# Xiugapurin/Etude

Measured on AMD Instinct MI355X. Metric: audio-sec/s transcribed + decoder tokens/s, 3-min clip batch, higher is better.
Workload: dtype f16

## Files before the change

etude_amd/_lib.py:

```python
from __future__ import annotations

import ctypes as C
import os
from pathlib import Path

import torch

LIB_PATH = Path(os.environ["ETD_LIB_PATH"]) if os.environ.get("ETD_LIB_PATH") else Path(__file__).resolve().parent / "libetude_hip.so"

c_int_p = C.POINTER(C.c_int)
c_i32_p = C.POINTER(C.c_int32)
c_i64_p = C.POINTER(C.c_int64)
c_f32_p = C.POINTER(C.c_float)


class _SizedCfg(C.Structure):

    def __init__(self, *a, **k):
        super().__init__(*a, **k)
        self.struct_bytes = C.sizeof(type(self))


class ExtCfg(_SizedCfg):
    _fields_ = [("struct_bytes", C.c_int)] + [(n, C.c_int) for n in ("n_margin", "n_frame", "n_bin", "cnn_channel", "cnn_kernel", "hid_dim", "pf_dim",
# ... 156 lines not shown
    "etd_prof_entry": (C.c_int, [C.c_int, C.c_char_p, C.c_int, C.POINTER(C.c_double), C.POINTER(C.c_longlong),
                                 C.POINTER(C.c_double), C.POINTER(C.c_double)]),
    "etd_debug_boundary_cost": (C.c_int, [C.c_int, C.c_int, C.c_int, C.c_void_p, C.POINTER(C.c_double), C.POINTER(C.c_double)]),
    "etd_debug_linear": (C.c_int, [C.c_int, C.c_int, C.c_int, C.c_int, C.c_void_p, C.POINTER(C.c_double)]),
    "etd_debug_kernel_loop": (C.c_int, [C.c_int, C.c_int, C.c_void_p]),
    "etd_debug_g3_bounds": (C.c_int, [C.c_void_p, C.c_void_p, C.c_int, C.c_int, C.c_void_p, C.c_void_p, C.c_float, C.c_void_p, C.c_void_p]),
    "etd_debug_gemm3": (C.c_int, [C.c_void_p, C.c_int, C.c_int, C.c_void_p, C.c_void_p, C.c_int, C.c_float, C.c_int, C.c_void_p, C.c_void_p, C.c_void_p, C.c_void_p]),
    "etd_debug_gemm3_case": (C.c_int, [C.POINTER(G3Case), C.c_void_p]),
    "etd_debug_ln_rows_f32": (C.c_int, [C.c_void_p, C.c_int, C.c_int, C.c_void_p, C.c_void_p, C.c_void_p, C.c_void_p, C.c_float, C.c_void_p, C.c_void_p, C.c_void_p]),
    "etd_debug_g3_pack": (C.c_int, [C.c_void_p, C.c_int, C.c_int, C.c_void_p, C.c_longlong, C.POINTER(C.c_longlong), C.POINTER(C.c_int32)]),
    "etd_debug_attn3": (C.c_int, [C.c_void_p, C.c_void_p, C.c_void_p, C.c_void_p, C.c_int, C.c_int, C.c_int, C.c_int, C.c_float, C.c_float, C.c_float, C.c_int, C.c_void_p, C.c_void_p]),
    "etd_debug_attn3_case": (C.c_int, [C.POINTER(Attn3Case), C.c_void_p]),
    "etd_debug_dattn_f32": (C.c_int, [C.c_void_p, C.c_void_p, C.c_void_p, C.c_void_p, C.c_longlong, C.c_longlong, C.c_int, C.c_int, C.c_int, C.c_int, C.c_void_p, C.c_void_p,
                                      C.c_int, C.c_void_p]),
    "etd_debug_empty_launch": (C.c_int, [C.c_int, C.c_int, C.c_int, C.c_void_p, C.c_void_p]),
    "etd_frontend_create": (C.c_int, [C.c_int, C.c_int, C.c_int, C.c_int, C.c_int, C.c_int, C.c_void_p, C.c_int, C.c_int,
                                      C.c_void_p, C.c_int, C.c_void_p, C.c_void_p, C.c_void_p, C.c_float, C.POINTER(C.c_void_p)]),
    "etd_frontend_destroy": (None, [C.c_void_p]),
    "etd_frontend_set_pad_mode": (C.c_int, [C.c_void_p, C.c_int]),
    "etd_rms_frames": (C.c_int, [C.c_void_p, C.c_longlong, C.c_int, C.c_int, C.c_void_p, C.c_longlong, C.c_void_p]),
    "etd_frontend_resampled_len": (C.c_longlong, [C.c_void_p, C.c_longlong]),
    "etd_frontend_num_frames": (C.c_longlong, [C.c_void_p, C.c_longlong]),
    "etd_frontend_run": (C.c_int, [C.c_void_p, C.c_void_p, C.c_int, C.c_longlong, C.c_void_p, C.c_void_p, C.c_longlong,
                                   C.POINTER(C.c_longlong), C.c_void_p]),
    "etd_extractor_create": (C.c_int, [C.POINTER(ExtCfg), C.POINTER(C.c_char_p), C.POINTER(C.c_void_p), c_i64_p, C.c_int,
                                       C.POINTER(C.c_void_p)]),
    "etd_extractor_destroy": (None, [C.c_void_p]),
    "etd_transcript": (C.c_int, [C.c_void_p, C.c_void_p, C.c_longlong] + [C.c_void_p] * 8 + [C.c_void_p]),
    "etd_transcript_windows": (C.c_int, [C.c_void_p, C.c_void_p, C.c_int] + [C.c_void_p] * 8 + [C.c_void_p]),
    "etd_extractor_debug_vel_logits": (C.c_int, [C.c_void_p, C.c_void_p]),
    "etd_extractor_debug_tap": (C.c_int, [C.c_void_p, C.c_int, C.c_void_p]),
    "etd_extractor_window_flops": (C.c_double, [C.c_void_p]),
    "etd_mpe2note": (C.c_int, [C.c_void_p, C.c_void_p, C.c_void_p, C.c_void_p, C.c_longlong, C.c_int, C.c_float, C.c_float,
                               C.c_float, C.c_int, C.c_int, C.c_int, C.POINTER(Note), C.c_longlong, C.POINTER(C.c_longlong)]),
    "etd_mpe2note_modes": (C.c_int, [C.c_void_p, C.c_void_p, C.c_void_p, C.c_void_p, C.c_longlong, C.c_int, C.c_float, C.c_float,
                                     C.c_float, C.c_int, C.c_int, C.c_int, C.c_int, C.c_int, C.POINTER(Note), C.c_longlong, C.POINTER(C.c_longlong)]),
    "etd_mpe2note_dev_create": (C.c_int, [C.c_int, C.POINTER(C.c_void_p)]),
    "etd_mpe2note_dev_destroy": (None, [C.c_void_p]),
    "etd_mpe2note_dev": (C.c_int, [C.c_void_p, C.c_void_p, C.c_void_p, C.c_void_p, C.c_void_p, C.c_longlong, C.c_float, C.c_float, C.c_float,
                                   C.c_int, C.c_int, C.c_int, C.POINTER(Note), C.c_longlong, C.POINTER(C.c_longlong), C.c_void_p]),
    "etd_mpe2note_dev_modes": (C.c_int, [C.c_void_p, C.c_void_p, C.c_void_p, C.c_void_p, C.c_void_p, C.c_longlong, C.c_float, C.c_float, C.c_float,
                                         C.c_int, C.c_int, C.c_int, C.c_int, C.c_int, C.POINTER(Note), C.c_longlong, C.POINTER(C.c_longlong), C.c_void_p]),
    "etd_tok_create": (C.c_int, [C.c_void_p, C.c_int, C.POINTER(C.c_void_p)]),
    "etd_tok_destroy": (None, [C.c_void_p]),
    "etd_tok_num_measures": (C.c_int, [C.c_void_p]),
    "etd_tok_measures": (C.c_int, [C.c_void_p, C.c_void_p, C.c_void_p, C.c_void_p, C.c_void_p]),
    "etd_tok_encode": (C.c_int, [C.c_void_p, C.c_void_p, C.c_longlong, C.c_int, C.c_void_p, C.c_longlong, C.POINTER(C.c_longlong)]),
    "etd_tok_split_bars": (C.c_int, [C.c_void_p, C.c_longlong, C.c_int, C.c_int, C.c_void_p, C.c_longlong, C.c_void_p, C.c_longlong,
                                     C.POINTER(C.c_longlong)]),
    "etd_tok_decode": (C.c_int, [C.c_void_p, C.c_void_p, C.c_longlong, C.c_void_p, C.c_longlong, C.c_void_p, C.c_longlong,
                                 C.POINTER(C.c_longlong)]),
    "etd_midi_write": (C.c_int, [C.c_void_p, C.c_longlong, C.c_char_p]),
    "etd_decoder_create": (C.c_int, [C.POINTER(DecCfg), C.POINTER(C.c_char_p), C.POINTER(C.c_void_p), c_i64_p, C.c_int,
                                     C.POINTER(C.c_void_p)]),
    "etd_decoder_destroy": (None, [C.c_void_p]),
    "etd_decoder_clone": (C.c_int, [C.c_void_p, C.POINTER(C.c_void_p)]),
    "etd_decoder_set_sampling": (C.c_int, [C.c_void_p, C.c_float, C.c_float, C.c_ulonglong, C.c_void_p]),
    "etd_decoder_set_keys": (C.c_int, [C.c_void_p, C.c_int, C.c_void_p, C.c_void_p]),
    "etd_decoder_begin_bar": (C.c_int, [C.c_void_p, C.c_int, C.c_void_p, C.c_void_p, C.c_void_p, C.c_int, C.c_void_p, C.c_int,
                                        C.c_int, C.c_void_p]),
    "etd_decoder_begin_bars": (C.c_int, [C.c_void_p, C.c_int] + [C.c_void_p] * 8 + [C.c_void_p]),
    "etd_decoder_step": (C.c_int, [C.c_void_p, C.c_void_p, C.c_int, C.c_int, C.c_void_p]),
    "etd_decoder_poll": (C.c_int, [C.c_void_p, C.c_void_p, C.c_int, C.c_void_p, C.c_void_p, C.c_void_p]),
    "etd_decoder_read_tokens": (C.c_int, [C.c_void_p, C.c_int, C.c_void_p, C.c_int, c_int_p, C.c_void_p]),
    "etd_decoder_read_many": (C.c_int, [C.c_void_p, C.c_int, C.c_void_p, C.c_void_p, C.c_int, C.c_void_p, C.c_void_p]),
    "etd_decoder_run_jobs": (C.c_int, [C.c_void_p, C.POINTER(SchedCfg), C.POINTER(Job), C.c_int, C.c_void_p, C.c_longlong, C.c_void_p,
                                       C.POINTER(C.c_longlong), C.c_void_p]),
    "etd_debug_assemble_prompt": (C.c_int, [C.POINTER(SchedCfg), C.c_int, C.c_void_p, C.c_void_p, C.c_void_p, C.c_void_p, C.c_void_p, C.c_void_p,
                                            C.c_int, C.c_void_p, C.c_void_p, C.c_void_p, C.c_void_p, C.c_int, c_int_p]),
    "etd_decoder_generate_bar": (C.c_int, [C.c_void_p, C.c_int, C.c_void_p, C.c_void_p, C.c_void_p, C.c_int, C.c_void_p,
                                           C.c_int, C.c_int, C.c_void_p, c_int_p, C.c_void_p]),
    "etd_decoder_prefill_logits": (C.c_int, [C.c_void_p, C.c_int, C.c_void_p, C.c_void_p, C.c_void_p, C.c_int, C.c_void_p,
                                             C.c_void_p]),
    "etd_decoder_score": (C.c_int, [C.c_void_p, C.c_int] + [C.c_void_p] * 11 + [C.c_void_p]),
    "etd_decoder_score_jobs": (C.c_int, [C.c_void_p, C.POINTER(SchedCfg), C.POINTER(ScoreJob), C.c_int, C.c_void_p, C.c_void_p, C.c_void_p, C.c_void_p]),
    "etd_debug_assemble_scored": (C.c_int, [C.POINTER(SchedCfg), C.c_int, C.c_void_p, C.c_void_p, C.c_void_p, C.c_void_p, C.c_void_p, C.c_void_p,
                                            C.c_int, C.c_void_p, C.c_int, C.c_void_p, C.c_void_p, C.c_void_p, C.c_void_p, C.c_void_p, C.c_int, c_int_p]),
    "etd_decoder_step_bytes": (C.c_double, [C.c_void_p, C.c_int, C.c_int]),
    "etd_decoder_stats": (C.c_int, [C.c_void_p, C.POINTER(C.c_double), C.c_int, C.c_void_p]),
    "etd_decoder_stats_reset": (C.c_int, [C.c_void_p, C.c_void_p]),
    "etd_decoder_stamp": (C.c_int, [C.c_void_p, C.c_int, C.c_int, C.c_void_p]),
    "etd_decoder_stamp_log": (C.c_int, [C.c_void_p, C.c_void_p, C.c_longlong, C.POINTER(C.c_longlong), C.c_void_p]),
    "etd_debug_decoder_force_pair": (C.c_int, [C.c_void_p, C.c_int]),
    "etd_debug_decoder_step_logits": (C.c_int, [C.c_void_p, C.c_int, C.c_void_p, C.c_int, C.c_void_p]),
    "etd_debug_decoder_bar_logits": (C.c_int, [C.c_void_p, C.c_void_p, C.c_int, C.c_void_p]),
    "etd_debug_sample_rows": (C.c_int, [C.c_void_p, C.c_int, C.c_int, C.c_int, C.c_float, C.c_float, C.c_ulonglong, C.c_void_p, C.c_void_p, C.c_void_p, C.c_void_p]),
    "etd_debug_decoder_checksum": (C.c_int, [C.c_void_p, C.POINTER(C.c_ulonglong), C.c_int, C.c_void_p]),
    "etd_debug_decoder_kv_rowsums": (C.c_int, [C.c_void_p, C.c_void_p, C.c_longlong, C.c_void_p]),
    "etd_debug_decoder_trace_begin": (C.c_int, [C.c_void_p, C.c_int, C.c_void_p]),
    "etd_debug_decoder_trace_slabs": (C.c_int, [C.c_void_p, C.c_void_p, C.c_longlong, C.c_int, C.c_void_p]),
    "etd_debug_decoder_trace_lanes": (C.c_int, [C.c_void_p, C.c_void_p, C.c_longlong, C.c_int, C.c_void_p]),
    "etd_debug_decoder_trace_q": (C.c_int, [C.c_void_p, C.c_void_p, C.c_longlong, C.c_int, C.c_void_p]),
    "etd_debug_decoder_stage_taps": (C.c_int, [C.c_void_p, C.c_void_p, C.c_void_p]),
    "etd_debug_decoder_peek_kv_many": (C.c_int, [C.c_void_p, C.c_int, C.c_int, C.c_void_p, C.c_int, C.c_void_p, C.c_void_p, C.c_void_p]),
    "etd_debug_decoder_peek_kv": (C.c_int, [C.c_void_p, C.c_int, C.c_int, C.c_int, C.c_int, C.c_void_p, C.c_void_p, C.c_void_p]),
    "etd_beat_create": (C.c_int, [C.POINTER(BeatCfg), C.POINTER(C.c_char_p), C.POINTER(C.c_void_p), c_i64_p, C.c_int, C.POINTER(C.c_void_p)]),
    "etd_beat_destroy": (None, [C.c_void_p]),
    "etd_beat_forward": (C.c_int, [C.c_void_p, C.c_void_p, C.c_int, c_i64_p, C.c_void_p, C.c_void_p, C.c_void_p]),
    "etd_beat_flops": (C.c_double, [C.c_void_p, C.c_longlong]),
    "etd_beat_debug_taps": (C.c_int, [C.c_void_p, C.c_void_p, C.c_void_p]),
    "etd_beat_debug_stage_taps": (C.c_int, [C.c_void_p, C.c_void_p]),
    "etd_dbn_describe": (C.c_int, [C.POINTER(DbnCfg), C.c_int, C.c_void_p, C.c_int, c_int_p, c_int_p, c_int_p, C.c_void_p, C.c_void_p]),
    "etd_dbn_workspace_bytes": (C.c_longlong, [C.POINTER(DbnCfg), C.c_longlong, C.c_int]),
    "etd_dbn_create": (C.c_int, [C.POINTER(DbnCfg), C.POINTER(C.c_void_p)]),
    "etd_dbn_destroy": (None, [C.c_void_p]),
    "etd_dbn_track": (C.c_int, [C.c_void_p, C.c_void_p, C.c_int, C.c_int, c_i64_p, C.c_void_p, C.c_longlong, C.c_void_p, C.c_void_p, C.c_void_p, C.c_longlong,
                                C.c_void_p, C.c_void_p, C.POINTER(C.c_longlong), C.c_void_p]),
    "etd_dbn_debug_viterbi": (C.c_int, [C.c_void_p, C.c_int, C.c_void_p, C.c_longlong, C.c_void_p, C.POINTER(C.c_double)]),
    "etd_stemfeat_create": (C.c_int, [C.POINTER(StemFeatCfg), C.c_void_p, C.c_void_p, C.c_void_p, C.c_void_p, C.POINTER(C.c_void_p)]),
    "etd_stemfeat_destroy": (None, [C.c_void_p]),
    "etd_stemfeat_num_frames": (C.c_longlong, [C.c_void_p, C.c_longlong]),
    "etd_stemfeat_workspace_bytes": (C.c_longlong, [C.c_void_p, C.c_int, C.c_int, c_i64_p]),
    "etd_stemfeat_run": (C.c_int, [C.c_void_p, C.POINTER(C.c_void_p), C.c_int, C.c_int, C.c_int, c_i64_p, C.c_void_p, C.c_void_p]),
    "etd_dtw_create": (C.c_int, [C.POINTER(DtwCfg), C.POINTER(C.c_void_p)]),
    "etd_dtw_destroy": (None, [C.c_void_p]),
    "etd_dtw_limits": (C.c_int, [c_int_p, c_int_p, C.POINTER(C.c_longlong), c_int_p]),
    "etd_dtw_workspace_bytes": (C.c_longlong, [C.c_void_p, C.c_int, c_i64_p, c_i64_p, C.POINTER(C.c_longlong), c_i64_p]),
    "etd_dtw_align": (C.c_int, [C.c_void_p, C.POINTER(C.c_void_p), C.c_int, c_i64_p, c_i64_p, C.c_void_p, C.c_longlong, C.c_void_p, C.c_longlong, C.c_void_p, C.c_void_p]),
    "etd_dtw_debug_cost": (C.c_int, [C.c_void_p, C.POINTER(C.c_void_p), C.c_longlong, C.c_longlong, C.c_int, C.c_void_p]),
    "etd_dtw_debug_path": (C.c_int, [C.c_void_p, C.POINTER(C.c_void_p), C.c_longlong, C.c_longlong, C.c_int, C.c_void_p, C.c_longlong, C.POINTER(C.c_longlong)]),
    "etd_dtw_debug_total": (C.c_int, [C.c_void_p, C.POINTER(C.c_void_p), C.c_longlong, C.c_longlong, C.c_int, C.POINTER(C.c_double)]),
    "etd_alignfeat_limits": (C.c_int, [c_int_p, c_int_p, C.POINTER(C.c_longlong), c_int_p, c_int_p]),
    "etd_alignfeat_create": (C.c_int, [C.POINTER(AlignFeatCfg), C.c_void_p, C.c_void_p, C.c_void_p, C.c_void_p, C.POINTER(C.c_void_p)]),
    "etd_alignfeat_destroy": (None, [C.c_void_p]),
    "etd_alignfeat_num_frames": (C.c_longlong, [C.c_void_p, C.c_longlong]),
    "etd_alignfeat_workspace_bytes": (C.c_longlong, [C.c_void_p, C.c_int, c_i64_p]),
    "etd_alignfeat_run": (C.c_int, [C.c_void_p, C.POINTER(C.c_void_p), C.c_int, c_i64_p, c_i32_p, C.c_void_p, C.c_void_p, C.c_void_p, C.c_longlong, C.c_void_p]),
    "etd_alignfeat_debug_layout": (C.c_int, [C.c_void_p, C.c_int, c_i64_p, C.c_int, c_i64_p, C.c_int]),
    "etd_tuning_limits": (C.c_int, [C.POINTER(C.c_longlong), C.POINTER(C.c_longlong), c_int_p]),
    "etd_tuning_create": (C.c_int, [C.POINTER(TuningCfg), C.POINTER(C.c_void_p)]),
    "etd_tuning_destroy": (None, [C.c_void_p]),
    "etd_tuning_workspace_bytes": (C.c_longlong, [C.c_void_p, C.c_int, c_i64_p]),
    "etd_tuning_run": (C.c_int, [C.c_void_p, C.POINTER(C.c_void_p), C.c_int, c_i64_p, C.c_void_p, C.c_void_p, C.c_void_p, C.c_longlong, C.c_void_p]),
    "etd_tuning_debug_layout": (C.c_int, [C.c_void_p, C.c_int, c_i64_p, C.c_int, c_i64_p, C.c_int]),
    "etd_tuning_debug_power": (C.c_int, [C.c_void_p, C.c_int, c_i32_p, C.c_int, C.c_void_p]),
    "etd_resample_create": (C.c_int, [C.POINTER(ResampleCfg), C.c_void_p, C.POINTER(C.c_void_p)]),
    "etd_resample_destroy": (None, [C.c_void_p]),
    "etd_resample_out_len": (C.c_longlong, [C.c_void_p, C.c_longlong]),
    "etd_resample_workspace_bytes": (C.c_longlong, [C.c_void_p, C.c_int, c_i64_p, c_i32_p, c_i32_p]),
    "etd_resample_run": (C.c_int, [C.c_void_p, C.POINTER(C.c_void_p), C.c_int, c_i64_p, c_i32_p, c_i32_p, c_i32_p, c_i64_p, C.POINTER(C.c_void_p), C.c_void_p, C.c_longlong, C.c_void_p]),
    "etd_resample_debug_layout": (C.c_int, [C.c_void_p, C.c_int, c_i64_p, c_i32_p, c_i32_p, c_i64_p, C.c_longlong, C.POINTER(C.c_longlong)]),
    "etd_rhythm_limits": (C.c_int, [c_int_p, c_int_p, c_int_p, c_int_p]),
    "etd_rhythm_create": (C.c_int, [C.POINTER(RhythmCfg), C.POINTER(C.c_void_p)]),
    "etd_rhythm_destroy": (None, [C.c_void_p]),
    "etd_rhythm_check": (C.c_int, [C.c_void_p, c_i64_p, C.c_int]),
    "etd_rhythm_run": (C.c_int, [C.c_void_p, C.c_void_p, C.c_void_p, c_i64_p, C.c_int, C.c_void_p, C.c_void_p, C.c_void_p]),
    "etd_rhythm_debug_logioi": (C.c_int, [C.c_void_p, C.c_void_p, C.c_void_p, C.c_void_p]),
    "etd_attr_limits": (C.c_int, [c_int_p, c_int_p, c_int_p, c_int_p]),
    "etd_attr_create": (C.c_int, [C.POINTER(AttrCfg), C.c_void_p, C.c_int, C.POINTER(C.c_void_p)]),
    "etd_attr_destroy": (None, [C.c_void_p]),
    "etd_attr_check": (C.c_int, [C.c_void_p, c_i64_p, C.c_int]),
    "etd_attr_run": (C.c_int, [C.c_void_p, C.c_void_p, C.c_void_p, c_i64_p, C.c_int, C.c_void_p, C.c_void_p, C.c_void_p, c_i64_p, C.c_int, C.c_void_p, C.c_int,
                               C.c_void_p, C.c_void_p, C.c_void_p, C.c_void_p, C.c_void_p, C.c_void_p, C.c_void_p]),
    "etd_render_limits": (C.c_int, [c_int_p, C.POINTER(C.c_longlong), c_int_p, c_int_p, c_int_p]),
    "etd_render_create": (C.c_int, [C.POINTER(RenderCfg), C.POINTER(C.c_void_p)]),
    "etd_render_destroy": (None, [C.c_void_p]),
    "etd_render_bytes": (C.c_longlong, [C.c_void_p, C.c_int, c_i64_p, c_i64_p]),
    "etd_render_run": (C.c_int, [C.c_void_p, C.c_void_p, c_i64_p, C.c_void_p, C.c_int, c_i64_p, c_i64_p, C.c_void_p, C.c_void_p, C.c_longlong, C.c_void_p]),
    "etd_render_peaks": (C.c_int, [C.c_void_p, C.c_void_p, C.c_void_p, C.c_void_p, C.c_int, C.c_void_p, C.c_void_p]),
    "etd_render_debug_plan": (C.c_int, [C.c_void_p, C.c_void_p, c_i64_p, C.c_int, c_i64_p, C.c_void_p, C.c_void_p]),
    "etd_sep_create": (C.c_int, [C.POINTER(SepCfg), C.POINTER(C.c_char_p), C.POINTER(C.c_char_p), C.POINTER(C.c_void_p), c_i64_p, C.c_int, C.POINTER(C.c_void_p)]),
    "etd_sep_destroy": (None, [C.c_void_p]),
    "etd_sep_num_frames": (C.c_longlong, [C.c_void_p, C.c_longlong]),
    "etd_sep_unit_bytes": (C.c_longlong, [C.c_void_p]),
    "etd_sep_workspace_bytes": (C.c_longlong, [C.c_void_p, C.c_int, c_i64_p]),
    "etd_sep_run": (C.c_int, [C.c_void_p, C.POINTER(C.c_void_p), C.c_int, c_i64_p, C.POINTER(C.c_void_p), C.c_void_p]),
# ... 175 lines not shown
```

etude_amd/csrc/api_dec.hip:

```cpp
#include <algorithm>
#include <atomic>
#include <chrono>
#include <cmath>
#include <cstdlib>
#include <cstring>
#include <map>
#include <string>
#include <mutex>
#include <vector>

#include "../../include/etude_hip_debug.h"
#include "dec_kernels.h"
#include "gemm3.h"
#include "ext_kernels.h"
#include "dec_score.h"
#include "prof.h"

namespace {

inline uint16_t f2bf_h(float f) { return ETD_DEC_IS_F16 ? f32_to_f16_bits(f) : f32_to_bf16_bits(f); }

struct Lin { void* W = nullptr; float* b = nullptr; int N = 0, Npad = 0, K = 0;
             void* Wf = nullptr;
             G3Lin g3; };
struct Layer { float *ln1g, *ln1b, *ln2g, *ln2b; Lin qkv, dense, up, down;
               void* dense_hw = nullptr;
               Lin cat;
               void* mlp_frag = nullptr;
               int q_log2 = 0, k_log2 = 0, v_log2 = 0; };

}

#define ETD_STAMP_WORDS (ETD_STAMP_HDR + 2 * ETD_STAMP_LOGCAP)
struct etd_dec {
  etd_dec_cfg cfg;
  DevPool pool;
  bool bf16w = false;
  int H, I, V, L, nh, S, ctx, Mmax, Mcap, out_cap;
  float *word = nullptr, *cls_emb = nullptr, *attr_tab = nullptr;
  std::vector<Layer> layers;
  float *lnfg = nullptr, *lnfb = nullptr;
  Lin head;
  float *X1f = nullptr, *X2f = nullptr;
  float *t_q = nullptr, *t_ao = nullptr, *t_do = nullptr, *t_m1 = nullptr;
  void* head_frag = nullptr;
  float *rope_cos = nullptr, *rope_sin = nullptr;
  void *Kc = nullptr, *Vc = nullptr;
  long long slot_stride = 0, layer_stride = 0;
  float *h = nullptr, *h2 = nullptr, *Q = nullptr, *AO = nullptr, *DO = nullptr, *M1 = nullptr, *logits = nullptr;
  int *row_slot = nullptr, *row_pos = nullptr, *row_active = nullptr, *row_sp = nullptr, *ids = nullptr, *slots_dev = nullptr;
  int *cur_tok = nullptr, *len = nullptr, *done = nullptr, *n_out = nullptr, *eos = nullptr, *limit = nullptr, *tgt_attrs = nullptr, *out_tok = nullptr;
  float* tgt_proj = nullptr;
  std::vector<int> last_slots;
  float* qkv_raw = nullptr;
  d16 *X1b = nullptr, *X2b = nullptr, *AOb = nullptr, *M1b = nullptr;
  d16* Qb = nullptr;
  float* hlast = nullptr;
  DSampleCfg* samp_dev = nullptr;
  unsigned long long* rng_key = nullptr;
  std::vector<unsigned long long> host_key; bool keys_dirty = true; bool sampling = false;
  float* Pk = nullptr;
  unsigned* trace = nullptr; int* trace_step = nullptr; int trace_cap = 0; float* trace_pk = nullptr; float* trace_q = nullptr; float* trace_dbg = nullptr;
  int* row_cnt = nullptr;
  d16* Xcat = nullptr;
  std::vector<int> stage;
  int* pin_stage = nullptr; size_t pin_stage_ints = 0; hipEvent_t pin_stage_evt = nullptr;
  int* pin_rb = nullptr;
  std::vector<int> host_n_out; bool host_n_out_valid = false;
  std::map<int, hipGraphExec_t> graphs;
  bool rows_identity = false;
  std::vector<int> host_len;
  double attn_bytes_hint = 0;
  bool step_pair = false;
  double stat_steps = 0, stat_row_steps = 0, stat_kv_bytes = 0, stat_attn_launches = 0, stat_stamp_bytes = 0;
  int force_pair = -1;
  unsigned long long* stamp_dev = nullptr;
  bool stamp_on = false, stamp_armed = false; long long stamp_skip = 0;
  int bar_logit_rows = 0;
  float* logits_dbg = nullptr; bool logits_dbg_on = false, last_step_fused = false;
  int* sc_i = nullptr; float* sc_f = nullptr; double* sc_d = nullptr; float* sc_x = nullptr; int score_hb = 0;
  etd_debug_dec_taps taps = {}; bool taps_on = false;
  etd_dec* weights_owner = nullptr;
  size_t n_weight_allocs = 0;
  int n_clones = 0; bool zombie = false;
};

namespace {

int load_lin(etd_dec* d, const WeightTable& L, const std::string& pfx, int N, int K, bool has_bias, Lin* w) {
  const float* W = L.get(pfx + ".weight", (int64_t)N * K);
  if (!W) return ETD_EINVAL;
  const float* b = nullptr;
  if (has_bias) { b = L.get(pfx + ".bias", N); if (!b) return ETD_EINVAL; }
  const int Npad = ((N + 127) / 128) * 128;
  w->N = N; w->Npad = Npad; w->K = K;
  DevPool& P = d->pool;
  if (d->bf16w) {
    std::vector<uint16_t> hb((size_t)Npad * K, 0);
    for (size_t i = 0; i < (size_t)N * K; ++i) hb[i] = f2bf_h(W[i]);
    uint16_t* p; ETD_TRY(P.upload(&p, hb.data(), hb.size()));
    w->W = p;
    if (K % 16 == 0) {
      std::vector<uint16_t> hp(hb.size());
      pack_wfrag_host(hb.data(), Npad, K, hp.data());
      uint16_t* pf; ETD_TRY(P.upload(&pf, hp.data(), hp.size()));
      w->Wf = pf;
    }
  } else {
    std::vector<float> hf((size_t)Npad * K, 0.f);
    memcpy(hf.data(), W, (size_t)N * K * 4);
    float* p; ETD_TRY(P.upload(&p, hf.data(), hf.size()));
    w->W = p;
    if (K % 32 == 0) {
      ETD_TRY(g3_lin_upload(P, W, b, N, K, 0.f, &w->g3));
      w->b = w->g3.b;
      return ETD_OK;
    }
  }
  std::vector<float> hb2(Npad, 0.f);
  if (b) memcpy(hb2.data(), b, (size_t)N * 4);
  return P.upload(&w->b, hb2.data(), hb2.size());
}

int load_vec(etd_dec* d, const WeightTable& L, const std::string& name, int n, float** dst) {
  const float* p = L.get(name, n);
  if (!p) return ETD_EINVAL;
  return d->pool.upload(dst, p, n);
}

struct PrefillInfo { int n; const int* seq_row0; const int* seq_len; int max_len; double attn_flops; };
__global__ __launch_bounds__(64) void k_trace_rows(const unsigned* buf, long long row_stride, int words, long long slab_stride, int M,
                                                   unsigned* trace, const int* step, int cap, long long wps, int off) {
  const int row = blockIdx.x, slab = blockIdx.y, lane = threadIdx.x;
  const unsigned* p = buf + (long long)slab * slab_stride + (long long)row * row_stride;
  unsigned acc = 0;
  for (int i = lane; i < words; i += 64) acc += p[i] * (2654435761u * (unsigned)(i + 1) | 1u);
  for (int o = 32; o; o >>= 1) acc += __shfl_xor(acc, o);
  if (lane == 0) trace[(long long)(*step % cap) * wps + off + slab * M + row] = acc;
}
__global__ __launch_bounds__(64) void k_trace_kv(const unsigned* Kc, const unsigned* Vc, long long slot_stride_w, int max_ctx, const int* row_slot, const int* row_pos, int M,
                                                 unsigned* trace, const int* step, int cap, long long wps, int off) {
  const int row = blockIdx.x, head = blockIdx.y, lane = threadIdx.x;
  const int slot = row_slot[row], pos = row_pos[row] < max_ctx ? row_pos[row] : max_ctx - 1;
  unsigned* out = trace + (long long)(*step % cap) * wps + off;
  for (int which = 0; which < 2; ++which) {
    const unsigned* base = (which ? Vc : Kc) + (long long)slot * slot_stride_w + (long long)head * max_ctx * 32;
    unsigned a_new = 0, a_all = 0;
    for (long long i = lane; i < (long long)(pos + 1) * 32; i += 64) {
      const unsigned w = base[i] * (2654435761u * (unsigned)(i + 1) | 1u);
      a_all += w;
      if (i >= (long long)pos * 32) a_new += w;
    }
    for (int o = 32; o; o >>= 1) { a_new += __shfl_xor(a_new, o); a_all += __shfl_xor(a_all, o); }
    if (lane == 0) { out[(which * 8 + head) * M + row] = a_new; out[(16 + which * 8 + head) * M + row] = a_all; }
  }
}
__global__ void k_trace_next(int* step) { *step += 1; }
#define ETD_TRACE_LAYER 49
static inline long long trace_wps(const etd_dec* d, int M) { return (long long)(ETD_TRACE_LAYER * d->L + 2) * M; }
static int trace_rows(etd_dec* d, const void* buf, long long row_stride, int words, int nslab, long long slab_stride, int M, int off, hipStream_t st) {
  hipLaunchKernelGGL(k_trace_rows, dim3(M, nslab), dim3(64), 0, st, (const unsigned*)buf, row_stride, words, slab_stride, M, d->trace, d->trace_step,
                     d->trace_cap, trace_wps(d, M), off);
  HIP_TRY(hipGetLastError());
  return ETD_OK;
// ... 177 lines not shown
                       d->row_slot, d->row_pos, M, d->trace, d->trace_step, d->trace_cap, trace_wps(d, M), l * ETD_TRACE_LAYER * M + 17 * M);
    HIP_TRY(hipGetLastError());
  }
  return ETD_OK;
}
static int skinny_attn_down(etd_dec* d, int l, const DecRows& rows, int M, const float* hin, float* hout, hipStream_t st, int ts) {
  const Layer& w = d->layers[l]; const NextLn nx = next_ln(d, l);
  const int ksd = d->I / 512;
  DAttnArgs at = attn_args(d, l, rows, M);
  attn_step_pairs(d, &at); attn_stamp(d, l, &at); at.pair = d->step_pair ? 1 : 0;
  at.dense_w = (const d16*)w.dense_hw; at.dense_out = d->Pk + (size_t)ksd * M * d->H; at.dbg = (d->trace && l == 0) ? d->trace_dbg : nullptr;
  DGemmArgs dn = lin_args(w.cat, nullptr, d->I + d->H, M); dn.Xb = d->Xcat; dn.k_splits = ksd; dn.Y = d->Pk; dn.ldy = d->H;
  if (rowfin_on() && ksd + d->nh == 12 && M <= DS_STEP_MAX_ROWS) {
    DRowFin fin = {};
    fin.cnt = d->row_cnt + (size_t)l * DS_STEP_MAX_ROWS; fin.target = d->nh + 16 * ksd; fin.P = d->Pk; fin.nslab = 12;
    fin.bias = w.cat.b; fin.hin = hin; fin.hout = hout; fin.eps = d->cfg.layer_norm_eps;
    fin.g1 = nx.g1; fin.b1 = nx.b1; fin.g2 = nx.g2; fin.b2 = nx.b2; fin.x1 = nx.x1; fin.x2 = nx.x2;
    return launch_dstep_attn_down(at, dn, &fin, st);
  }
  ETD_TRY(launch_dstep_attn_down(at, dn, nullptr, st));
  ETD_TRY(tap_xcat(d, ts, M, st));
  ETD_TRY(tap_slabs(d, ts, ksd + d->nh, M, st));
  if (d->trace && ksd + d->nh == 12) ETD_TRY(trace_rows(d, d->Pk, d->H, d->H, 12, (long long)M * d->H, M, l * ETD_TRACE_LAYER * M + 2 * M, st));
  if (d->trace && l == 0 && ksd + d->nh == 12) HIP_TRY(hipMemcpyAsync(d->trace_pk, d->Pk, (size_t)12 * M * d->H * 4, hipMemcpyDeviceToDevice, st));
  ETD_TRY(resid_ln(d, l, ksd + d->nh, hin, hout, M, nx, st));
  ETD_TRY(tap_rows(d, d->taps.hout, ts, hout, M, d->H, 4, st));
  if (d->trace) {
    ETD_TRY(trace_rows(d, hout, d->H, d->H, 1, 0, M, l * ETD_TRACE_LAYER * M + 14 * M, st));
    if (nx.x1) {
      ETD_TRY(trace_rows(d, d->X1b, d->H / 2, d->H / 2, 1, 0, M, l * ETD_TRACE_LAYER * M + 15 * M, st));
      ETD_TRY(trace_rows(d, d->X2b, d->H / 2, d->H / 2, 1, 0, M, l * ETD_TRACE_LAYER * M + 16 * M, st));
    }
  }
  return ETD_OK;
}
static int forward_skinny16(etd_dec* d, int M, const DecRows& rows, bool ln0_done, hipStream_t st, float** hfinal) {
  const bool attn_down = rows.slot == d->row_slot && d->H == 512 && d->nh == 8 && d->I % 512 == 0 && d->I / 512 + d->nh <= 12 && d->layers[0].dense_hw &&
                         d->ctx >= 256 && !getenv("ETD_NO_ATTN_DOWN");
  float* hin = d->h; float* hout = d->h2;
  if (!ln0_done) ETD_TRY(ln_rows16(d, 0, hin, M, st));
  for (int l = 0; l < d->L; ++l) {
    const int ts = tap_slice(d, l);
    ETD_TRY(tap_layer_in(d, ts, hin, M, st));
    ETD_TRY(step_qkv_up(d, l, hin, rows, M, st));
    ETD_TRY(tap_rows(d, d->taps.q, ts, d->Q, M, d->H, 4, st));
    ETD_TRY(trace_qkv_up(d, l, M, st));
    if (attn_down) ETD_TRY(skinny_attn_down(d, l, rows, M, hin, hout, st, ts));
    else {
      ETD_TRY(layer_dattn(d, l, rows, M, d->Xcat + d->I, d->I + d->H, st));
      ETD_TRY(tap_xcat(d, ts, M, st));
      ETD_TRY(down_splitk(d, l, hin, hout, M, next_ln(d, l), st, ts));
    }
    std::swap(hin, hout);
  }
  *hfinal = hin;
  return ETD_OK;
}

static int prefill16_qkv(etd_dec* d, int l, const float* hin, const DecRows& rows, int M, bool mfma_attn, hipStream_t st) {
  const Layer& w = d->layers[l];
  DGemmArgs q = qkv_args(d, l, hin, rows, M); q.Xb = d->X1b; q.Y = d->qkv_raw; q.ldy = 3 * d->H;
  if (mfma_attn) q.Qb = d->Qb;
  static const bool pqkv_on = !getenv("ETD_NO_PQKV");
  if (!(mfma_attn && pqkv_on && M >= 49152 && d->H == 512 && d->nh == 8 && w.qkv.N == 1536)) return linear16(w.qkv, d->X1b, M, q, DEPI_QKV, st);
  PQkvArgs pa = {};
  pa.X = d->X1b; pa.ldx = d->H; pa.Wf = (const d16*)w.qkv.Wf; pa.bias = w.qkv.b; pa.M = M; pa.N = w.qkv.N; pa.rows = rows;
  pa.rope_cos = d->rope_cos; pa.rope_sin = d->rope_sin; pa.Qb = d->Qb; pa.Kc = (d16*)q.Kc; pa.Vc = (d16*)q.Vc; pa.slot_stride = d->slot_stride; pa.max_ctx = d->ctx; pa.n_heads = d->nh;
  return launch_pqkv(pa, st);
}
static int prefill16_layer_rest(etd_dec* d, int l, const DecRows& rows, int M, const PrefillInfo* pf, bool fmlp, const float* hin, float* hout, hipStream_t st) {
  const Layer& w = d->layers[l]; const int ts = tap_slice(d, l);
  if (pf) {
    PAttnArgs t = {};
    t.Q = d->Qb; t.ldq = d->H; t.Kc = (const d16*)kv_layer(d, d->Kc, l); t.Vc = (const d16*)kv_layer(d, d->Vc, l); t.slot_stride = d->slot_stride; t.max_ctx = d->ctx; t.n_heads = d->nh;
    t.O = d->Xcat + d->I; t.ldo = d->I + d->H; t.seq_row0 = pf->seq_row0; t.seq_len = pf->seq_len; t.row_slot = rows.slot;
    t.n_seq = pf->n; t.max_len = pf->max_len; t.scale_log2e = 0.125f * 1.4426950408889634f; t.flops_hint = pf->attn_flops;
    ETD_TRY(launch_pattn(t, st));
  } else ETD_TRY(layer_dattn(d, l, rows, M, d->Xcat + d->I, d->I + d->H, st));
  if (fmlp) {
    const NextLn nx = next_ln(d, l); DMlpArgs ma = {};
    ma.X2 = d->X2b; ma.AO = d->Xcat + d->I; ma.ldao = d->I + d->H; ma.hin = hin; ma.hout = hout; ma.Wm = (const d16*)w.mlp_frag;
    ma.b_up = w.up.b; ma.b_cat = w.cat.b; ma.eps = d->cfg.layer_norm_eps; ma.M = M;
    ma.g1 = nx.g1; ma.b1 = nx.b1; ma.g2 = nx.g2; ma.b2 = nx.b2; ma.nx1 = nx.x1; ma.nx2 = nx.x2;
    ETD_TRY(tap_xcat(d, ts, M, st));
    ETD_TRY(launch_dmlp_fused(ma, st));
    return tap_rows(d, d->taps.hout, ts, hout, M, d->H, 4, st);
  }
  DGemmArgs up = {}; up.Yb = d->Xcat; up.ldy = d->I + d->H;
  ETD_TRY(linear16(w.up, d->X2b, M, up, DEPI_GELU, st));
  ETD_TRY(tap_xcat(d, ts, M, st));
  DGemmArgs dn = {}; dn.N = d->H; dn.hin = hin; dn.hout = hout;
  ETD_TRY(linear16(w.cat, d->Xcat, M, dn, DEPI_RESID, st));
  return tap_rows(d, d->taps.hout, ts, hout, M, d->H, 4, st);
}
static int prefill16_last_rows(etd_dec* d, const LastOnly& lo, const float* hin, float* hout, hipStream_t st) {
  const int n = lo.n, l = d->L - 1, ts = tap_slice(d, l, true);
  ETD_TRY(launch_gather_rows(hin, lo.idx, n, d->H, d->hlast, st));
  ETD_TRY(ln_rows16(d, l, d->hlast, n, st));
  ETD_TRY(tap_layer_in(d, ts, d->hlast, n, st));
  ETD_TRY(step_qkv_up(d, l, d->hlast, lo.rows, n, st));
  ETD_TRY(tap_rows(d, d->taps.q, ts, d->Q, n, d->H, 4, st));
  DAttnArgs at = attn_args(d, l, lo.rows, n); at.O = d->AO; at.Ob = d->Xcat + d->I; at.ldob = d->I + d->H; at.bytes_hint = 0;
  ETD_TRY(launch_dattn(at, d->bf16w, st));
  ETD_TRY(tap_xcat(d, ts, n, st));
  return down_splitk(d, l, d->hlast, hout, n, NextLn{}, st, ts);
}
static int forward_prefill16(etd_dec* d, int M, const DecRows& rows, const PrefillInfo* pf, const LastOnly* lo, hipStream_t st, float** hfinal, bool* compact) {
  const bool fmlp = d->layers[0].mlp_frag && d->H == 512 && d->I == 2048 && fused_pmlp_on();
  const bool tail = lo && pf && lo->n > 1 && lo->n <= DS_STEP_MAX_ROWS && step_shape(d) && !getenv("ETD_NO_LAST_ONLY");
  float* hin = d->h; float* hout = d->h2;
  for (int l = 0; l < d->L; ++l) {
    if (l == 0 || !fmlp) ETD_TRY(ln_rows16(d, l, hin, M, st));
    const int ts = tap_slice(d, l);
    ETD_TRY(tap_layer_in(d, ts, hin, M, st));
    ETD_TRY(prefill16_qkv(d, l, hin, rows, M, pf != nullptr, st));
    ETD_TRY(pf ? tap_rows(d, d->taps.qb, ts, d->Qb, M, d->H, 2, st) : tap_rows(d, d->taps.q, ts, d->Q, M, d->H, 4, st));
    ETD_TRY(tail && l == d->L - 1 ? prefill16_last_rows(d, *lo, hin, hout, st) : prefill16_layer_rest(d, l, rows, M, pf, fmlp, hin, hout, st));
    std::swap(hin, hout);
  }
  *hfinal = hin; if (tail) *compact = true;
  return ETD_OK;
}

static int forward_rows(etd_dec* d, int M, const DecRows& rows, const PrefillInfo* pf, const LastOnly* lo, hipStream_t st, float** hfinal, bool* compact) {
  if (compact) *compact = false; else lo = nullptr;
  const Layer& w0 = d->layers[0];
  if (!d->bf16w && M >= G3_MIN_ROWS && d->X1f && w0.qkv.g3.Wp && w0.down.g3.Wp) return forward_x3(d, M, rows, pf, lo, st, hfinal, compact);
  const bool act16 = d->bf16w && M > 1;
  if (act16 && M > DS_MAX_ROWS && w0.qkv.Wf && w0.up.Wf && w0.cat.Wf) return forward_prefill16(d, M, rows, pf, lo, st, hfinal, compact);
  if (act16 && ksplit_fits(d)) return forward_skinny16(d, M, rows, false, st, hfinal);
  return forward_plain(d, M, rows, act16, st, hfinal);
}

int head_logits(etd_dec* d, const float* X, int n, float* logits, hipStream_t st) {
  const bool g3 = !d->bf16w && n >= G3_MIN_ROWS && d->X1f && d->head.g3.Wp;
  if (g3) ETD_TRY(launch_ln_rows_f32(X, n, d->H, d->lnfg, d->lnfb, nullptr, nullptr, d->cfg.layer_norm_eps, d->X1f, nullptr, st));
  DGemmArgs lm = lin_args(d->head, g3 ? d->X1f : X, d->H, n);
  lm.bias = nullptr; lm.Y = logits; lm.ldy = d->V;
  if (g3) return launch_gemm3(lm, DEPI_LOGITS, st);
  lm.ln_g = d->lnfg; lm.ln_b = d->lnfb; lm.ln_eps = d->cfg.layer_norm_eps;
  return launch_dgemm(lm, DEPI_LOGITS, d->bf16w, st);
}

int check_slot(etd_dec* d, int slot) {
  if (!d || slot < 0 || slot >= d->S) ETD_FAIL(ETD_EINVAL, "decoder: bad slot %d", slot);
  return ETD_OK;
}

__global__ void k_init_slots(const int* __restrict__ init, int n, int* tgt_attrs, int* cur_tok, int* len, int* done, int* n_out, int* eos, int* limit) {
  const int i = blockIdx.x * blockDim.x + threadIdx.x;
  if (i >= n) return;
  const int* p = init + i * 7;
  const int s = p[0];
  tgt_attrs[4 * s] = p[1]; tgt_attrs[4 * s + 1] = p[2]; tgt_attrs[4 * s + 2] = p[3]; tgt_attrs[4 * s + 3] = p[4];
  cur_tok[s] = 0; len[s] = 0; done[s] = 0; n_out[s] = 0; eos[s] = p[5]; limit[s] = p[6];
}

__global__ __launch_bounds__(128) void k_slot_proj(const int* __restrict__ init, const float* __restrict__ attr_tab, int n_bins, int H, float* proj) {
  const int* p = init + blockIdx.x * 7;
  const int s = p[0];
  for (int k = threadIdx.x * 4; k < H; k += 128 * 4) {
    f32x4 t[4];
#pragma unroll
    for (int a = 0; a < 4; ++a) t[a] = *reinterpret_cast<const f32x4*>(attr_tab + (long long)(a * n_bins + p[1 + a]) * H + k);
    f32x4 o;
#pragma unroll
    for (int c = 0; c < 4; ++c) o[c] = ((t[0][c] + t[1][c]) + t[2][c]) + t[3][c];
    *reinterpret_cast<f32x4*>(proj + (long long)s * H + k) = o;
  }
}

struct Staged { int Mtot; const int *ids, *cls, *attrs, *row_slot, *row_pos, *row_active, *last_idx, *last_slot, *last_pos, *last_active, *init, *row_seq, *seq_row0, *seq_len; };

int stage_and_forward(etd_dec* d, int n, const int32_t* slots, const int32_t* T, const int32_t* ids, const int32_t* cls,
                      const int32_t* attrs4, const int32_t* init7 , Staged* sg, float** hfinal, hipStream_t st, bool* last_only = nullptr) {
  if (!d || n < 1 || n > d->S || !slots || !T || !ids || !cls || !attrs4) ETD_FAIL(ETD_EINVAL, "prefill: bad arguments");
  long long Mtot = 0;
  std::vector<char> seen((size_t)d->S, 0);
  for (int i = 0; i < n; ++i) {
    ETD_TRY(check_slot(d, slots[i]));
    if (T[i] <= 0 || T[i] > d->ctx) ETD_FAIL(ETD_EINVAL, "prefill: prompt %d has T=%d (max_ctx=%d)", i, T[i], d->ctx);
    if (seen[slots[i]]) ETD_FAIL(ETD_EINVAL, "prefill: slot %d listed twice", slots[i]);
    seen[slots[i]] = 1;
    Mtot += T[i];
  }
  if (Mtot > d->Mcap) ETD_FAIL(ETD_EINVAL, "prefill: %lld prompt rows exceed max_prefill_rows=%d", Mtot, d->Mcap);
  const int M = (int)Mtot;
  ETD_TRY(taps_fit(d, M, DS_K_SPLITS, n > 1 && M > DS_MAX_ROWS));
  for (int i = 0; i < M; ++i) {
    if (ids[i] < 0 || ids[i] >= d->V || cls[i] < 0 || cls[i] >= d->cfg.num_classes) ETD_FAIL(ETD_EINVAL, "prefill: token/class id out of range at row %d", i);
    for (int k = 0; k < 4; ++k) if (attrs4[(size_t)k * M + i] < 0 || attrs4[(size_t)k * M + i] >= d->cfg.num_attribute_bins) ETD_FAIL(ETD_EINVAL, "prefill: attribute bin out of range at row %d", i);
  }
  const size_t sv_ints = (size_t)10 * M + 13 * n;
  int* svp;
  const bool pinned = d->pin_stage && sv_ints <= d->pin_stage_ints;
  if (pinned) {
    HIP_TRY(hipEventSynchronize(d->pin_stage_evt));
    svp = d->pin_stage;
  } else {
    d->stage.resize(sv_ints);
    svp = d->stage.data();
  }
  memcpy(svp, ids, (size_t)M * 4);
  memcpy(svp + M, cls, (size_t)M * 4);
  memcpy(svp + 2 * (size_t)M, attrs4, (size_t)4 * M * 4);
  int* rs = svp + 6 * (size_t)M; int* rp = rs + M; int* ra = rp + M;
  int* li = ra + M; int* ls = li + n; int* lp = ls + n; int* la = lp + n; int* in7 = la + n;
  int* rq = in7 + 7 * n; int* sr0 = rq + M; int* sln = sr0 + n;
  int row = 0, max_len = 0; double kvb = 0, aflops = 0;
  for (int i = 0; i < n; ++i) {
    sr0[i] = row; sln[i] = T[i]; if (T[i] > max_len) max_len = T[i];
    aflops += 0.5 * 256.0 * d->nh * (double)T[i] * T[i];
    for (int t = 0; t < T[i]; ++t, ++row) { rs[row] = slots[i]; rp[row] = t; ra[row] = 1; rq[row] = i; }
    li[i] = row - 1; ls[i] = slots[i]; lp[i] = T[i] - 1; la[i] = 1;
    d->host_len[slots[i]] = T[i];
    kvb += (double)T[i] * d->nh * 64 * (2.0 * (d->bf16w ? 2 : 4) + 4 + 4);
  }
  if (init7) memcpy(in7, init7, (size_t)7 * n * 4); else memset(in7, 0, (size_t)7 * n * 4);
  d->attn_bytes_hint = kvb;
  HIP_TRY(hipMemcpyAsync(d->ids, svp, sv_ints * 4, hipMemcpyHostToDevice, st));
  if (pinned) HIP_TRY(hipEventRecord(d->pin_stage_evt, st));
  d->host_n_out_valid = false;
  const int* b = d->ids;
  *sg = Staged{M, b, b + M, b + 2 * (size_t)M, b + 6 * (size_t)M, b + 7 * (size_t)M, b + 8 * (size_t)M, b + 9 * (size_t)M, b + 9 * (size_t)M + n,
               b + 9 * (size_t)M + 2 * n, b + 9 * (size_t)M + 3 * n, b + 9 * (size_t)M + 4 * n,
               b + 9 * (size_t)M + 11 * n, b + 10 * (size_t)M + 11 * n, b + 10 * (size_t)M + 12 * n};
  if (init7) {
    hipLaunchKernelGGL(k_init_slots, dim3((n + 63) / 64), dim3(64), 0, st, sg->init, n, d->tgt_attrs, d->cur_tok, d->len, d->done, d->n_out, d->eos, d->limit);
    HIP_TRY(hipGetLastError());
    hipLaunchKernelGGL(k_slot_proj, dim3(n), dim3(128), 0, st, sg->init, d->attr_tab, d->cfg.num_attribute_bins, d->H, d->tgt_proj);
    HIP_TRY(hipGetLastError());
  }
  DEmbedArgs e = {};
  e.ids = sg->ids; e.cls = sg->cls; e.attrs = sg->attrs; e.M = M; e.H = d->H; e.n_bins = d->cfg.num_attribute_bins;
  e.word = d->word; e.cls_emb = d->cls_emb; e.attr_tab = d->attr_tab; e.h = d->h;
  e.rows = DecRows{sg->row_slot, sg->row_pos, sg->row_active, sg->row_seq};
  ETD_TRY(launch_dembed(e, st));
  PrefillInfo pf{n, sg->seq_row0, sg->seq_len, max_len, aflops};
  const bool can_mfma_attn = (d->bf16w ? d->Qb != nullptr : d->X1f != nullptr);
  LastOnly lo{n, sg->last_idx, DecRows{sg->last_slot, sg->last_pos, sg->last_active}};
  return forward_rows(d, M, e.rows, can_mfma_attn ? &pf : nullptr, &lo, st, hfinal, last_only);
}

int alloc_workspaces(etd_dec* d) {
  const int H = d->H;
  DevPool& P = d->pool;
  d->slot_stride = (long long)d->nh * d->ctx * 64;
  d->layer_stride = d->slot_stride * d->S;
  const size_t kv_elems = (size_t)d->layer_stride * d->L;
  if (d->bf16w) { uint16_t *k, *v; ETD_TRY(P.alloc(&k, kv_elems, true)); ETD_TRY(P.alloc(&v, kv_elems, true)); d->Kc = k; d->Vc = v; }
  else { float *k, *v; ETD_TRY(P.alloc(&k, kv_elems, true)); ETD_TRY(P.alloc(&v, kv_elems, true)); d->Kc = k; d->Vc = v; }
  const size_t M = d->Mcap;
  const size_t Mf = d->bf16w ? (size_t)(d->S > 1 ? d->S : 1) : M;
  ETD_TRY(P.alloc(&d->h, M * H)); ETD_TRY(P.alloc(&d->h2, M * H));
  ETD_TRY(P.alloc(&d->Q, M * H)); ETD_TRY(P.alloc(&d->AO, M * H)); ETD_TRY(P.alloc(&d->DO, M * H));
  ETD_TRY(P.alloc(&d->M1, Mf * d->I)); ETD_TRY(P.alloc(&d->logits, (size_t)d->Mmax * d->V));
  ETD_TRY(P.alloc(&d->qkv_raw, (size_t)3 * H)); ETD_TRY(P.alloc(&d->hlast, (size_t)d->S * H));
  if (d->bf16w) {
    ETD_TRY(P.alloc(&d->X1b, M * H)); ETD_TRY(P.alloc(&d->X2b, M * H)); ETD_TRY(P.alloc(&d->AOb, M * H));
    ETD_TRY(P.alloc(&d->M1b, M * d->I));
    ETD_TRY(P.alloc(&d->Pk, (size_t)12 * DS_STEP_MAX_ROWS * H));
    ETD_TRY(P.alloc(&d->row_cnt, (size_t)d->L * DS_STEP_MAX_ROWS, true));
    ETD_TRY(P.alloc(&d->Xcat, M * (d->I + H)));
    ETD_TRY(P.alloc(&d->Qb, M * H));
  }
  if (!d->bf16w) {
    ETD_TRY(P.alloc(&d->X1f, M * H)); ETD_TRY(P.alloc(&d->X2f, M * H));
    const size_t Sr = d->S > 1 ? d->S : 1;
    ETD_TRY(P.alloc(&d->t_q, Sr * H)); ETD_TRY(P.alloc(&d->t_ao, Sr * H)); ETD_TRY(P.alloc(&d->t_do, Sr * H)); ETD_TRY(P.alloc(&d->t_m1, Sr * d->I));
  }
  ETD_TRY(P.alloc(&d->samp_dev, (size_t)1, true)); ETD_TRY(P.alloc(&d->rng_key, (size_t)d->S, true));
  ETD_TRY(P.alloc(&d->row_sp, (size_t)2 * d->Mmax, true));
  ETD_TRY(P.alloc(&d->row_slot, (size_t)d->Mmax)); ETD_TRY(P.alloc(&d->row_pos, (size_t)d->Mmax)); ETD_TRY(P.alloc(&d->row_active, (size_t)d->Mmax));
  ETD_TRY(P.alloc(&d->ids, 10 * M + 13 * (size_t)d->S)); ETD_TRY(P.alloc(&d->slots_dev, (size_t)d->S));
  const size_t S = d->S;
  ETD_TRY(P.alloc(&d->cur_tok, S, true)); ETD_TRY(P.alloc(&d->len, S, true)); ETD_TRY(P.alloc(&d->done, S, true));
  ETD_TRY(P.alloc(&d->n_out, S, true)); ETD_TRY(P.alloc(&d->eos, S, true)); ETD_TRY(P.alloc(&d->limit, S, true));
  ETD_TRY(P.alloc(&d->tgt_proj, S * (size_t)d->H, true));
  ETD_TRY(P.alloc(&d->tgt_attrs, 4 * S, true)); ETD_TRY(P.alloc(&d->out_tok, S * d->out_cap, true));
  d->pin_stage_ints = 10 * M + 13 * S;
  if (hipHostMalloc((void**)&d->pin_stage, d->pin_stage_ints * 4, hipHostMallocDefault) != hipSuccess) { d->pin_stage = nullptr; (void)hipGetLastError(); }
  if (hipHostMalloc((void**)&d->pin_rb, (2 * S + S * (size_t)d->out_cap) * 4, hipHostMallocDefault) != hipSuccess) { d->pin_rb = nullptr; (void)hipGetLastError(); }
  if (d->pin_stage && hipEventCreateWithFlags(&d->pin_stage_evt, hipEventDisableTiming) != hipSuccess) { (void)hipHostFree(d->pin_stage); d->pin_stage = nullptr; d->pin_stage_evt = nullptr; }
  d->host_n_out.assign(S, 0);
  return ETD_OK;
}

void free_unborn(etd_dec* d) {
  d->pool.free_all();
  if (d->pin_stage) (void)hipHostFree(d->pin_stage);
  if (d->pin_rb) (void)hipHostFree(d->pin_rb);
  if (d->pin_stage_evt) (void)hipEventDestroy(d->pin_stage_evt);
  delete d;
}

struct LayerBounds { float ln1, ln2, q, k, v, up; };
int layer_bounds(const WeightTable& L, const std::string& p, int H, int I, LayerBounds* B) {
  const float* g1 = L.get(p + "input_layernorm.weight", H); const float* b1 = L.get(p + "input_layernorm.bias", H);
  const float* g2 = L.get(p + "post_attention_layernorm.weight", H); const float* b2 = L.get(p + "post_attention_layernorm.bias", H);
  const float* Wq = L.get(p + "attention.query_key_value.weight", (int64_t)3 * H * H); const float* bq = L.get(p + "attention.query_key_value.bias", 3 * H);
  const float* Wu = L.get(p + "mlp.dense_h_to_4h.weight", (int64_t)I * H); const float* bu = L.get(p + "mlp.dense_h_to_4h.bias", I);
  if (!g1 || !b1 || !g2 || !b2 || !Wq || !bq || !Wu || !bu) return ETD_EINVAL;
  std::vector<float> rb((size_t)3 * H);
  g3_row_bounds_of_ln(Wq, bq, 3 * H, H, g1, b1, rb.data());
  float bnd[3] = {0.f, 0.f, 0.f};
  for (int j = 0; j < 3 * H; ++j) { const int part = (j % 192) >> 6; bnd[part] = fmaxf(bnd[part], rb[j]); }
  *B = LayerBounds{g3_bound_ln(g1, b1, H), g3_bound_ln(g2, b2, H), 2.f * bnd[0], 2.f * bnd[1], bnd[2], g3_bound_linear_of_ln(Wu, bu, I, H, g2, b2)};
  return ETD_OK;
}

}

extern "C" int etd_has_experiments(void) {
#ifdef ETD_EXPERIMENTS
  return 1;
#else
  return 0;
#endif
}

extern "C" int etd_decoder_operand_type(void) { return ETD_DEC_IS_F16; }

extern "C" int etd_decoder_create(const etd_dec_cfg* cfg, const char* const* names, const float* const* host_ptrs,
                                  const int64_t* numels, int n, etd_dec** out) {
  if (!cfg || !names || !host_ptrs || !numels || !out) ETD_FAIL(ETD_EINVAL, "decoder_create: null argument");
  if (cfg->struct_bytes != (int)sizeof(etd_dec_cfg)) ETD_FAIL(ETD_EINVAL, "decoder_create: etd_dec_cfg of %d bytes, this library (ABI %d) expects %d -- caller built against another etude_hip.h", cfg->struct_bytes, ETD_ABI_VERSION, (int)sizeof(etd_dec_cfg));
  const etd_dec_cfg& c = *cfg;
  if (c.hidden_size % 256 || c.num_attention_heads <= 0 || c.hidden_size / c.num_attention_heads != 64 || c.intermediate_size % 128 ||
      (int)(64 * c.rotary_pct) != 16 || c.num_hidden_layers < 1 || c.vocab_size < 2 || c.max_streams < 1 || c.max_ctx < 16 ||
      c.attribute_emb_dim < 1 || c.num_attribute_bins < 1)
    ETD_FAIL(ETD_EINVAL, "decoder_create: unsupported config (need head_dim 64, rotary_ndims 16, hidden %% 256 == 0, intermediate %% 128 == 0)");
  etd_dec* d = new etd_dec();
  d->cfg = c; d->bf16w = c.precision == 1;
  d->H = c.hidden_size; d->I = c.intermediate_size; d->V = c.vocab_size; d->L = c.num_hidden_layers; d->nh = c.num_attention_heads;
  d->S = c.max_streams; d->ctx = c.max_ctx; d->out_cap = 1024;
  d->Mmax = d->ctx > d->S ? d->ctx : d->S;
  d->Mcap = c.max_prefill_rows > d->Mmax ? c.max_prefill_rows : d->Mmax;
  d->host_len.assign(d->S, 0);
  d->host_key.resize(d->S);
  for (int i = 0; i < d->S; ++i) d->host_key[i] = (unsigned long long)i;
  const WeightTable Ld(names, host_ptrs, numels, n);
  DevPool& P = d->pool;
  auto fail = [&](int rc) { free_unborn(d); return rc; };
  const int H = d->H, E = c.attribute_emb_dim, NB = c.num_attribute_bins;
  ETD_TRY_OR(fail, load_vec(d, Ld, "word_embeddings.weight", d->V * H, &d->word));
  ETD_TRY_OR(fail, load_vec(d, Ld, "class_embeddings.weight", c.num_classes * H, &d->cls_emb));
  {
    const char* an[4] = {"pitch_overlap_embeddings.weight", "polyphony_embeddings.weight", "note_sustain_embeddings.weight", "rhythm_intensity_embeddings.weight"};
    const float* pw = Ld.get("attribute_projection.weight", (int64_t)H * 4 * E);
    const float* pb = Ld.get("attribute_projection.bias", H);
    if (!pw || !pb) return fail(ETD_EINVAL);
    std::vector<float> tab((size_t)4 * NB * H);
    for (int a = 0; a < 4; ++a) {
      const float* em = Ld.get(an[a], (int64_t)NB * E);
      if (!em) return fail(ETD_EINVAL);
      for (int b = 0; b < NB; ++b)
        for (int o = 0; o < H; ++o) {
          double s = (a == 0) ? (double)pb[o] : 0.0;
          for (int e = 0; e < E; ++e) s += (double)pw[(size_t)o * 4 * E + a * E + e] * em[b * E + e];
          tab[((size_t)a * NB + b) * H + o] = (float)s;
        }
    }
    ETD_TRY_OR(fail, P.upload(&d->attr_tab, tab.data(), tab.size()));
// ... 70 lines not shown
  ETD_TRY_OR(fail, load_vec(d, Ld, "transformer.final_layer_norm.weight", H, &d->lnfg));
  ETD_TRY_OR(fail, load_vec(d, Ld, "transformer.final_layer_norm.bias", H, &d->lnfb));
  ETD_TRY_OR(fail, load_lin(d, Ld, "lm_head", d->V, H, false, &d->head));
  if (!d->bf16w) {
    const float* gf = Ld.get("transformer.final_layer_norm.weight", H); const float* bf_ = Ld.get("transformer.final_layer_norm.bias", H);
    if (!gf || !bf_) return fail(ETD_EINVAL);
    d->head.g3.x_log2 = g3_scale_log2(g3_bound_ln(gf, bf_, H));
  }
  if (d->bf16w && H % 16 == 0) {
    const float* W = Ld.get("lm_head.weight", (int64_t)d->V * H);
    if (!W) return fail(ETD_EINVAL);
    const int tiles = d->head.Npad / 32, ks = H / 16;
    std::vector<uint16_t> hp((size_t)tiles * ks * 64 * 8, 0);
    for (int t = 0; t < tiles; ++t)
      for (int sx = 0; sx < ks; ++sx)
        for (int l = 0; l < 64; ++l) {
          const int row = t * 32 + (l & 31);
          if (row >= d->V) continue;
          for (int e = 0; e < 8; ++e) hp[(((size_t)t * ks + sx) * 64 + l) * 8 + e] = f2bf_h(W[(size_t)row * H + sx * 16 + (l >> 5) * 8 + e]);
        }
    uint16_t* pp; ETD_TRY_OR(fail, P.upload(&pp, hp.data(), hp.size()));
    d->head_frag = pp;
  }
  {
    std::vector<float> cs((size_t)d->ctx * 8), sn((size_t)d->ctx * 8);
    for (int i = 0; i < 8; ++i) {
      const float inv = 1.0f / powf(c.rope_theta, (float)(2 * i) / 16.0f);
      for (int p = 0; p < d->ctx; ++p) { const float ang = (float)p * inv; cs[(size_t)p * 8 + i] = cosf(ang); sn[(size_t)p * 8 + i] = sinf(ang); }
    }
    ETD_TRY_OR(fail, P.upload(&d->rope_cos, cs.data(), cs.size()));
    ETD_TRY_OR(fail, P.upload(&d->rope_sin, sn.data(), sn.size()));
  }
  d->n_weight_allocs = P.mark();
  ETD_TRY_OR(fail, alloc_workspaces(d));
  if (hipDeviceSynchronize() != hipSuccess) { g_etd_err = "decoder_create: device synchronisation failed"; return fail(ETD_EHIP); }
  *out = d;
  return ETD_OK;
}

static std::mutex g_family_mu;

extern "C" int etd_decoder_clone(etd_dec* src, etd_dec** out) {
  if (!src || !out) ETD_FAIL(ETD_EINVAL, "decoder_clone: null argument");
  etd_dec* own = src->weights_owner ? src->weights_owner : src;
  {
    std::lock_guard<std::mutex> lk(g_family_mu);
    if (own->zombie) ETD_FAIL(ETD_EINVAL, "decoder_clone: the source handle was destroyed");
    ++own->n_clones;
  }
  auto unref = [own]() {
    bool last;
    { std::lock_guard<std::mutex> lk(g_family_mu); last = --own->n_clones == 0 && own->zombie; }
    if (last) { own->pool.free_all(); delete own; }
  };
  etd_dec* d = new etd_dec();
  d->cfg = own->cfg; d->bf16w = own->bf16w;
  d->H = own->H; d->I = own->I; d->V = own->V; d->L = own->L; d->nh = own->nh; d->S = own->S; d->ctx = own->ctx;
  d->Mmax = own->Mmax; d->Mcap = own->Mcap; d->out_cap = own->out_cap;
  d->word = own->word; d->cls_emb = own->cls_emb; d->attr_tab = own->attr_tab; d->layers = own->layers;
  d->lnfg = own->lnfg; d->lnfb = own->lnfb; d->head = own->head; d->head_frag = own->head_frag;
  d->rope_cos = own->rope_cos; d->rope_sin = own->rope_sin;
  d->host_len.assign(d->S, 0);
  d->host_key.resize(d->S);
  for (int i = 0; i < d->S; ++i) d->host_key[i] = (unsigned long long)i;
  d->weights_owner = own;
  int rc = alloc_workspaces(d);
  if (!rc && hipDeviceSynchronize() != hipSuccess) { g_etd_err = "decoder_clone: device synchronisation failed"; rc = ETD_EHIP; }
  if (rc) { free_unborn(d); unref(); return rc; }
  *out = d;
  return ETD_OK;
}

extern "C" void etd_decoder_destroy(etd_dec* d) {
  if (!d) return;
  (void)hipDeviceSynchronize();
  for (auto& kv : d->graphs) (void)hipGraphExecDestroy(kv.second);
  d->graphs.clear();
  if (d->trace) { (void)hipFree(d->trace); d->trace = nullptr; }
  if (d->trace_step) { (void)hipFree(d->trace_step); d->trace_step = nullptr; }
  if (d->trace_pk) { (void)hipFree(d->trace_pk); d->trace_pk = nullptr; }
  if (d->trace_q) { (void)hipFree(d->trace_q); d->trace_q = nullptr; }
  if (d->trace_dbg) { (void)hipFree(d->trace_dbg); d->trace_dbg = nullptr; }
  if (d->stamp_dev) { (void)hipFree(d->stamp_dev); d->stamp_dev = nullptr; }
  if (d->logits_dbg) { (void)hipFree(d->logits_dbg); d->logits_dbg = nullptr; }
  if (d->sc_i) { (void)hipFree(d->sc_i); d->sc_i = nullptr; }
  if (d->sc_f) { (void)hipFree(d->sc_f); d->sc_f = nullptr; }
  if (d->sc_d) { (void)hipFree(d->sc_d); d->sc_d = nullptr; }
  if (d->sc_x) { (void)hipFree(d->sc_x); d->sc_x = nullptr; }
  if (d->pin_stage) { (void)hipHostFree(d->pin_stage); d->pin_stage = nullptr; }
  if (d->pin_rb) { (void)hipHostFree(d->pin_rb); d->pin_rb = nullptr; }
  if (d->pin_stage_evt) { (void)hipEventDestroy(d->pin_stage_evt); d->pin_stage_evt = nullptr; }
  if (d->weights_owner) {
    etd_dec* own = d->weights_owner;
    d->pool.free_all();
    delete d;
    bool last;
    { std::lock_guard<std::mutex> lk(g_family_mu); last = --own->n_clones == 0 && own->zombie; }
    if (last) { own->pool.free_all(); delete own; }
    return;
  }
  bool keep;
  { std::lock_guard<std::mutex> lk(g_family_mu); keep = d->n_clones > 0; if (keep) d->zombie = true; }
  if (keep) {
    d->pool.free_from(d->n_weight_allocs);
    return;
  }
  d->pool.free_all();
  delete d;
}

static DArgmaxArgs argmax_args(const etd_dec* d, const DecRows& rows, int M) {
  DArgmaxArgs am = {};
  am.logits = d->logits; am.ldl = d->V; am.V = d->V; am.M = M; am.rows = rows; am.eos = d->eos; am.limit = d->limit;
  am.cur_tok = d->cur_tok; am.len = d->len; am.done = d->done; am.n_out = d->n_out; am.out_tok = d->out_tok; am.out_cap = d->out_cap;
  return am;
}
extern "C" int etd_decoder_begin_bars(etd_dec* d, int n, const int32_t* slots, const int32_t* T, const int32_t* ids, const int32_t* cls,
                                      const int32_t* attrs4, const int32_t* tgt_attrs4, const int32_t* eos_ids, const int32_t* limits, void* stream) {
  hipStream_t st = (hipStream_t)stream;
  if (!d || n < 1 || !T || !tgt_attrs4 || !eos_ids || !limits) ETD_FAIL(ETD_EINVAL, "begin_bars: bad arguments");
  std::vector<int> init((size_t)7 * n);
  for (int i = 0; i < n; ++i) {
    if (limits[i] < 1 || limits[i] > d->out_cap) ETD_FAIL(ETD_EINVAL, "begin_bars: limit %d outside [1, %d]", limits[i], d->out_cap);
    if ((long long)T[i] + limits[i] - 1 > d->ctx) ETD_FAIL(ETD_EINVAL, "begin_bars: prompt of %d tokens + limit %d needs %d KV positions, max_ctx is %d", T[i], limits[i], T[i] + limits[i] - 1, d->ctx);
    for (int k = 0; k < 4; ++k) if (tgt_attrs4[4 * i + k] < 0 || tgt_attrs4[4 * i + k] >= d->cfg.num_attribute_bins) ETD_FAIL(ETD_EINVAL, "begin_bars: target attribute out of range");
    init[7 * i] = slots ? slots[i] : 0;
    for (int k = 0; k < 4; ++k) init[7 * i + 1 + k] = tgt_attrs4[4 * i + k];
    init[7 * i + 5] = eos_ids[i]; init[7 * i + 6] = limits[i];
  }
  if (d->sampling && d->keys_dirty) {
    HIP_TRY(hipMemcpyAsync(d->rng_key, d->host_key.data(), (size_t)d->S * sizeof(unsigned long long), hipMemcpyHostToDevice, st));
    d->keys_dirty = false;
  }
  if (rowfin_on() && d->row_cnt) HIP_TRY(hipMemsetAsync(d->row_cnt, 0, (size_t)d->L * DS_STEP_MAX_ROWS * sizeof(int), st));
  Staged sg; float* hf = nullptr;
  bool compact = false;
  ETD_TRY(stage_and_forward(d, n, slots, T, ids, cls, attrs4, init.data(), &sg, &hf, st, &compact));
  if (compact) {
    ETD_TRY(head_logits(d, hf, n, d->logits, st));
  } else {
    ETD_TRY(launch_gather_rows(hf, sg.last_idx, n, d->H, d->hlast, st));
    ETD_TRY(head_logits(d, d->hlast, n, d->logits, st));
  }
  DArgmaxArgs am = argmax_args(d, DecRows{sg.last_slot, sg.last_pos, sg.last_active}, n);
  if (d->sampling) { am.samp = d->samp_dev; am.rng_key = d->rng_key; }
  ETD_TRY(launch_dargmax(am, st));
  d->bar_logit_rows = n;
  return ETD_OK;
}

extern "C" int etd_decoder_set_sampling(etd_dec* d, float temperature, float top_p, unsigned long long seed, void* stream) {
  if (!d || !(temperature >= 0.f) || !(top_p == top_p)) ETD_FAIL(ETD_EINVAL, "set_sampling: bad arguments");
  if (temperature > 0.f && d->V > 256) ETD_FAIL(ETD_EINVAL, "set_sampling: sampling supports vocabularies up to 256 entries");
  DSampleCfg c; c.inv_temp = temperature > 0.f ? 1.0f / temperature : 0.f; c.top_p = top_p; c.seed = seed;
  HIP_TRY(hipMemcpyAsync(d->samp_dev, &c, sizeof(c), hipMemcpyHostToDevice, (hipStream_t)stream));
  d->sampling = temperature > 0.f;
  return ETD_OK;
}

extern "C" int etd_decoder_set_keys(etd_dec* d, int n, const int32_t* slots, const unsigned long long* keys) {
  if (!d || n < 1 || !slots || !keys) ETD_FAIL(ETD_EINVAL, "set_keys: bad arguments");
  for (int i = 0; i < n; ++i) { ETD_TRY(check_slot(d, slots[i])); d->host_key[slots[i]] = keys[i]; }
  d->keys_dirty = true;
  return ETD_OK;
}

// ... 68 lines not shown
    const DecRows rows{d->row_slot, d->row_pos, d->row_active};
    if (!fused) ETD_TRY(embed(s_));
    if (fused && d->taps_on) {
      if (d->taps.step_slot) HIP_TRY(hipMemcpyAsync(d->taps.step_slot, d->row_slot, (size_t)n_active * 4, hipMemcpyDeviceToDevice, s_));
      if (d->taps.step_pos) HIP_TRY(hipMemcpyAsync(d->taps.step_pos, d->row_pos, (size_t)n_active * 4, hipMemcpyDeviceToDevice, s_));
    }
    float* hf = nullptr;
    ETD_TRY(fused ? forward_skinny16(d, n_active, rows, true, s_, &hf) : forward_rows(d, n_active, rows, nullptr, nullptr, s_, &hf, nullptr));
    if (fused) {
      ETD_TRY(launch_dstep_head(head_args(d, hf, n_active, vpad), s_));
      if (d->taps_on) {
        ETD_TRY(tap_rows(d, d->taps.next_h, 0, d->h, n_active, d->H, 4, s_));
        ETD_TRY(tap_rows(d, d->taps.next_ln1, 0, d->X1b, n_active, d->H, 2, s_));
        ETD_TRY(tap_rows(d, d->taps.next_ln2, 0, d->X2b, n_active, d->H, 2, s_));
        ETD_TRY(tap_rows(d, d->taps.next_pos, 0, d->row_pos, n_active, 1, 4, s_));
      }
      if (d->trace) {
        ETD_TRY(trace_rows(d, d->h, d->H, d->H, 1, 0, n_active, ETD_TRACE_LAYER * d->L * n_active, s_));
        ETD_TRY(trace_rows(d, d->cur_tok, 1, 1, 1, 0, n_active, ETD_TRACE_LAYER * d->L * n_active + n_active, s_));
        hipLaunchKernelGGL(k_trace_next, dim3(1), dim3(1), 0, s_, d->trace_step);
      }
      return ETD_OK;
    }
    ETD_TRY(head_logits(d, hf, n_active, d->logits, s_));
    DArgmaxArgs am = argmax_args(d, rows, n_active);
    am.samp = d->samp_dev; am.rng_key = d->rng_key;
    ETD_TRY(launch_dargmax(am, s_));
    return ETD_OK;
  };
  if (fused) {
    ETD_TRY(embed(st));
    ETD_TRY(ln_rows16(d, 0, d->h, n_active, st));
  }
  const bool use_graph = st != nullptr && !prof_enabled() && !ETD_XENV("ETD_NO_GRAPH");
  if (use_graph) {
    const int gkey = 16 * n_active + (d->logits_dbg_on ? 8 : 0) + (d->stamp_on ? 4 : 0) + (d->step_pair ? 2 : 0) + (d->rows_identity ? 1 : 0);
    auto it = d->graphs.find(gkey);
    if (it == d->graphs.end()) {
      hipGraph_t g = nullptr;
      HIP_TRY(hipStreamBeginCapture(st, hipStreamCaptureModeThreadLocal));
      const int rc = one_step(st);
      const hipError_t ce = hipStreamEndCapture(st, &g);
      eager_step = 0;
      if (rc != ETD_OK) { if (g) (void)hipGraphDestroy(g); return rc; }
      if (ce != hipSuccess || !g) ETD_FAIL(ETD_EHIP, "decoder_step: stream capture failed: %s", hipGetErrorString(ce));
      hipGraphExec_t ge = nullptr;
      const hipError_t ie = hipGraphInstantiate(&ge, g, nullptr, nullptr, 0);
      (void)hipGraphDestroy(g);
      if (ie != hipSuccess) ETD_FAIL(ETD_EHIP, "decoder_step: graph instantiate failed: %s", hipGetErrorString(ie));
      it = d->graphs.emplace(gkey, ge).first;
    }
    for (int s = 0; s < n_steps; ++s) HIP_TRY(hipGraphLaunch(it->second, st));
  } else {
    for (int s = 0; s < n_steps; ++s) ETD_TRY(one_step(st));
  }
  {
    double kv = 0;
    for (int s2 = 0; s2 < n_steps; ++s2) kv += step_kv_bytes(s2);
    kv *= d->L;
    d->stat_steps += n_steps; d->stat_row_steps += (double)n_steps * n_active; d->stat_kv_bytes += kv; d->stat_attn_launches += (double)n_steps * d->L;
    if (d->stamp_on) d->stat_stamp_bytes += kv + (fused ? (double)n_steps * d->L * ((double)d->I + d->H) * d->H * 2.0 : 0.0);
    for (int i = 0; i < n_active; ++i) { int& hl = d->host_len[slots[i]]; hl = hl + n_steps < d->ctx - 1 ? hl + n_steps : d->ctx - 1; }
  }
  return ETD_OK;
}

extern "C" int etd_decoder_stats(etd_dec* d, double* out, int n, void* stream) {
  if (!d || !out || n < 1) ETD_FAIL(ETD_EINVAL, "decoder_stats: bad arguments");
  unsigned long long sum_ticks = 0, n_stamped = 0;
  if (d->stamp_dev) {
    std::vector<unsigned long long> sp(ETD_STAMP_HDR);
    HIP_TRY(hipStreamSynchronize((hipStream_t)stream));
    HIP_TRY(hipMemcpy(sp.data(), d->stamp_dev, ETD_STAMP_HDR * 8, hipMemcpyDeviceToHost));
    sum_ticks = sp[0]; n_stamped = sp[1];
    for (int bank = 0; bank < 2; ++bank) {
      unsigned long long e = 0;
      for (int i = 0; i < 64; ++i) e = std::max(e, sp[8 + 64 * bank + i]);
      if (sp[2 + bank] != 0 && e > sp[2 + bank]) { sum_ticks += e - sp[2 + bank]; ++n_stamped; }
    }
  }
  double w = 0;
  for (const Layer& l : d->layers) w += ((double)l.qkv.N * l.qkv.K + (double)l.dense.N * l.dense.K + (double)l.up.N * l.up.K + (double)l.down.N * l.down.K) * (d->bf16w ? 2.0 : 4.0);
  w += (double)d->V * d->H * (d->bf16w ? 2.0 : 4.0);
  const double v[8] = {d->stat_steps, d->stat_row_steps, d->stat_kv_bytes, d->stat_attn_launches, (double)n_stamped, (double)sum_ticks * 1e-8 , d->stat_stamp_bytes, w};
  for (int i = 0; i < n; ++i) out[i] = i < 8 ? v[i] : 0.0;
  return ETD_OK;
}

extern "C" int etd_decoder_stamp_log(etd_dec* d, unsigned long long* out_pairs, long long cap, long long* n, void* stream) {
  if (!d || !out_pairs || cap < 1 || !n) ETD_FAIL(ETD_EINVAL, "decoder_stamp_log: bad arguments");
  *n = 0;
  if (!d->stamp_dev) return ETD_OK;
  std::vector<unsigned long long> sp(ETD_STAMP_WORDS);
  HIP_TRY(hipStreamSynchronize((hipStream_t)stream));
  HIP_TRY(hipMemcpy(sp.data(), d->stamp_dev, ETD_STAMP_WORDS * 8, hipMemcpyDeviceToHost));
  long long k = (long long)std::min<unsigned long long>(sp[1], ETD_STAMP_LOGCAP), w = 0;
  for (long long i = 0; i < k && w < cap; ++i, ++w) { out_pairs[2 * w] = sp[ETD_STAMP_HDR + 2 * i]; out_pairs[2 * w + 1] = sp[ETD_STAMP_HDR + 2 * i + 1]; }
  for (int bank = 0; bank < 2 && w < cap; ++bank) {
    unsigned long long e = 0;
    for (int i = 0; i < 64; ++i) e = std::max(e, sp[8 + 64 * bank + i]);
    if (sp[2 + bank] != 0 && e > sp[2 + bank]) { out_pairs[2 * w] = sp[2 + bank]; out_pairs[2 * w + 1] = e; ++w; }
  }
  *n = w;
  return ETD_OK;
}

extern "C" int etd_decoder_stats_reset(etd_dec* d, void* stream) {
  if (!d) ETD_FAIL(ETD_EINVAL, "decoder_stats_reset: null handle");
  d->stat_steps = d->stat_row_steps = d->stat_kv_bytes = d->stat_attn_launches = d->stat_stamp_bytes = 0;
  if (d->stamp_dev) {
    HIP_TRY(hipStreamSynchronize((hipStream_t)stream));
    HIP_TRY(hipMemset(d->stamp_dev, 0, ETD_STAMP_HDR * 8));
  }
  return ETD_OK;
}

extern "C" int etd_decoder_stamp(etd_dec* d, int on, int skip_steps, void* stream) {
  if (!d || skip_steps < 0) ETD_FAIL(ETD_EINVAL, "decoder_stamp: bad arguments");
  if (on && !d->stamp_dev) {
    HIP_TRY(hipMalloc((void**)&d->stamp_dev, ETD_STAMP_WORDS * 8));
    HIP_TRY(hipMemset(d->stamp_dev, 0, ETD_STAMP_WORDS * 8));
  }
  HIP_TRY(hipStreamSynchronize((hipStream_t)stream));
  d->stamp_armed = on != 0; d->stamp_on = false; d->stamp_skip = on ? skip_steps : 0;
  return ETD_OK;
}

extern "C" int etd_debug_decoder_force_pair(etd_dec* d, int mode) {
  if (!d || mode < -1 || mode > 1) ETD_FAIL(ETD_EINVAL, "force_pair: bad arguments");
  d->force_pair = mode;
  return ETD_OK;
}

extern "C" int etd_debug_decoder_step_logits(etd_dec* d, int on, float* out_host, int n_active, void* stream) {
  hipStream_t st = (hipStream_t)stream;
  if (!d || n_active < 0 || n_active > d->S) ETD_FAIL(ETD_EINVAL, "step_logits: bad arguments");
  HIP_TRY(hipStreamSynchronize(st));
  if (out_host && n_active > 0) {
    if (d->last_step_fused && !(d->logits_dbg_on && d->logits_dbg)) ETD_FAIL(ETD_EINVAL, "step_logits: the fused step stores its logits only while the hook is on");
    const float* src = d->last_step_fused ? d->logits_dbg : d->logits;
    HIP_TRY(hipMemcpy(out_host, src, (size_t)n_active * d->V * 4, hipMemcpyDeviceToHost));
  }
  if (on && !d->logits_dbg) HIP_TRY(hipMalloc((void**)&d->logits_dbg, (size_t)d->S * d->V * 4));
  d->logits_dbg_on = on != 0;
  return ETD_OK;
}

extern "C" int etd_debug_decoder_bar_logits(etd_dec* d, float* out_host, int n, void* stream) {
  if (!d || !out_host || n < 1 || n > d->bar_logit_rows) ETD_FAIL(ETD_EINVAL, "bar_logits: bad arguments (the latest begin_bars had %d streams)", d ? d->bar_logit_rows : 0);
  HIP_TRY(hipStreamSynchronize((hipStream_t)stream));
  HIP_TRY(hipMemcpy(out_host, d->logits, (size_t)n * d->V * 4, hipMemcpyDeviceToHost));
  return ETD_OK;
}

extern "C" int etd_decoder_poll(etd_dec* d, const int32_t* slots, int n, int32_t* done_out, int32_t* n_out_out, void* stream) {
  hipStream_t st = (hipStream_t)stream;
  if (!d || !slots || n < 1 || !done_out || !n_out_out) ETD_FAIL(ETD_EINVAL, "decoder_poll: bad args");
  std::vector<int> dnv, nov;
  int *dn, *no;
  if (d->pin_rb) { dn = d->pin_rb; no = d->pin_rb + d->S; }
  else { dnv.resize(d->S); nov.resize(d->S); dn = dnv.data(); no = nov.data(); }
  HIP_TRY(hipMemcpyAsync(dn, d->done, (size_t)d->S * 4, hipMemcpyDeviceToHost, st));
  HIP_TRY(hipMemcpyAsync(no, d->n_out, (size_t)d->S * 4, hipMemcpyDeviceToHost, st));
  HIP_TRY(hipStreamSynchronize(st));
  for (int i = 0; i < n; ++i) { ETD_TRY(check_slot(d, slots[i])); done_out[i] = dn[slots[i]]; n_out_out[i] = no[slots[i]]; }
  memcpy(d->host_n_out.data(), no, (size_t)d->S * 4);
  d->host_n_out_valid = true;
  return ETD_OK;
}

extern "C" int etd_decoder_read_tokens(etd_dec* d, int slot, int32_t* out, int cap, int* n, void* stream) {
  hipStream_t st = (hipStream_t)stream;
  ETD_TRY(check_slot(d, slot));
  if (!out || !n) ETD_FAIL(ETD_EINVAL, "read_tokens: null");
  int cnt = 0;
  HIP_TRY(hipMemcpyAsync(&cnt, d->n_out + slot, 4, hipMemcpyDeviceToHost, st));
  HIP_TRY(hipStreamSynchronize(st));
  if (cnt > d->out_cap) cnt = d->out_cap;
  *n = cnt;
  if (cnt > cap) ETD_FAIL(ETD_ENOMEM, "read_tokens: need room for %d tokens", cnt);
  if (cnt > 0) {
    HIP_TRY(hipMemcpyAsync(out, d->out_tok + (size_t)slot * d->out_cap, (size_t)cnt * 4, hipMemcpyDeviceToHost, st));
    HIP_TRY(hipStreamSynchronize(st));
  }
  return ETD_OK;
}

extern "C" int etd_decoder_read_many(etd_dec* d, int n, const int32_t* slots, int32_t* out, int cap, int32_t* counts, void* stream) {
  hipStream_t st = (hipStream_t)stream;
  if (!d || n < 1 || !slots || !out || !counts || cap < 1) ETD_FAIL(ETD_EINVAL, "read_many: bad args");
  for (int i = 0; i < n; ++i) ETD_TRY(check_slot(d, slots[i]));
  if (!d->host_n_out_valid) {
    HIP_TRY(hipMemcpyAsync(d->host_n_out.data(), d->n_out, (size_t)d->S * 4, hipMemcpyDeviceToHost, st));
    HIP_TRY(hipStreamSynchronize(st));
  }
  int wmax = 0;
  for (int i = 0; i < n; ++i) { int c = d->host_n_out[slots[i]]; if (c > d->out_cap) c = d->out_cap; if (c > wmax) wmax = c; }
  std::vector<int> allv;
  int* all;
  if (d->pin_rb) all = d->pin_rb + 2 * (size_t)d->S; else { allv.resize((size_t)d->S * (wmax > 0 ? wmax : 1)); all = allv.data(); }
  if (wmax > 0) {
    HIP_TRY(hipMemcpy2DAsync(all, (size_t)wmax * 4, d->out_tok, (size_t)d->out_cap * 4, (size_t)wmax * 4, (size_t)d->S, hipMemcpyDeviceToHost, st));
    HIP_TRY(hipStreamSynchronize(st));
  }
  for (int i = 0; i < n; ++i) {
    int c = d->host_n_out[slots[i]]; if (c > d->out_cap) c = d->out_cap;
    if (c > cap) ETD_FAIL(ETD_ENOMEM, "read_many: slot %d holds %d tokens (cap %d)", slots[i], c, cap);
// ... 271 lines not shown
```

etude_amd/csrc/dec_epilogue.h:

```cpp
#pragma once
#include "dec_kernels.h"

__device__ __forceinline__ float gelu_erf(float x) { return 0.5f * x * (1.f + erff(x * 0.70710678118654752440f)); }
__device__ __forceinline__ float gelu_fast(float x) {
  const float u = __builtin_amdgcn_fmed3f(x, -3.875f, 3.875f);
  const float s = u * u;
  float q = fmaf(3.1433767589e-08f, s, -2.0315644633e-06f);
  q = fmaf(q, s, 5.6378066802e-05f); q = fmaf(q, s, -8.9401804144e-04f); q = fmaf(q, s, 9.1527355835e-03f);
  q = fmaf(q, s, -6.5392248333e-02f); q = fmaf(q, s, 3.9845609665e-01f);
  return x * fmaf(q, u, 0.5f);
}

template <bool WBF16, int EPI>
__device__ __forceinline__ void dgemm_epilogue(const DGemmArgs& a, const f32x16& acc, int m, int nb, int h) {
  if constexpr (EPI == DEPI_QKV) {
    const int head = nb / 192, j0 = nb - head * 192, part = j0 >> 6, dbase = j0 & 63;
    float v[16];
#pragma unroll
    for (int i = 0; i < 16; ++i) v[i] = acc[i] + a.bias[nb + acc_row(i, h)];
    const int pos = a.rows.pos[m];
    if (part < 2 && dbase == 0) {
      const int pt = pos < a.max_ctx ? pos : a.max_ctx - 1;
      const float* cs = a.rope_cos + (long long)pt * a.rot_half;
      const float* sn = a.rope_sin + (long long)pt * a.rot_half;
#pragma unroll
      for (int i = 0; i < 4; ++i) {
        const int d = i + 4 * h;
        const float c = cs[d], s = sn[d];
        const float x1 = v[i], x2 = v[i + 4];
        v[i] = x1 * c - x2 * s;
        v[i + 4] = x2 * c + x1 * s;
      }
    }
    if (a.Qb && part == 0) {
      d16* dp = a.Qb + (long long)m * (a.n_heads * 64) + head * 64 + dbase;
#pragma unroll
      for (int q = 0; q < 4; ++q) *reinterpret_cast<d16x4*>(dp + 8 * q + 4 * h) = pack4d(v[4 * q], v[4 * q + 1], v[4 * q + 2], v[4 * q + 3]);
    }
    if (part == 0) {
      if (!a.Qb) {
        float* qp = a.Q + (long long)m * (a.n_heads * 64) + head * 64 + dbase;
#pragma unroll
        for (int q = 0; q < 4; ++q) { const f32x4 o = {v[4 * q], v[4 * q + 1], v[4 * q + 2], v[4 * q + 3]}; *reinterpret_cast<f32x4*>(qp + 8 * q + 4 * h) = o; }
      }
    } else if (a.rows.active[m] && pos < a.max_ctx) {
      const long long off = (long long)a.rows.slot[m] * a.slot_stride + ((long long)head * a.max_ctx + pos) * 64 + dbase;
      void* base = part == 1 ? a.Kc : a.Vc;
      if constexpr (WBF16) {
        d16* kp = reinterpret_cast<d16*>(base) + off;
#pragma unroll
        for (int q = 0; q < 4; ++q) *reinterpret_cast<d16x4*>(kp + 8 * q + 4 * h) = pack4d(v[4 * q], v[4 * q + 1], v[4 * q + 2], v[4 * q + 3]);
      } else {
        float* kp = reinterpret_cast<float*>(base) + off;
#pragma unroll
        for (int q = 0; q < 4; ++q) { const f32x4 o = {v[4 * q], v[4 * q + 1], v[4 * q + 2], v[4 * q + 3]}; *reinterpret_cast<f32x4*>(kp + 8 * q + 4 * h) = o; }
      }
    }
  } else {
#pragma unroll
    for (int q = 0; q < 4; ++q) {
      const int n = nb + 8 * q + 4 * h;
      if (n >= a.N) continue;
      float v[4];
#pragma unroll
      for (int j = 0; j < 4; ++j) {
        v[j] = acc[4 * q + j];
        if (EPI != DEPI_LOGITS && EPI != DEPI_PARTIAL) v[j] += a.bias[n + j];
        if (EPI == DEPI_GELU) v[j] = WBF16 ? gelu_fast(v[j]) : gelu_erf(v[j]);
        if (EPI == DEPI_RELU) v[j] = fmaxf(v[j], 0.f);
      }
      if constexpr (EPI == DEPI_RESID) {
        const f32x4 ad = *reinterpret_cast<const f32x4*>(a.add + (long long)m * a.N + n);
        const f32x4 hi = *reinterpret_cast<const f32x4*>(a.hin + (long long)m * a.N + n);
        const f32x4 o = {(v[0] + ad[0]) + hi[0], (v[1] + ad[1]) + hi[1], (v[2] + ad[2]) + hi[2], (v[3] + ad[3]) + hi[3]};
        *reinterpret_cast<f32x4*>(a.hout + (long long)m * a.N + n) = o;
      } else if (a.Yb) {
        *reinterpret_cast<d16x4*>(a.Yb + (long long)m * a.ldy + n) = pack4d(v[0], v[1], v[2], v[3]);
      } else if (n + 3 < a.N) {
        const f32x4 o = {v[0], v[1], v[2], v[3]};
        float* yp = a.Y + (long long)m * a.ldy + n;
        if ((a.ldy & 3) == 0) *reinterpret_cast<f32x4*>(yp) = o;
        else { yp[0] = v[0]; yp[1] = v[1]; yp[2] = v[2]; yp[3] = v[3]; }
      } else {
        for (int j = 0; j < 4 && n + j < a.N; ++j) a.Y[(long long)m * a.ldy + n + j] = v[j];
      }
    }
  }
}
```

etude_amd/csrc/dec_fused.hip:

```cpp
#include "dec_epilogue.h"
#include "dec_kernels.h"
#include "prof.h"

#include <cstdlib>
#include <utility>
#define PM_SLOT_ELEMS (32 * 1024)

typedef const __attribute__((address_space(1))) void* pm_gptr_t;
typedef __attribute__((address_space(3))) void* pm_lptr_t;

template <int F> __device__ __forceinline__ void pm_rd(d16x8& b, unsigned addr) {
  asm volatile("ds_read_b128 %0, %1 offset:%2" : "=v"(b) : "v"(addr), "n"(F * 1024));
}
template <int F0> __device__ __forceinline__ void pm_rd4(d16x8 (&b)[4], unsigned addr) {
  pm_rd<F0>(b[0], addr); pm_rd<F0 + 1>(b[1], addr); pm_rd<F0 + 2>(b[2], addr); pm_rd<F0 + 3>(b[3], addr);
}
template <int N> __device__ __forceinline__ void pm_wait_lds() { asm volatile("s_waitcnt lgkmcnt(%0)" ::"n"(N) : "memory"); }
__device__ __forceinline__ void pm_mfma_v_a(f32x16& acc, const d16x8& af, const d16x8& bf) {
  asm volatile(ETD_MFMA16_DEC " %0, %1, %2, %0" : "+v"(acc) : "v"(af), "a"(bf));
}
template <int T, bool B_AGPR> __device__ __forceinline__ void pm_mfma_out(f32x16& acc, const d16x8& af, const d16x8& bf) {
  if constexpr (T < 8) {
    if constexpr (B_AGPR) asm volatile(ETD_MFMA16_DEC " %0, %1, %2, %0" : "+a"(acc) : "v"(af), "a"(bf));
    else                  asm volatile(ETD_MFMA16_DEC " %0, %1, %2, %0" : "+a"(acc) : "v"(af), "v"(bf));
// ... 93 lines not shown
    else pm_mfma_out<t0 + (q), false>(acc2[t0 + (q)], buf[J & 1][q], hfk);                                                      \
  } while (0)
  PM_MFMA(0);
  float x0 = 0.f, uu = 0.f, ss = 0.f, qq = 0.f;
  if constexpr (GELU) {
    if constexpr (!LAST) asm volatile("s_waitcnt lgkmcnt(4)" : "+v"(bb) : : "memory"); else asm volatile("s_waitcnt lgkmcnt(0)" : "+v"(bb) : : "memory");
    x0 = g[GR < 0 ? 0 : GR] + bb;
    uu = __builtin_amdgcn_fmed3f(x0, -3.875f, 3.875f);
    ss = uu * uu;
    qq = fmaf(3.1433767589e-08f, ss, -2.0315644633e-06f);
    qq = fmaf(qq, ss, 5.6378066802e-05f);
    PM_PIN(x0); PM_PIN(uu); PM_PIN(ss); PM_PIN(qq);
  }
  PM_MFMA(1);
  if constexpr (GELU) {
    PM_PIN(x0); PM_PIN(uu); PM_PIN(ss); PM_PIN(qq);
    qq = fmaf(qq, ss, -8.9401804144e-04f); qq = fmaf(qq, ss, 9.1527355835e-03f);
    qq = fmaf(qq, ss, -6.5392248333e-02f); qq = fmaf(qq, ss, 3.9845609665e-01f);
    float r0 = x0 * fmaf(qq, uu, 0.5f);
    PM_PIN(r0);
    g[GR < 0 ? 0 : GR] = r0;
  }
  PM_MFMA(2);
  if constexpr (ND >= 1) pm_dma<D0>(nx);
  PM_MFMA(3);
  if constexpr (ND >= 2) pm_dma<D0 + 1>(nx);
#undef PM_MFMA
#undef PM_PIN
  __builtin_amdgcn_sched_barrier(0);
}
template <int KS> __device__ __forceinline__ void pm_hidden_frag1(const f32x16& acc1, d16x8& hfk) {
  const d16x4 p0 = pack4d(acc1[8 * KS], acc1[8 * KS + 1], acc1[8 * KS + 2], acc1[8 * KS + 3]);
  const d16x4 p1 = pack4d(acc1[8 * KS + 4], acc1[8 * KS + 5], acc1[8 * KS + 6], acc1[8 * KS + 7]);
  const u32x2 v0 = __builtin_bit_cast(u32x2, p0), v1 = __builtin_bit_cast(u32x2, p1);
  const auto s0 = __builtin_amdgcn_permlane32_swap(v0[0], v1[0], false, false);
  const auto s1 = __builtin_amdgcn_permlane32_swap(v0[1], v1[1], false, false);
  const u32x4 o = {s0[0], s1[0], s0[1], s1[1]};
  hfk = __builtin_bit_cast(d16x8, o);
  asm volatile("s_nop 4" : "+v"(hfk) : : "memory");
}
#define PM_LOADX(dst, ptr, S) asm volatile("global_load_dwordx4 %0, %1, off offset:%2" : "=a"(dst) : "v"(ptr), "n"(32 * (S)) : "memory")
template <bool AOL>
__device__ __forceinline__ void pm_chunk(d16x8 (&buf)[2][4], unsigned sa, f32x16& prev, f32x16& cur, f32x16 (&acc2)[16], d16x8 (&xf)[32], d16x8 (&hf)[2],
                                         unsigned bias_prev, unsigned bias_cur, const PmNext& nx, const d16* ao, long long ao_off) {
  const d16* ap = nullptr;
  if constexpr (AOL) { ap = ao + ao_off; asm volatile("" : "+v"(ap)); }
#define PM_AOL(G) do { if constexpr (AOL) { PM_LOADX(xf[4 * (G)], ap, 4 * (G)); PM_LOADX(xf[4 * (G) + 1], ap, 4 * (G) + 1); PM_LOADX(xf[4 * (G) + 2], ap, 4 * (G) + 2); PM_LOADX(xf[4 * (G) + 3], ap, 4 * (G) + 3); } } while (0)
  pm_rd4<PmMlpGroup<0>::f0>(buf[0], sa);
  pm_group<0, 4, 0, 2>(buf, sa, cur, acc2, xf, hf[0], prev, bias_prev, nx);
  pm_group<1, 5, 2, 2>(buf, sa, cur, acc2, xf, hf[0], prev, bias_prev, nx);
  pm_group<2, 6, 4, 1>(buf, sa, cur, acc2, xf, hf[0], prev, bias_prev, nx);
  pm_group<3, 7, 5, 1>(buf, sa, cur, acc2, xf, hf[0], prev, bias_prev, nx);
  pm_group<4, 8, 6, 2>(buf, sa, cur, acc2, xf, hf[0], prev, bias_prev, nx);
  pm_group<5, 9, 8, 2>(buf, sa, cur, acc2, xf, hf[0], prev, bias_prev, nx);
  pm_group<6, 10, 10, 1>(buf, sa, cur, acc2, xf, hf[0], prev, bias_prev, nx);
  pm_group<7, 11, 11, 1>(buf, sa, cur, acc2, xf, hf[0], prev, bias_prev, nx);
  pm_hidden_frag1<0>(prev, hf[0]);
  pm_group<8, 12, 12, 1>(buf, sa, cur, acc2, xf, hf[0], prev, bias_prev, nx);
  PM_AOL(0);
  pm_group<9, 13, 13, 1>(buf, sa, cur, acc2, xf, hf[0], prev, bias_prev, nx);
  PM_AOL(1);
  pm_group<10, 14, 14, 1>(buf, sa, cur, acc2, xf, hf[0], prev, bias_prev, nx);
  PM_AOL(2);
  pm_group<11, 15, 15, 1>(buf, sa, cur, acc2, xf, hf[0], prev, bias_prev, nx);
  PM_AOL(3);
  pm_hidden_frag1<1>(prev, hf[1]);
  pm_group<12, 0, 0, 0>(buf, sa, cur, acc2, xf, hf[1], cur, bias_cur, nx);
  PM_AOL(4);
  pm_group<13, 1, 0, 0>(buf, sa, cur, acc2, xf, hf[1], cur, bias_cur, nx);
  PM_AOL(5);
  pm_group<14, 2, 0, 0>(buf, sa, cur, acc2, xf, hf[1], cur, bias_cur, nx);
  PM_AOL(6);
  pm_group<15, 3, 0, 0>(buf, sa, cur, acc2, xf, hf[1], cur, bias_cur, nx);
  PM_AOL(7);
#undef PM_AOL
}

#ifdef ETD_PMLP_STAMP
__device__ unsigned long long g_pmlp_stamp[64 * 4 * 8];
#define PMS(i) do { const unsigned long long t_ = __builtin_amdgcn_s_memtime(); ps_acc[i] += t_ - ps_t; ps_t = t_; } while (0)
#else
#define PMS(i) do { } while (0)
#endif
__global__ __launch_bounds__(256) __attribute__((amdgpu_waves_per_eu(1, 1))) void k_dmlp_fused(DMlpArgs a) {
  __shared__ __attribute__((aligned(16))) unsigned char smem[2 * PM_SLOT_ELEMS * 2 + 2048 * 4];
  d16* ring = reinterpret_cast<d16*>(smem);
  float* sbu = reinterpret_cast<float*>(smem + 2 * PM_SLOT_ELEMS * 2);
  const int tid = threadIdx.x, lane = tid & 63, wave = __builtin_amdgcn_readfirstlane(tid >> 6), r = lane & 31, h = lane >> 5;
  const int m = blockIdx.x * 128 + wave * 32 + r;
  const int mc = m < a.M ? m : a.M - 1;
  const unsigned ring_lds = (unsigned)reinterpret_cast<uintptr_t>(ring) + lane * 16;
#ifdef ETD_PMLP_STAMP
  const unsigned long long ps_t0 = __builtin_amdgcn_s_memtime();
#endif
  const unsigned sbu_lds = (unsigned)reinterpret_cast<uintptr_t>(sbu) + h * 16;

  auto issue = [&](int k) {
    const d16* src = a.Wm + (long long)k * PM_SLOT_ELEMS + wave * (16 * 512) + lane * 8;
    d16* dst = ring + (k & 1) * PM_SLOT_ELEMS + wave * (16 * 512);
#pragma unroll
    for (int i = 0; i < 16; ++i)
      __builtin_amdgcn_global_load_lds((pm_gptr_t)(src + i * 512), (pm_lptr_t)(dst + i * 512), 16, 0, 0);
  };
#define PM_TOP(k)                                                                                                     \
  do {                                                                                                                \
    asm volatile("s_waitcnt vmcnt(0) lgkmcnt(0)" ::: "memory");      \
    __syncthreads();                                     \
  } while (0)
  auto next_of = [&](int k) {
    return PmNext{a.Wm + (long long)(k + 1) * PM_SLOT_ELEMS + wave * (16 * 512) + lane * 8, ring + ((k + 1) & 1) * PM_SLOT_ELEMS + wave * (16 * 512), k + 1 < DMLP_NCHUNK};
  };

  issue(0);
  d16x8 xf[32];
  {
    const d16* xp = a.X2 + (long long)mc * 512 + 8 * h;
#define PM_X4(S) PM_LOADX(xf[S], xp, S); PM_LOADX(xf[(S) + 1], xp, (S) + 1); PM_LOADX(xf[(S) + 2], xp, (S) + 2); PM_LOADX(xf[(S) + 3], xp, (S) + 3)
    PM_X4(0); PM_X4(4); PM_X4(8); PM_X4(12); PM_X4(16); PM_X4(20); PM_X4(24); PM_X4(28);
#undef PM_X4
    asm volatile("s_waitcnt vmcnt(0)" ::: "memory");
  }
#ifdef ETD_PMLP_STAMP
  const unsigned long long ps_tx = __builtin_amdgcn_s_memtime();
#endif
  for (int i = tid; i < 2048; i += 256) sbu[i] = a.b_up[i];

  f32x16 acc2[16];
#pragma unroll
  for (int t = 0; t < 16; ++t)
#pragma unroll
    for (int i = 0; i < 16; ++i) acc2[t][i] = 0.f;
  f32x16 accA, accB;
  d16x8 buf[2][4], hf[2];
  using seq8 = std::make_integer_sequence<int, 8>;
  using seq16 = std::make_integer_sequence<int, 16>;
#define PM_ZERO(x) _Pragma("unroll") for (int i_ = 0; i_ < 16; ++i_) x[i_] = 0.f

  {
    PM_TOP(0);
    PM_ZERO(accA);
    pm_up_only(buf, ring_lds, accA, xf, next_of(0), seq8{});
    asm volatile("s_nop 15\n\ts_nop 15" : "+v"(accA) : : "memory");
    pm_gelu2<0>(accA, sbu, 0, h); pm_gelu2<1>(accA, sbu, 0, h);
  }
#ifdef ETD_PMLP_STAMP
  unsigned long long ps_acc[5] = {0, 0, 0, 0, 0}, ps_t = __builtin_amdgcn_s_memtime();
  const unsigned long long ps_t1 = ps_t;
#define PM_TOP_S(k)                                                                         \
  do {                                                                                      \
    if ((k) > 1) PMS(0); else ps_t = __builtin_amdgcn_s_memtime();                          \
    asm volatile("s_waitcnt vmcnt(0) lgkmcnt(0)" ::: "memory");                             \
    PMS(1);                                                                                 \
    __syncthreads();                                                                        \
    PMS(2);                                                                                 \
  } while (0)
#else
#define PM_TOP_S(k) PM_TOP(k)
#endif
#define PM_CHUNK(k, prev, cur, AOLV)                                                                                                                \
  do {                                                                                                                                          \
    PM_TOP_S(k);                                                                                                                                \
    pm_chunk<(AOLV)>(buf, ring_lds + ((k) & 1) * (PM_SLOT_ELEMS * 2), prev, cur, acc2, xf, hf, sbu_lds + ((k) - 1) * 128, sbu_lds + (k) * 128, next_of(k), a.AO, (long long)mc * a.ldao + 8 * h); \
  } while (0)
  for (int k = 1; k < 63; k += 2) {
    PM_CHUNK(k, accA, accB, false);
    PM_CHUNK(k + 1, accB, accA, false);
  }
  PM_CHUNK(63, accA, accB, true);
#ifdef ETD_PMLP_STAMP
  PMS(0);
  const unsigned long long ps_t2 = ps_t;
#endif
  {
    PM_TOP(64);
    const unsigned sa = ring_lds;
    pm_gelu2<2>(accB, sbu, 63, h); pm_gelu2<3>(accB, sbu, 63, h);
    pm_gelu2<4>(accB, sbu, 63, h); pm_gelu2<5>(accB, sbu, 63, h); pm_gelu2<6>(accB, sbu, 63, h); pm_gelu2<7>(accB, sbu, 63, h);
    pm_hidden_frags(accB, hf);
    pm_down_only(buf, sa, acc2, hf, next_of(64), seq8{});
  }
#ifdef ETD_PMLP_STAMP
  const unsigned long long ps_t2b = __builtin_amdgcn_s_memtime();
#endif
  { PM_TOP(65); pm_dense_chunk<0>(buf, ring_lds + (65 & 1) * (PM_SLOT_ELEMS * 2), acc2, xf, next_of(65), seq16{}); }
  { PM_TOP(66); pm_dense_chunk<1>(buf, ring_lds + (66 & 1) * (PM_SLOT_ELEMS * 2), acc2, xf, next_of(66), seq16{}); }
  { PM_TOP(67); pm_dense_chunk<2>(buf, ring_lds + (67 & 1) * (PM_SLOT_ELEMS * 2), acc2, xf, next_of(67), seq16{}); }
  { PM_TOP(68); pm_dense_chunk<3>(buf, ring_lds + (68 & 1) * (PM_SLOT_ELEMS * 2), acc2, xf, next_of(68), seq16{}); }
  { PM_TOP(69); pm_dense_chunk<4>(buf, ring_lds + (69 & 1) * (PM_SLOT_ELEMS * 2), acc2, xf, next_of(69), seq16{}); }
  { PM_TOP(70); pm_dense_chunk<5>(buf, ring_lds + (70 & 1) * (PM_SLOT_ELEMS * 2), acc2, xf, next_of(70), seq16{}); }
  { PM_TOP(71); pm_dense_chunk<6>(buf, ring_lds + (71 & 1) * (PM_SLOT_ELEMS * 2), acc2, xf, next_of(71), seq16{}); }
  { PM_TOP(72); pm_dense_chunk<7>(buf, ring_lds + (72 & 1) * (PM_SLOT_ELEMS * 2), acc2, xf, next_of(72), seq16{}); }

#ifdef ETD_PMLP_STAMP
  const unsigned long long ps_t3 = __builtin_amdgcn_s_memtime();
#endif
  asm volatile("s_nop 15\n\ts_nop 15" : "+a"(acc2[0]), "+a"(acc2[1]), "+a"(acc2[2]), "+a"(acc2[3]), "+a"(acc2[4]), "+a"(acc2[5]), "+a"(acc2[6]), "+a"(acc2[7]) : : "memory");
  asm volatile("" : "+v"(acc2[8]), "+v"(acc2[9]), "+v"(acc2[10]), "+v"(acc2[11]), "+v"(acc2[12]), "+v"(acc2[13]), "+v"(acc2[14]), "+v"(acc2[15]));
  __syncthreads();
  constexpr int SROW = 132;
  float* stg = reinterpret_cast<float*>(smem) + wave * (32 * SROW + 128);
  float* spar = reinterpret_cast<float*>(smem) + 4 * (32 * SROW + 128);
  for (int i = tid; i < 512; i += 256) {
    spar[i] = a.b_cat[i];
    if (a.nx1) { spar[512 + i] = a.g1[i]; spar[1024 + i] = a.b1[i]; spar[1536 + i] = a.g2[i]; spar[2048 + i] = a.b2[i]; }
  }
  __syncthreads();
  const int m0w = blockIdx.x * 128 + wave * 32;
  const int rrow = lane >> 5, rcol = lane & 31;
  f32x4 hv[16];
  auto load_rows = [&](int g) {
#pragma unroll
    for (int it = 0; it < 16; ++it) {
      int mm = m0w + 2 * it + rrow; mm = mm < a.M ? mm : a.M - 1;
      hv[it] = *reinterpret_cast<const f32x4*>(a.hin + (long long)mm * 512 + g * 128 + rcol * 4);
    }
  };
  load_rows(0);
  float gs[16][2];
#pragma unroll
  for (int g = 0; g < 4; ++g) {
#pragma unroll
    for (int it = 0; it < 16; ++it) *reinterpret_cast<f32x4*>(stg + (2 * it + rrow) * SROW + rcol * 4) = hv[it];
    if (g < 3) load_rows(g + 1);
#pragma unroll
    for (int tt = 0; tt < 4; ++tt)
#pragma unroll
      for (int u = 0; u < 2; ++u) {
        const int t = 4 * g + tt, f0 = 32 * t + 16 * u + 8 * h;
        float* sp = stg + r * SROW + 32 * tt + 16 * u + 8 * h;
        const f32x4 ba = *reinterpret_cast<const f32x4*>(spar + f0), bb = *reinterpret_cast<const f32x4*>(spar + f0 + 4);
        const f32x4 ha = *reinterpret_cast<const f32x4*>(sp), hb = *reinterpret_cast<const f32x4*>(sp + 4);
        float sm = 0.f;
#pragma unroll
        for (int j = 0; j < 4; ++j) {
          const float va = (acc2[t][8 * u + j] + ba[j]) + ha[j], vb = (acc2[t][8 * u + 4 + j] + bb[j]) + hb[j];
          acc2[t][8 * u + j] = va; acc2[t][8 * u + 4 + j] = vb;
        }
#pragma unroll
        for (int j = 0; j < 8; ++j) sm += acc2[t][8 * u + j];
        gs[t][u] = sm;
        const f32x4 oa = {acc2[t][8 * u], acc2[t][8 * u + 1], acc2[t][8 * u + 2], acc2[t][8 * u + 3]};
        const f32x4 ob = {acc2[t][8 * u + 4], acc2[t][8 * u + 5], acc2[t][8 * u + 6], acc2[t][8 * u + 7]};
        *reinterpret_cast<f32x4*>(sp) = oa;
        *reinterpret_cast<f32x4*>(sp + 4) = ob;
      }
#pragma unroll
    for (int it = 0; it < 16; ++it) {
      const int mm = m0w + 2 * it + rrow;
      const f32x4 v = *reinterpret_cast<const f32x4*>(stg + (2 * it + rrow) * SROW + rcol * 4);
      if (mm < a.M) *reinterpret_cast<f32x4*>(a.hout + (long long)mm * 512 + g * 128 + rcol * 4) = v;
    }
  }
#ifdef ETD_PMLP_STAMP
  {
    asm volatile("s_waitcnt vmcnt(0)" ::: "memory");
    const unsigned long long ps_t4 = __builtin_amdgcn_s_memtime();
    if (lane == 0 && blockIdx.x < 64) {
      unsigned long long* o = g_pmlp_stamp + (blockIdx.x * 4 + wave) * 8;
      o[0] = ps_t2b - ps_t2; o[1] = ps_tx - ps_t0; o[2] = ps_acc[1] + ps_acc[2];
      o[3] = ps_t1 - ps_t0; o[4] = ps_t2 - ps_t1; o[5] = ps_t3 - ps_t2; o[6] = ps_t4 - ps_t3;
    }
  }
#endif
  if (!a.nx1) return;
#define PM_FOLD(gsv, tot)                                                                                             \
  {                                                                                                                   \
    _Pragma("unroll") for (int w = 8; w >= 1; w >>= 1)                                                                \
      _Pragma("unroll") for (int t = 0; t < w; ++t) { gsv[t][0] += gsv[t + w][0]; gsv[t][1] += gsv[t + w][1]; }        \
    tot = gsv[0][0] + gsv[0][1];                                                                                      \
    tot += xhalf(tot);                                                                                                \
  }
  float tot;
  PM_FOLD(gs, tot);
  const float mean = tot / 512.f;
#pragma unroll
  for (int t = 0; t < 16; ++t)
#pragma unroll
    for (int u = 0; u < 2; ++u) {
      float q = 0.f;
#pragma unroll
      for (int j = 0; j < 8; ++j) { const float d0 = acc2[t][8 * u + j] - mean; q += d0 * d0; }
      gs[t][u] = q;
    }
  float qt;
  PM_FOLD(gs, qt);
  const float rstd = rsqrtf(qt / 512.f + a.eps);
  d16* stb = reinterpret_cast<d16*>(stg);
#pragma unroll
  for (int which = 0; which < 2; ++which) {
    const float* gam = spar + (which ? 1536 : 512); const float* bet = spar + (which ? 2048 : 1024);
    d16* dstp = which ? a.nx2 : a.nx1;
#pragma unroll
    for (int hh = 0; hh < 2; ++hh) {
#pragma unroll
      for (int tt = 0; tt < 8; ++tt)
#pragma unroll
        for (int u = 0; u < 2; ++u) {
          const int t = 8 * hh + tt, f0 = 32 * t + 16 * u + 8 * h;
          const f32x4 ga = *reinterpret_cast<const f32x4*>(gam + f0), gb = *reinterpret_cast<const f32x4*>(gam + f0 + 4);
          const f32x4 ba = *reinterpret_cast<const f32x4*>(bet + f0), bb = *reinterpret_cast<const f32x4*>(bet + f0 + 4);
          d16x8 o;
#pragma unroll
          for (int j = 0; j < 4; ++j) {
            o[j] = (d16)((acc2[t][8 * u + j] - mean) * rstd * ga[j] + ba[j]); o[4 + j] = (d16)((acc2[t][8 * u + 4 + j] - mean) * rstd * gb[j] + bb[j]);
          }
          *reinterpret_cast<d16x8*>(stb + r * (2 * SROW) + 32 * tt + 16 * u + 8 * h) = o;
        }
#pragma unroll
      for (int it = 0; it < 16; ++it) {
        const int mm = m0w + 2 * it + rrow;
        const u32x4 v = *reinterpret_cast<const u32x4*>(stb + (2 * it + rrow) * (2 * SROW) + rcol * 8);
        if (mm < a.M) *reinterpret_cast<u32x4*>(dstp + (long long)mm * 512 + hh * 256 + rcol * 8) = v;
      }
    }
  }
#ifdef ETD_PMLP_STAMP
  asm volatile("s_waitcnt vmcnt(0)" ::: "memory");
  if (lane == 0 && blockIdx.x < 64) g_pmlp_stamp[(blockIdx.x * 4 + wave) * 8 + 7] = __builtin_amdgcn_s_memtime() - ps_t0;
#endif
}

#ifdef ETD_PMLP_STAMP
extern "C" int etd_debug_pmlp_stamps(unsigned long long* out) {
  HIP_TRY(hipDeviceSynchronize());
  HIP_TRY(hipMemcpyFromSymbol(out, HIP_SYMBOL(g_pmlp_stamp), sizeof(unsigned long long) * 64 * 4 * 8));
  return ETD_OK;
}
#endif
int launch_dmlp_fused(const DMlpArgs& a, hipStream_t st) {
  if (a.M <= 0 || !a.X2 || !a.AO || a.ldao < 512 || (a.ldao % 8) || !a.hin || !a.hout || a.hin == a.hout || !a.Wm || !a.b_up || !a.b_cat ||
      (((uintptr_t)a.X2 | (uintptr_t)a.AO | (uintptr_t)a.Wm | (uintptr_t)a.hin | (uintptr_t)a.hout | (uintptr_t)a.nx1 | (uintptr_t)a.nx2) & 15) ||
      (a.nx1 && (!a.nx2 || !a.g1 || !a.b1 || !a.g2 || !a.b2)))
    ETD_FAIL(ETD_EINVAL, "dmlp_fused: bad arguments");
  ProfScope ps("k_dmlp_fused", st, 2.0 * a.M * 512.0 * (2048.0 * 2 + 512.0), (double)a.M * 512 * (2 + 2 + 4 + 4 + (a.nx1 ? 4 : 0)) + (double)DMLP_STREAM_ELEMS * 2);
  hipLaunchKernelGGL(k_dmlp_fused, dim3((a.M + 127) / 128), dim3(256), 0, st, a);
  HIP_TRY(hipGetLastError());
  return ETD_OK;
}

void pack_dmlp_weights(const uint16_t* Wup, const uint16_t* Wcat, uint16_t* dst) {
  auto perm = [](int r) { const int i = (r & 3) + 4 * (r >> 3), hh = (r >> 2) & 1; return 16 * (i >> 3) + 8 * hh + (i & 7); };
  const int KC = 2560;
  for (int k = 0; k < DMLP_NCHUNK; ++k)
    for (int fr = 0; fr < 64; ++fr)
      for (int l = 0; l < 64; ++l) {
        const int r = l & 31, h = l >> 5;
        uint16_t* d = dst + (((size_t)k * 64 + fr) * 64 + l) * 8;
        for (int j = 0; j < 8; ++j) d[j] = 0;
        if (k <= 64) {
          if (fr < 32) {
            if (k == 0) continue;
            const int ks = fr >> 4, t = fr & 15, feat = 32 * t + perm(r);
            for (int j = 0; j < 8; ++j) d[j] = Wcat[(size_t)feat * KC + 32 * (k - 1) + 16 * ks + 8 * h + j];
          } else {
            if (k == 64) continue;
            const int s = fr - 32;
            for (int j = 0; j < 8; ++j) d[j] = Wup[(size_t)(32 * k + r) * 512 + 16 * s + 8 * h + j];
          }
        } else {
          const int dc = k - 65, sl = fr >> 4, t = fr & 15, feat = 32 * t + perm(r), s = 4 * dc + sl;
          for (int j = 0; j < 8; ++j) d[j] = Wcat[(size_t)feat * KC + 2048 + 16 * s + 8 * h + j];
        }
      }
}
```

etude_amd/csrc/dec_kernels.h:

```cpp
#pragma once
#include "common.h"

#ifdef ETD_DEC_BF16
typedef bf16 d16; typedef bf16x8 d16x8; typedef bf16x4 d16x4; typedef bf16x2 d16x2;
#define ETD_MFMA16_DEC "v_mfma_f32_32x32x16_bf16"
#define ETD_DEC_IS_F16 0
#ifdef __HIPCC__
__device__ __forceinline__ d16x4 pack4d(float a, float b, float c, float d) { return pack4(a, b, c, d); }
#endif
#else
typedef f16 d16; typedef f16x8 d16x8; typedef f16x4 d16x4; typedef f16x2 d16x2;
#define ETD_MFMA16_DEC "v_mfma_f32_32x32x16_f16"
#define ETD_DEC_IS_F16 1
#ifdef __HIPCC__
__device__ __forceinline__ d16x4 pack4d(float a, float b, float c, float d) { return pack4h(a, b, c, d); }
#endif
#endif

#define DS_MAX_ROWS 512
#define DS_STEP_MAX_ROWS 2048

struct DecRows {
  const int* slot;
  const int* pos;
// ... 20 lines not shown
  d16* Yb;
  int k_splits;
  const d16* Xb;
  const float* add; const float* hin; float* hout;
  DecRows rows;
  const float* rope_cos; const float* rope_sin;
  int rot_half;
  float* Q;
  void* Kc; void* Vc;
  long long slot_stride;
  int max_ctx, n_heads;
  d16* Qb;
  const void* Wp; int w_log2;
  int x_log2;
};
int launch_dgemm(const DGemmArgs& a, int epi, bool w_bf16, hipStream_t st);
int launch_dstep_qkv_up(const DGemmArgs& q, const DGemmArgs& up, hipStream_t st);

struct DHeadArgs {
  const float* hfin; int M, H, V, Vpad;
  const float* lnf_g; const float* lnf_b; float eps;
  const d16* Whead;
  int* row_slot; int* row_pos; int* row_active; int* row_sp;
  int* cur_tok; int* len; int* done; int* n_out; int* out_tok; int out_cap; const int* eos; const int* limit;
  const int* tgt_attrs; const float* tgt_proj ; int tgt_cls; int n_bins;
  const float* word; const float* cls_emb; const float* attr_tab;
  const float* g1; const float* b1; const float* g2; const float* b2;
  float* h; d16* x1; d16* x2;
  const DSampleCfg* samp; const unsigned long long* rng_key;
  float* logits_dbg;
};
int launch_dstep_head(const DHeadArgs& a, hipStream_t st);

struct DAttnArgs {
  const float* Q;
  const void* Kc; const void* Vc; long long slot_stride; int max_ctx, n_heads;
  DecRows rows; int M;
  const int* row_sp;
  int identity;
  int pair;
  float* O;
  d16* Ob; int ldob;
  float scale;
  double bytes_hint;
  const d16* dense_w;
  float* dense_out;
  float* dbg;
  unsigned long long* stamp;
  int stamp_par;
};
int launch_dattn(const DAttnArgs& a, bool kv_bf16, hipStream_t st);
struct DRowFin {
  int* cnt; int target;
  const float* P; int nslab;
  const float* bias; const float* hin; float* hout;
  const float* g1; const float* b1; const float* g2; const float* b2; float eps;
  d16* x1; d16* x2;
};
int launch_dstep_attn_down(const DAttnArgs& a, const DGemmArgs& down, const DRowFin* fin, hipStream_t st);

struct PAttnArgs {
  const d16* Q; int ldq;
  const d16* Kc; const d16* Vc;
  long long slot_stride; int max_ctx, n_heads;
  d16* O; int ldo;
  const int* seq_row0; const int* seq_len; const int* row_slot;
  int n_seq, max_len;
  float scale_log2e;
  double flops_hint;
};
int launch_pattn(const PAttnArgs& a, hipStream_t st);

struct PQkvArgs {
  const d16* X; int ldx;
  const d16* Wf;
  const float* bias;
  int M, N;
  DecRows rows;
  const float* rope_cos; const float* rope_sin;
  d16* Qb;
  d16* Kc; d16* Vc; long long slot_stride; int max_ctx, n_heads;
};
int launch_pqkv(const PQkvArgs& a, hipStream_t st);

int launch_ln_rows(const float* h, int M, int H, const float* g1, const float* b1, const float* g2, const float* b2, float eps,
                   d16* x1, d16* x2, hipStream_t st);
int launch_resid_ln_rows(const float* P, int k_splits, const float* bias, const float* add, const float* hin, float* hout, int M, int H,
                         const float* g1, const float* b1, const float* g2, const float* b2, float eps, d16* x1, d16* x2, hipStream_t st);
int launch_gather_rows(const float* src, const int* idx, int n, int H, float* out, hipStream_t st);

#define DMLP_NCHUNK 73
#define DMLP_STREAM_ELEMS (DMLP_NCHUNK * 32 * 1024)
struct DMlpArgs {
  const d16* X2;
  const d16* AO; int ldao;
  const float* hin; float* hout;
  const d16* Wm;
  const float* b_up;
  const float* b_cat;
  const float* g1; const float* b1; const float* g2; const float* b2; float eps;
  d16* nx1; d16* nx2;
  int M;
};
int launch_dmlp_fused(const DMlpArgs& a, hipStream_t st);
void pack_dmlp_weights(const uint16_t* Wup_bf16 , const uint16_t* Wcat_bf16 , uint16_t* dst );

struct DEmbedArgs {
  const int* ids; const int* cls; const int* attrs;
  const int* cur_tok; const int* tgt_attrs;
  int tgt_cls;
  DecRows rows; int M, H, n_bins;
  const int* slots; const int* len; const int* done;
  int* row_slot_out; int* row_pos_out; int* row_active_out; int* row_sp_out;
  const float* word; const float* cls_emb; const float* attr_tab;
  float* h;
};
int launch_dembed(const DEmbedArgs& a, hipStream_t st);

struct DArgmaxArgs {
  const float* logits; int ldl; int V; int M;
  DecRows rows;
  int* cur_tok; int* len; int* done; int* n_out; int* out_tok; int out_cap; const int* eos; const int* limit;
  int set_len_from_pos;
  const DSampleCfg* samp; const unsigned long long* rng_key;
};
int launch_dargmax(const DArgmaxArgs& a, hipStream_t st);
extern "C" int etd_debug_sample_rows(const float* logits_dev, int M, int V, int ld, float temperature, float top_p, unsigned long long seed,
                                     const unsigned long long* keys_dev, const unsigned* ctrs_dev, int* out_tok_dev, void* stream);
```

etude_amd/csrc/dec_prefill.hip:

```cpp
#include "dec_kernels.h"
#include "prof.h"

#include <cstdlib>

#define PA_LDK 72
#define PA_LDV 96

typedef __attribute__((ext_vector_type(4))) short pa_s16x4;
typedef __attribute__((address_space(3))) pa_s16x4* pa_lds_s16x4;

__global__ __launch_bounds__(256) void k_pattn(PAttnArgs a) {
  __shared__ __attribute__((aligned(16))) unsigned char smem[64 * PA_LDK * 2 + 64 * PA_LDV * 2];
  d16* Ks = reinterpret_cast<d16*>(smem);
  d16* Vs = Ks + 64 * PA_LDK;
  const int tid = threadIdx.x, lane = tid & 63, wave = __builtin_amdgcn_readfirstlane(tid >> 6), r = lane & 31, h = lane >> 5;
  const int nh = a.n_heads;
  const int seq = blockIdx.y / nh, head = blockIdx.y - seq * nh;
  const int S = a.seq_len[seq];
  const long long r0 = a.seq_row0[seq];
  const int off = (128 - (S & 127)) & 127;
  if ((int)blockIdx.x * 128 - off >= S) return;
  const int slot = a.row_slot[r0];
  const int q0 = (int)blockIdx.x * 128 + wave * 32 - off;
  int qi = q0 + r; const bool qvalid = qi >= 0 && qi < S; qi = qi < 0 ? 0 : (qi < S ? qi : S - 1);
// ... 157 lines not shown
      __builtin_amdgcn_global_load_lds((pq_gptr_t)(src + 2048), (pq_lptr_t)(dst + 2048), 16, 0, 0);
      __builtin_amdgcn_global_load_lds((pq_gptr_t)(src + 2048), (pq_lptr_t)(dst + 2048), 16, 1024, 0);
      __builtin_amdgcn_global_load_lds((pq_gptr_t)(src + 2048), (pq_lptr_t)(dst + 2048), 16, 2048, 0);
      __builtin_amdgcn_global_load_lds((pq_gptr_t)(src + 2048), (pq_lptr_t)(dst + 2048), 16, 3072, 0);
    }
  };
  issue(0);
  for (int i = tid; i < a.N; i += 64 * NW) sb[i] = a.bias[i];
  d16x8 xf[32];
  {
    const d16* xp = a.X + (long long)mc * a.ldx + 8 * h;
#pragma unroll
    for (int s = 0; s < 32; ++s) xf[s] = *reinterpret_cast<const d16x8*>(xp + 16 * s);
  }
  const int pos_l = a.rows.pos[mc];
  const f32x4 c4 = *reinterpret_cast<const f32x4*>(a.rope_cos + (long long)pos_l * 8 + 4 * h);
  const f32x4 s4 = *reinterpret_cast<const f32x4*>(a.rope_sin + (long long)pos_l * 8 + 4 * h);
  const int er8 = lane >> 3, ec8 = lane & 7;
  long long qoff[4], coff[4];
#pragma unroll
  for (int it = 0; it < 4; ++it) {
    const int mr = mw + it * 8 + er8, mrc = mr < a.M ? mr : a.M - 1;
    const int rpos = a.rows.pos[mrc], rslot = a.rows.slot[mrc], ract = a.rows.active[mrc];
    qoff[it] = mr < a.M ? (long long)mr * (a.n_heads * 64) + ec8 * 8 : -1;
    coff[it] = (mr < a.M && ract && rpos < a.max_ctx) ? (long long)rslot * a.slot_stride + (long long)rpos * 64 + ec8 * 8 : -1;
  }
  const unsigned ring_l = (unsigned)reinterpret_cast<uintptr_t>(ring) + lane * 16;

  auto store_block = [&](int u) {
    const int head = u / 3, part = u - head * 3;
    d16* cbase = (part == 1 ? a.Kc : a.Vc) + (long long)head * a.max_ctx * 64;
#pragma unroll
    for (int it = 0; it < 4; ++it) {
      const u32x4 val = *reinterpret_cast<const u32x4*>(stg + (it * 8 + er8) * PQ_EPP + ec8 * 8);
      if (part == 0) { if (qoff[it] >= 0) *reinterpret_cast<u32x4*>(a.Qb + qoff[it] + head * 64) = val; }
      else if (coff[it] >= 0) *reinterpret_cast<u32x4*>(cbase + coff[it]) = val;
    }
  };
#define PQ_RD4(buf, F0)                                                                                                  \
  do {                                                                                                                   \
    asm volatile("ds_read_b128 %0, %1 offset:%2" : "=v"(buf[0]) : "v"(sl), "n"((F0) * 1024));                            \
    asm volatile("ds_read_b128 %0, %1 offset:%2" : "=v"(buf[1]) : "v"(sl), "n"((F0) * 1024 + 1024));                     \
    asm volatile("ds_read_b128 %0, %1 offset:%2" : "=v"(buf[2]) : "v"(sl), "n"((F0) * 1024 + 2048));                     \
    asm volatile("ds_read_b128 %0, %1 offset:%2" : "=v"(buf[3]) : "v"(sl), "n"((F0) * 1024 + 3072));                     \
  } while (0)
#define PQ_MFMA(c, af, bfr) asm volatile(ETD_MFMA16_DEC " %0, %1, %2, %0" : "+v"(c) : "v"(af), "v"(bfr))
#define PQ_MFMA0(c, af, bfr) asm volatile(ETD_MFMA16_DEC " %0, %1, %2, 0" : "=&v"(c) : "v"(af), "v"(bfr))
#define PQ_GROUP(c, G)                                                                                                   \
  do {                                                                                                                   \
    if constexpr ((G) < 7) { PQ_RD4(wf[((G) + 1) & 1], ((G) + 1) * 4); asm volatile("s_waitcnt lgkmcnt(4)" ::: "memory"); } \
    else asm volatile("s_waitcnt lgkmcnt(0)" ::: "memory");                                                              \
    if constexpr ((G) == 0) PQ_MFMA0(c, wf[0][0], xf[0]); else PQ_MFMA(c, wf[(G) & 1][0], xf[4 * (G)]);                  \
    PQ_MFMA(c, wf[(G) & 1][1], xf[4 * (G) + 1]);                                                                         \
    PQ_MFMA(c, wf[(G) & 1][2], xf[4 * (G) + 2]);                                                                         \
    PQ_MFMA(c, wf[(G) & 1][3], xf[4 * (G) + 3]);                                                                         \
    __builtin_amdgcn_sched_barrier(0);                                                                                   \
  } while (0)
#define PQ_TILE(c, t)                                                                                                    \
  do {                                                                                                                   \
    asm volatile("s_waitcnt vmcnt(0) lgkmcnt(0)" ::: "memory");    \
    __syncthreads();                                               \
    if ((t) + 1 < NT) issue((t) + 1);                                                                                    \
    if ((t) >= 2 && !((t) & 1)) store_block(((t) - 2) >> 1);                                                              \
    const unsigned sl = ring_l + ((t) & 1) * (PQ_TILE_ELEMS * 2);                                                        \
    d16x8 wf[2][4];                                                                                                     \
    asm volatile("s_waitcnt lgkmcnt(0)" ::: "memory");             \
    __builtin_amdgcn_sched_barrier(0);                                                                                   \
    PQ_RD4(wf[0], 0);                                                                                                    \
    PQ_GROUP(c, 0); PQ_GROUP(c, 1); PQ_GROUP(c, 2); PQ_GROUP(c, 3); PQ_GROUP(c, 4); PQ_GROUP(c, 5); PQ_GROUP(c, 6); PQ_GROUP(c, 7); \
  } while (0)
  for (int u = 0; u < (NT >> 1); ++u) {
    f32x16 c0, c1;
    PQ_TILE(c0, 2 * u);
    PQ_TILE(c1, 2 * u + 1);
    asm volatile("s_nop 15\n\ts_nop 15" : "+v"(c1) : : "memory");
    {
      const int part = u % 3;
      float v[2][16];
#pragma unroll
      for (int i = 0; i < 16; ++i) { v[0][i] = c0[i] + sb[64 * u + acc_row(i, h)]; v[1][i] = c1[i] + sb[64 * u + 32 + acc_row(i, h)]; }
      if (part < 2) {
#pragma unroll
        for (int i = 0; i < 4; ++i) {
          const float x1 = v[0][i], x2 = v[0][i + 4];
          v[0][i] = x1 * c4[i] - x2 * s4[i];
          v[0][i + 4] = x2 * c4[i] + x1 * s4[i];
        }
      }
#pragma unroll
      for (int nn = 0; nn < 2; ++nn)
#pragma unroll
        for (int q = 0; q < 4; ++q)
          *reinterpret_cast<d16x4*>(stg + r * PQ_EPP + nn * 32 + 8 * q + 4 * h) = pack4d(v[nn][4 * q], v[nn][4 * q + 1], v[nn][4 * q + 2], v[nn][4 * q + 3]);
    }
  }
#undef PQ_TILE
#undef PQ_GROUP
#undef PQ_MFMA
#undef PQ_MFMA0
#undef PQ_RD4
  store_block((NT >> 1) - 1);
}

int launch_pqkv(const PQkvArgs& a, hipStream_t st) {
  if (a.M <= 0 || a.N != 1536 || a.ldx < 512 || (a.ldx % 8) || !a.X || !a.Wf || !a.bias || !a.Qb || !a.Kc || !a.Vc || !a.rows.pos || !a.rows.slot || !a.rows.active ||
      !a.rope_cos || !a.rope_sin || a.n_heads != 8 || (((uintptr_t)a.X | (uintptr_t)a.Wf | (uintptr_t)a.Qb | (uintptr_t)a.Kc | (uintptr_t)a.Vc) & 15) || (a.slot_stride % 8))
    ETD_FAIL(ETD_EINVAL, "pqkv: bad arguments");
  ETD_LAUNCH_FILTER("k_pqkv");
  ProfScope ps("k_pqkv", st, 2.0 * a.M * a.N * 512.0, ((double)a.M * 512 + (double)a.N * 512 + 3.0 * a.M * 512) * 2);
  static const int nw = getenv("ETD_PQKV_WAVES") ? atoi(getenv("ETD_PQKV_WAVES")) : 8;
  if (nw == 4) hipLaunchKernelGGL(k_pqkv<4>, dim3((a.M + 127) / 128), dim3(256), 0, st, a);
  else hipLaunchKernelGGL(k_pqkv<8>, dim3((a.M + 255) / 256), dim3(512), 0, st, a);
  HIP_TRY(hipGetLastError());
  return ETD_OK;
}
```

etude_amd/csrc/ext_kernels.hip:

```cpp
#include "ext_kernels.h"
#include "prof.h"
#include "dec_epilogue.h"
#include <cstdint>
#include <cstdlib>
#include <cstdio>
#include <vector>

#define LDK 72
#define EPP 136

typedef __amdgpu_buffer_rsrc_t rsrc_t;
__device__ __forceinline__ rsrc_t lin_rsrc(const void* p, long long bytes) {
  return __builtin_amdgcn_make_buffer_rsrc(const_cast<void*>(p), 0, (int)(bytes > 0x7fffffffLL ? 0x7fffffffLL : bytes), 0x00020000);
}
__device__ __forceinline__ void lin_gload_x4(rsrc_t xs, const int (&xo)[4], int kc, u32x4 (&xr)[4]) {
#pragma unroll
  for (int i = 0; i < 4; ++i) xr[i] = __builtin_bit_cast(u32x4, __builtin_amdgcn_raw_buffer_load_b128(xs, xo[i], kc * 128, 0));
}
__device__ __forceinline__ void lin_gload_w8(rsrc_t ws, const int (&wo)[8], int kc, u32x4 (&wr)[8]) {
#pragma unroll
  for (int i = 0; i < 8; ++i) wr[i] = __builtin_bit_cast(u32x4, __builtin_amdgcn_raw_buffer_load_b128(ws, wo[i], kc * 128, 0));
}
__device__ __forceinline__ void lin_lstore_xw(e16* Xs, e16* Ws, int tid, const u32x4 (&xr)[4], const u32x4 (&wr)[8]) {
#pragma unroll
// ... 187 lines not shown
    if constexpr (EPI == DEPI_GELU) {
#pragma unroll
      for (int mt = 0; mt < 2; ++mt) {
#pragma unroll
        for (int nt = 0; nt < 4; ++nt)
#pragma unroll
          for (int q = 0; q < 4; ++q) {
            const int fl = nt * 32 + 8 * q + 4 * h, f = wn * 128 + fl;
            *reinterpret_cast<d16x4*>(stg + r * EPP + fl) =
                pack4d(gelu_fast(acc[mt][nt][4 * q] + sb[f]), gelu_fast(acc[mt][nt][4 * q + 1] + sb[f + 1]),
                      gelu_fast(acc[mt][nt][4 * q + 2] + sb[f + 2]), gelu_fast(acc[mt][nt][4 * q + 3] + sb[f + 3]));
          }
        __syncthreads();
#pragma unroll
        for (int it = 0; it < 8; ++it) {
          const int row = it * 4 + er, m = mw + mt * 32 + row;
          if (m < a.M) *reinterpret_cast<u32x4*>(g.Yb + (long long)m * g.ldy + nw + ec * 8) = *reinterpret_cast<const u32x4*>(stg + row * EPP + ec * 8);
        }
        __syncthreads();
      }
    } else if constexpr (EPI == DEPI_RESID) {
#pragma unroll
      for (int mt = 0; mt < 2; ++mt)
#pragma unroll
        for (int ntp = 0; ntp < 2; ++ntp) {
#pragma unroll
          for (int nn = 0; nn < 2; ++nn)
#pragma unroll
            for (int q = 0; q < 4; ++q) {
              const int nt = ntp * 2 + nn, fl = nn * 32 + 8 * q + 4 * h, f = wn * 128 + ntp * 64 + fl;
              const f32x4 o = {acc[mt][nt][4 * q] + sb[f], acc[mt][nt][4 * q + 1] + sb[f + 1], acc[mt][nt][4 * q + 2] + sb[f + 2], acc[mt][nt][4 * q + 3] + sb[f + 3]};
              *reinterpret_cast<f32x4*>(stf + r * (EPP / 2) + fl) = o;
            }
          __syncthreads();
#pragma unroll
          for (int it = 0; it < 8; ++it) {
            const int row = it * 4 + er, m = mw + mt * 32 + row;
            if (m < a.M) {
              const long long off = (long long)m * g.N + nw + ntp * 64 + ec * 4;
              f32x4 v = *reinterpret_cast<const f32x4*>(stf + row * (EPP / 2) + ec * 4);
              if (g.add) { const f32x4 ad = *reinterpret_cast<const f32x4*>(g.add + off); v[0] += ad[0]; v[1] += ad[1]; v[2] += ad[2]; v[3] += ad[3]; }
              const f32x4 hi = *reinterpret_cast<const f32x4*>(g.hin + off);
              const f32x4 o = {v[0] + hi[0], v[1] + hi[1], v[2] + hi[2], v[3] + hi[3]};
              *reinterpret_cast<f32x4*>(g.hout + off) = o;
            }
          }
          __syncthreads();
        }
    } else if constexpr (EPI == DEPI_QKV) {
      if (!g.Qb) {
#pragma unroll
        for (int mt = 0; mt < 2; ++mt) {
          const int m = mw + mt * 32 + r;
          if (m < a.M) {
#pragma unroll
            for (int nt = 0; nt < 4; ++nt) dgemm_epilogue<true, EPI>(g, acc[mt][nt], m, nw + nt * 32, h);
          }
        }
      } else {
        const int er8 = lane >> 3, ec8 = lane & 7;
#pragma unroll
        for (int mt = 0; mt < 2; ++mt) {
          const int ml = mw + mt * 32 + r, mlc = ml < a.M ? ml : a.M - 1;
          const int pos_l = g.rows.pos[mlc];
          int rpos[4], rslot[4], ract[4];
#pragma unroll
          for (int it = 0; it < 4; ++it) {
            int m = mw + mt * 32 + it * 8 + er8; m = m < a.M ? m : a.M - 1;
            rpos[it] = g.rows.pos[m]; rslot[it] = g.rows.slot[m]; ract[it] = g.rows.active[m];
          }
#pragma unroll
          for (int ntp = 0; ntp < 2; ++ntp) {
            const int fb = nw + ntp * 64, head = fb / 192, part = (fb - head * 192) >> 6;
            float v[2][16];
#pragma unroll
            for (int nn = 0; nn < 2; ++nn)
#pragma unroll
              for (int i = 0; i < 16; ++i) v[nn][i] = acc[mt][ntp * 2 + nn][i] + sb[wn * 128 + ntp * 64 + nn * 32 + acc_row(i, h)];
            if (part < 2) {
              const f32x4 c4 = *reinterpret_cast<const f32x4*>(g.rope_cos + (long long)pos_l * 8 + 4 * h);
              const f32x4 s4 = *reinterpret_cast<const f32x4*>(g.rope_sin + (long long)pos_l * 8 + 4 * h);
#pragma unroll
              for (int i = 0; i < 4; ++i) {
                const float x1 = v[0][i], x2 = v[0][i + 4];
                v[0][i] = x1 * c4[i] - x2 * s4[i];
                v[0][i + 4] = x2 * c4[i] + x1 * s4[i];
              }
            }
#pragma unroll
            for (int nn = 0; nn < 2; ++nn)
#pragma unroll
              for (int q = 0; q < 4; ++q)
                *reinterpret_cast<d16x4*>(stg + r * EPP + nn * 32 + 8 * q + 4 * h) = pack4d(v[nn][4 * q], v[nn][4 * q + 1], v[nn][4 * q + 2], v[nn][4 * q + 3]);
            __syncthreads();
#pragma unroll
            for (int it = 0; it < 4; ++it) {
              const int row = it * 8 + er8, m = mw + mt * 32 + row;
              if (m < a.M) {
                const u32x4 val = *reinterpret_cast<const u32x4*>(stg + row * EPP + ec8 * 8);
                if (part == 0) *reinterpret_cast<u32x4*>(g.Qb + (long long)m * (g.n_heads * 64) + head * 64 + ec8 * 8) = val;
                else {
                  if (ract[it] && rpos[it] < g.max_ctx) {
                    d16* cp = reinterpret_cast<d16*>(part == 1 ? g.Kc : g.Vc) + (long long)rslot[it] * g.slot_stride + ((long long)head * g.max_ctx + rpos[it]) * 64 + ec8 * 8;
                    *reinterpret_cast<u32x4*>(cp) = val;
                  }
                }
              }
            }
            __syncthreads();
          }
        }
      }
    } else {
#pragma unroll
      for (int mt = 0; mt < 2; ++mt) {
        const int m = mw + mt * 32 + r;
        if (m < a.M) {
#pragma unroll
          for (int nt = 0; nt < 4; ++nt) dgemm_epilogue<true, EPI>(g, acc[mt][nt], m, nw + nt * 32, h);
        }
      }
    }
  } else if constexpr (!LN) {
    if constexpr (vt) {
      const bool rowseg = (a.S % 64 == 0) && (a.M % 64 == 0) && (a.Spad % 8 == 0) && (a.vtz % 8 == 0) && ((reinterpret_cast<uintptr_t>(a.VT) & 15) == 0) && !(a.dbg & 4);
      if (rowseg) {
        const int mb = m0 + wm * 64, seq = mb / a.S, pos0 = mb - seq * a.S;
#pragma unroll
        for (int nt = 0; nt < 4; ++nt) {
          const float b = sb[wn * 128 + nt * 32 + r];
#pragma unroll
          for (int mt = 0; mt < 2; ++mt)
#pragma unroll
            for (int q = 0; q < 4; ++q)
              *reinterpret_cast<e16x4*>(stg + r * 72 + mt * 32 + 8 * q + 4 * h) =
                  pack4e(acc[mt][nt][4 * q] + b, acc[mt][nt][4 * q + 1] + b, acc[mt][nt][4 * q + 2] + b, acc[mt][nt][4 * q + 3] + b);
          __syncthreads();
          if (mb < a.M) {
#pragma unroll
            for (int it = 0; it < 4; ++it) {
              const int row = it * 8 + (lane >> 3), ch = lane & 7, fr = wn * 128 + nt * 32 + row;
              e16* dst = a.VT + (long long)z * a.vtz + ((long long)(seq * 4 + (fr >> 6)) * 64 + (fr & 63)) * a.Spad + pos0 + ch * 8;
              *reinterpret_cast<u32x4*>(dst) = *reinterpret_cast<const u32x4*>(stg + row * 72 + ch * 8);
            }
          }
          __syncthreads();
        }
      } else
#pragma unroll
      for (int nt = 0; nt < 4; ++nt) {
        const int f = wn * 128 + nt * 32 + r;
        const float b = sb[f];
        const int head = f >> 6, d = f & 63;
#pragma unroll
        for (int mt = 0; mt < 2; ++mt)
#pragma unroll
          for (int q = 0; q < 4; ++q) {
            const int m = m0 + wm * 64 + mt * 32 + 8 * q + 4 * h;
            if (m < a.M) {
              const int seq = m / a.S, pos = m - seq * a.S;
              e16* dst = a.VT + (long long)z * a.vtz + ((long long)(seq * 4 + head) * 64 + d) * a.Spad + pos;
              *reinterpret_cast<e16x4*>(dst) = pack4e(acc[mt][nt][4 * q] + b, acc[mt][nt][4 * q + 1] + b, acc[mt][nt][4 * q + 2] + b, acc[mt][nt][4 * q + 3] + b);
            }
          }
      }
    } else {
      e16* ybase = a.Y + (long long)z * a.yz + nw + ec * 8;
#pragma unroll
      for (int mt = 0; mt < 2; ++mt) {
// ... 539 lines not shown
```

include/etude_hip_debug.h:

```cpp
#ifndef ETUDE_HIP_DEBUG_H
#define ETUDE_HIP_DEBUG_H
#include "etude_hip.h"

#ifdef __cplusplus
extern "C" {
#endif

int etd_debug_boundary_cost(int n_nodes, int iters, int big_args, void* stream, double* eager_us, double* graph_us);
int etd_debug_linear(int M, int N, int K, int iters, void* stream, double* us);
int etd_debug_kernel_loop(int which, int iters, void* stream);
int etd_debug_empty_launch(int gx, int gy, int gz, int* sink_dev, void* stream);

int etd_extractor_debug_vel_logits(etd_ext*, float* vel_logits_dev);
int etd_extractor_debug_tap(etd_ext*, int stage, void* dst_dev);

int etd_debug_assemble_prompt(const etd_sched_cfg* cfg, int n_hist, const int32_t* const* hx, const int32_t* hxn, const int32_t* const* hy,
                              const int32_t* hyn, const int32_t* hattrs4, const int32_t* x, int xn, const int32_t* y_attrs4,
                              int32_t* ids_out, int32_t* cls_out, int32_t* attrs4_out, int cap, int* T_out);
int etd_debug_assemble_scored(const etd_sched_cfg* cfg, int n_hist, const int32_t* const* hx, const int32_t* hxn, const int32_t* const* hy,
                              const int32_t* hyn, const int32_t* hattrs4, const int32_t* x, int xn, const int32_t* y, int yn, const int32_t* y_attrs4,
                              int32_t* ids_out, int32_t* cls_out, int32_t* attrs4_out, int32_t* labels_out, int cap, int* T_out);

int etd_debug_decoder_checksum(etd_dec*, unsigned long long* out, int cap, void* stream);
int etd_debug_decoder_kv_rowsums(etd_dec*, unsigned* out_host, long long cap, void* stream);
int etd_debug_decoder_trace_begin(etd_dec*, int cap_steps, void* stream);
int etd_debug_decoder_trace_slabs(etd_dec*, float* out_host, long long cap_floats, int n_active, void* stream);
int etd_debug_decoder_trace_lanes(etd_dec*, float* out_host, long long cap_floats, int n_active, void* stream);
int etd_debug_decoder_trace_q(etd_dec*, float* out_host, long long cap_floats, int n_active, void* stream);
int etd_debug_decoder_peek_kv(etd_dec*, int layer, int slot, int head, int n_pos, unsigned short* k_out, unsigned short* v_out, void* stream);
int etd_debug_decoder_trace_read(etd_dec*, unsigned* out_host, long long cap_words, int n_active, int* steps_done, void* stream);

int etd_debug_decoder_force_pair(etd_dec*, int mode);
int etd_debug_decoder_step_logits(etd_dec*, int on, float* out_host, int n_active, void* stream);
int etd_debug_decoder_bar_logits(etd_dec*, float* out_host, int n, void* stream);
typedef struct etd_debug_dec_taps {
  int struct_bytes;
  unsigned layer_mask;
  int rows, hidden, intermediate, slab_cap;
  int slices;
  float* hin;
  void *ln1, *ln2;
  float* q;
  void* qb;
  void* xcat;
  float* slabs;
  float* hout;
  int32_t *step_slot, *step_pos;
  float* next_h; void *next_ln1, *next_ln2; int32_t* next_pos;
} etd_debug_dec_taps;
int etd_debug_decoder_stage_taps(etd_dec*, const etd_debug_dec_taps* taps, void* stream);
int etd_debug_decoder_peek_kv_many(etd_dec*, int layer, int n, const int32_t* slots, int n_pos, unsigned short* k_out, unsigned short* v_out, void* stream);

int etd_debug_sample_rows(const float* logits_dev, int M, int V, int ld, float temperature, float top_p, unsigned long long seed,
                          const unsigned long long* keys_dev, const unsigned* ctrs_dev, int* out_tok_dev, void* stream);

int etd_debug_gemm3(const float* x_dev, int M, int K, const float* w_host, const float* bias_host, int N, float x_bound, int gelu, float* y_dev,
                    const float* ln_g_host, const float* ln_b_host, void* stream);
enum { ETD_G3_KERNEL_AUTO = 0 , ETD_G3_KERNEL_TILE = 1 , ETD_G3_KERNEL_SMALL = 2  };
enum { ETD_G3_EPI_BIAS = 0, ETD_G3_EPI_GELU = 1, ETD_G3_EPI_RESID = 2, ETD_G3_EPI_LOGITS = 3, ETD_G3_EPI_QKV = 4, ETD_G3_EPI_RELU = 6 };
typedef struct etd_debug_g3_case {
  int struct_bytes;
  int kernel, epi;
  int M, N, K, ldx, ldy;
  const float* X; long long x_elems;
  const float* W; const float* bias;
  float x_bound;
  const float* ln_g; const float* ln_b; float ln_eps;
  float* Y; long long y_elems;
  const float* add; const float* hin; float* hout; long long h_elems;
  const int32_t* pos; const int32_t* slot; const int32_t* active;
  int n_heads, max_ctx, n_slots, rope_rows;
  const float* rope_cos; const float* rope_sin;
  float* Q; long long q_elems;
  float* Kc; float* Vc; long long kv_elems;
} etd_debug_g3_case;
int etd_debug_gemm3_case(const etd_debug_g3_case* c, void* stream);
int etd_debug_ln_rows_f32(const float* h_dev, int M, int H, const float* g1_host, const float* b1_host, const float* g2_host, const float* b2_host, float eps,
                          float* x1_dev, float* x2_dev, void* stream);
int etd_debug_g3_pack(const float* W, int N, int K, uint16_t* planes_out, long long cap, long long* n_out, int32_t* log2_out);

int etd_debug_attn3(const float* q_dev, const float* k_dev, const float* v_dev, float* o_dev, int n_seq, int n_heads, int Sq, int Sk, float q_bound, float k_bound, float v_bound,
                    int causal, const int32_t* lens_host, void* stream);
struct etd_debug_attn3_case {
  int struct_bytes;
  int n_seq, n_heads, Sq, Sk;
  const float* Q; long long q_elems; int ldq; long long q_seq;
  const float* K; long long k_elems; int ldk; long long k_seq;
  const float* V; long long v_elems; int ldv; long long v_seq;
  float* O; long long o_elems; int ldo; long long o_seq;
  float q_bound, k_bound, v_bound;
  const int32_t* seq_len; const int32_t* slot_of_seq;
  long long slot_stride; int max_ctx, n_slots, row0;
  int32_t* log2_out3;
};
int etd_debug_attn3_case(const struct etd_debug_attn3_case* c, void* stream);
int etd_debug_dattn_f32(const float* q_dev, const float* kc_dev, const float* vc_dev, float* o_dev, long long qo_elems, long long kv_elems, int M, int n_heads, int n_slots,
                        int max_ctx, const int32_t* slot_host, const int32_t* pos_host, int form, void* stream);

int etd_debug_g3_bounds(const float* W, const float* c, int N, int K, const float* g, const float* b, float elem_bound, float* out4, int32_t* log2_out4);

int etd_beat_debug_taps(etd_beat*, float* front_dev, float* layer0_dev);
typedef struct etd_debug_beat_taps {
  int struct_bytes;
  unsigned layer_mask;
  int rows, frames, segs;
  int d_hid;
  int slices, islices;
  float *c1, *c2, *x3, *c3, *front;
  float *ln1, *qkv, *skip, *x_attn, *tacc, *ln2, *hid, *x_ffn;
  float *iln1, *iqkv, *iao, *ix_attn, *iln2, *ihid, *ix_ffn;
  float* part;
} etd_debug_beat_taps;
int etd_beat_debug_stage_taps(etd_beat*, const etd_debug_beat_taps* taps);

int etd_dbn_debug_viterbi(etd_dbn*, int hmm_index, const double* densities_dev, long long T, int32_t* path_out, double* logprob_out);

int etd_dtw_debug_cost(etd_dtw*, const float* const* feat_ptrs, long long N1, long long N2, int shift, float* cost_dev);
int etd_dtw_debug_total(etd_dtw*, const float* const* feat_ptrs, long long N1, long long N2, int shift, double* total_host);
int etd_dtw_debug_path(etd_dtw*, const float* const* feat_ptrs, long long N1, long long N2, int shift, int32_t* path_host, long long cap, long long* n_out);

int etd_alignfeat_debug_layout(const etd_alignfeat*, int n_songs, const int64_t* N_host, int song, int64_t* out, int n_out);

int etd_tuning_debug_layout(const etd_tuning*, int n_songs, const int64_t* N_host, int song, int64_t* out, int n_out);
int etd_tuning_debug_power(etd_tuning*, int song, const int32_t* frames_host, int n_frames, float* power_dev);

int etd_resample_debug_layout(const etd_resample*, int n_songs, const int64_t* frames_host, const int32_t* channels_host, const int32_t* mono_host, int64_t* out,
                              long long capacity, long long* n_tiles);

int etd_rhythm_debug_logioi(etd_rhythm*, double* logioi_dev, signed char* labels_dev, double* centres_dev);

int etd_debug_dtrain_gemm(int form, int M, int N, int K, const float* A_dev, int lda, const float* B_dev, int ldb, const float* bias_dev, float* C_dev, int ldc,
                          int accumulate, void* stream);
int etd_debug_dtrain_attn(int n_seq, const int32_t* T_host, int n_heads, const float* qkv_dev, const float* dO_dev, float* O_dev, float* lse_dev, float* dqkv_dev,
// ... 70 lines not shown
```

Before: 597.3.

## Memoize decoder layer-0 QKV and MLP partials per token key in prefill

```diff
diff --git a/etude_amd/_lib.py b/etude_amd/_lib.py
--- a/etude_amd/_lib.py
+++ b/etude_amd/_lib.py
@@ -262,6 +262,9 @@
     "etd_decoder_stamp": (C.c_int, [C.c_void_p, C.c_int, C.c_int, C.c_void_p]),
     "etd_decoder_stamp_log": (C.c_int, [C.c_void_p, C.c_void_p, C.c_longlong, C.POINTER(C.c_longlong), C.c_void_p]),
     "etd_debug_decoder_force_pair": (C.c_int, [C.c_void_p, C.c_int]),
+    "etd_debug_decoder_l0_key": (C.c_int, [C.c_void_p, C.c_int, C.c_int, C.c_void_p, C.POINTER(C.c_longlong)]),
+    "etd_debug_decoder_l0_key_space": (C.c_longlong, [C.c_void_p]),
+    "etd_debug_decoder_l0_capacity": (C.c_int, [C.c_void_p, C.c_int, C.c_void_p]),
     "etd_debug_decoder_step_logits": (C.c_int, [C.c_void_p, C.c_int, C.c_void_p, C.c_int, C.c_void_p]),
     "etd_debug_decoder_bar_logits": (C.c_int, [C.c_void_p, C.c_void_p, C.c_int, C.c_void_p]),
     "etd_debug_sample_rows": (C.c_int, [C.c_void_p, C.c_int, C.c_int, C.c_int, C.c_float, C.c_float, C.c_ulonglong, C.c_void_p, C.c_void_p, C.c_void_p, C.c_void_p]),
diff --git a/etude_amd/csrc/api_dec.hip b/etude_amd/csrc/api_dec.hip
--- a/etude_amd/csrc/api_dec.hip
+++ b/etude_amd/csrc/api_dec.hip
@@ -80,6 +80,14 @@
   float* logits_dbg = nullptr; bool logits_dbg_on = false, last_step_fused = false;
   int* sc_i = nullptr; float* sc_f = nullptr; double* sc_d = nullptr; float* sc_x = nullptr; int score_hb = 0;
   etd_debug_dec_taps taps = {}; bool taps_on = false;
+  float* l0_D0 = nullptr;
+  unsigned char* l0_QKV = nullptr;
+  int l0_cap = 0, l0_n = 0, l0_cap_req = 0;
+  std::vector<int> l0_map;
+  std::vector<int> l0_idx, l0_new;
+  const int* l0_rows_dev = nullptr;
+  bool l0_failed = false;
+  double stat_l0_fills = 0, stat_l0_passes = 0, stat_l0_overflows = 0, stat_l0_keys = 0, stat_l0_nomem = 0;
   etd_dec* weights_owner = nullptr;
   size_t n_weight_allocs = 0;
   int n_clones = 0; bool zombie = false;
@@ -423,6 +431,7 @@
     ma.X2 = d->X2b; ma.AO = d->Xcat + d->I; ma.ldao = d->I + d->H; ma.hin = hin; ma.hout = hout; ma.Wm = (const d16*)w.mlp_frag;
     ma.b_up = w.up.b; ma.b_cat = w.cat.b; ma.eps = d->cfg.layer_norm_eps; ma.M = M;
     ma.g1 = nx.g1; ma.b1 = nx.b1; ma.g2 = nx.g2; ma.b2 = nx.b2; ma.nx1 = nx.x1; ma.nx2 = nx.x2;
+    if (l == 0 && pf && d->l0_rows_dev) { ma.mode = DMLP_L0;       ma.D0 = d->l0_D0; ma.l0_row = d->l0_rows_dev; d->stat_l0_passes += 1; }
     ETD_TRY(tap_xcat(d, ts, M, st));
     ETD_TRY(launch_dmlp_fused(ma, st));
     return tap_rows(d, d->taps.hout, ts, hout, M, d->H, 4, st);
@@ -451,10 +460,15 @@
   const bool tail = lo && pf && lo->n > 1 && lo->n <= DS_STEP_MAX_ROWS && step_shape(d) && !getenv("ETD_NO_LAST_ONLY");
   float* hin = d->h; float* hout = d->h2;
   for (int l = 0; l < d->L; ++l) {
-    if (l == 0 || !fmlp) ETD_TRY(ln_rows16(d, l, hin, M, st));
+    const bool l0 = l == 0 && fmlp && pf && d->l0_rows_dev;
+    if ((l == 0 || !fmlp) && !l0) ETD_TRY(ln_rows16(d, l, hin, M, st));
     const int ts = tap_slice(d, l);
     ETD_TRY(tap_layer_in(d, ts, hin, M, st));
-    ETD_TRY(prefill16_qkv(d, l, hin, rows, M, pf != nullptr, st));
+    if (l0) {
+      L0QkvArgs qa = {}; qa.tab = d->l0_QKV; qa.l0_row = d->l0_rows_dev; qa.M = M; qa.rows = rows; qa.rope_cos = d->rope_cos; qa.rope_sin = d->rope_sin; qa.Qb = d->Qb;
+      qa.Kc = (d16*)kv_layer(d, d->Kc, 0); qa.Vc = (d16*)kv_layer(d, d->Vc, 0); qa.slot_stride = d->slot_stride; qa.max_ctx = d->ctx;
+      ETD_TRY(launch_l0_qkv(qa, st));
+    } else ETD_TRY(prefill16_qkv(d, l, hin, rows, M, pf != nullptr, st));
     ETD_TRY(pf ? tap_rows(d, d->taps.qb, ts, d->Qb, M, d->H, 2, st) : tap_rows(d, d->taps.q, ts, d->Q, M, d->H, 4, st));
     ETD_TRY(tail && l == d->L - 1 ? prefill16_last_rows(d, *lo, hin, hout, st) : prefill16_layer_rest(d, l, rows, M, pf, fmlp, hin, hout, st));
     std::swap(hin, hout);
@@ -511,6 +525,50 @@
   }
 }
 
+constexpr long long L0_MAX_KEYS = 1ll << 22;
+constexpr int L0_MAX_ROWS = 65536;
+static long long l0_key_space(const etd_dec_cfg& c) {
+  if (c.vocab_size < 1 || c.num_classes < 1 || c.num_attribute_bins < 1) return 0;
+  const double nb = c.num_attribute_bins, ks = (double)c.vocab_size * c.num_classes * nb * nb * nb * nb;
+  return ks < 9e18 ? (long long)ks : 0;
+}
+static inline long long l0_key(const etd_dec_cfg& c, int id, int cls, int a0, int a1, int a2, int a3) {
+  const long long nb = c.num_attribute_bins;
+  return (((((long long)id * c.num_classes + cls) * nb + a0) * nb + a1) * nb + a2) * nb + a3;
+}
+static inline bool l0_switched_off() { const char* e = getenv("ETD_NO_L0_TABLE"); return e && atoi(e) > 0; }
+static bool l0_eligible(const etd_dec* d, int M) {
+  const Layer& w0 = d->layers[0];
+  if (!d->bf16w || M <= DS_MAX_ROWS || d->L < 2 || !d->Qb || d->nh != 8 || !w0.qkv.Wf || !w0.up.Wf || !w0.cat.Wf || !w0.mlp_frag || d->H != 512 || d->I != 2048) return false;
+  if (!fused_pmlp_on() || l0_switched_off() || (d->taps_on && (d->taps.layer_mask & 1u) && (d->taps.ln1 || d->taps.ln2 || d->taps.xcat))) return false;
+  const long long ks = l0_key_space(d->cfg);
+  return ks > 0 && ks <= L0_MAX_KEYS;
+}
+static void l0_release(etd_dec* d) {
+  if (d->l0_D0) { (void)hipFree(d->l0_D0); d->l0_D0 = nullptr; }
+  if (d->l0_QKV) { (void)hipFree(d->l0_QKV); d->l0_QKV = nullptr; }
+  d->l0_cap = d->l0_n = 0; d->l0_map.clear();
+}
+static bool l0_prepare(etd_dec* d) {
+  if (d->l0_failed) { d->stat_l0_nomem += 1; return false; }
+  if (d->l0_D0) return true;
+  const long long ks = l0_key_space(d->cfg);
+  const int cap = d->l0_cap_req > 0 ? d->l0_cap_req : (int)std::min<long long>(ks, L0_MAX_ROWS);
+  if (hipMalloc((void**)&d->l0_D0, (size_t)cap * 512 * 4) != hipSuccess || hipMalloc((void**)&d->l0_QKV, (size_t)cap * L0Q_ROW_BYTES) != hipSuccess) {
+    (void)hipGetLastError();
+    if (d->l0_D0) { (void)hipFree(d->l0_D0); d->l0_D0 = nullptr; }
+    d->l0_QKV = nullptr; d->l0_failed = true; d->stat_l0_nomem += 1;
+    return false;
+  }
+  d->l0_cap = cap; d->l0_n = 0; d->l0_map.assign((size_t)ks, -1);
+  return true;
+}
+struct L0Pending {
+  etd_dec* d; bool committed = false;
+  void rollback() { for (int k : d->l0_new) d->l0_map[k] = -1; d->l0_new.clear(); }
+  ~L0Pending() { if (!committed) rollback(); }
+};
+
 struct Staged { int Mtot; const int *ids, *cls, *attrs, *row_slot, *row_pos, *row_active, *last_idx, *last_slot, *last_pos, *last_active, *init, *row_seq, *seq_row0, *seq_len; };
 
 int stage_and_forward(etd_dec* d, int n, const int32_t* slots, const int32_t* T, const int32_t* ids, const int32_t* cls,
@@ -532,7 +590,25 @@
     if (ids[i] < 0 || ids[i] >= d->V || cls[i] < 0 || cls[i] >= d->cfg.num_classes) ETD_FAIL(ETD_EINVAL, "prefill: token/class id out of range at row %d", i);
     for (int k = 0; k < 4; ++k) if (attrs4[(size_t)k * M + i] < 0 || attrs4[(size_t)k * M + i] >= d->cfg.num_attribute_bins) ETD_FAIL(ETD_EINVAL, "prefill: attribute bin out of range at row %d", i);
   }
-  const size_t sv_ints = (size_t)10 * M + 13 * n;
+  d->l0_new.clear();
+  L0Pending l0p{d};
+  bool l0 = l0_eligible(d, M) && l0_prepare(d);
+  if (l0) {
+    d->l0_idx.resize((size_t)M);
+    int* map = d->l0_map.data(); const int room = d->l0_cap - d->l0_n;
+    for (int i = 0; i < M && l0; ++i) {
+      const int key = (int)l0_key(d->cfg, ids[i], cls[i], attrs4[i], attrs4[(size_t)M + i], attrs4[(size_t)2 * M + i], attrs4[(size_t)3 * M + i]);
+      int r = map[key];
+      if (r < 0) {
+        if ((int)d->l0_new.size() >= room) { l0 = false; break; }
+        r = d->l0_n + (int)d->l0_new.size(); map[key] = r; d->l0_new.push_back(key);
+      }
+      d->l0_idx[i] = r;
+    }
+    if (!l0) { l0p.rollback(); d->stat_l0_overflows += 1; }
+  }
+  const int K = l0 ? (int)d->l0_new.size() : 0;
+  const size_t sv_ints = (size_t)10 * M + 13 * n + (l0 ? (size_t)M + 6 * (size_t)K : 0);
   int* svp;
   const bool pinned = d->pin_stage && sv_ints <= d->pin_stage_ints;
   if (pinned) {
@@ -558,6 +634,16 @@
     kvb += (double)T[i] * d->nh * 64 * (2.0 * (d->bf16w ? 2 : 4) + 4 + 4);
   }
   if (init7) memcpy(in7, init7, (size_t)7 * n * 4); else memset(in7, 0, (size_t)7 * n * 4);
+  if (l0) {
+    int* l0r = sln + n; int* nid = l0r + M; int* ncl = nid + K; int* nat = ncl + K;
+    memcpy(l0r, d->l0_idx.data(), (size_t)M * 4);
+    const int nb = d->cfg.num_attribute_bins, nc = d->cfg.num_classes;
+    for (int j = 0; j < K; ++j) {
+      int k = d->l0_new[j];
+      for (int a = 3; a >= 0; --a) { nat[(size_t)a * K + j] = k % nb; k /= nb; }
+      ncl[j] = k % nc; nid[j] = k / nc;
+    }
+  }
   d->attn_bytes_hint = kvb;
   HIP_TRY(hipMemcpyAsync(d->ids, svp, sv_ints * 4, hipMemcpyHostToDevice, st));
   if (pinned) HIP_TRY(hipEventRecord(d->pin_stage_evt, st));
@@ -573,14 +659,38 @@
     HIP_TRY(hipGetLastError());
   }
   DEmbedArgs e = {};
-  e.ids = sg->ids; e.cls = sg->cls; e.attrs = sg->attrs; e.M = M; e.H = d->H; e.n_bins = d->cfg.num_attribute_bins;
-  e.word = d->word; e.cls_emb = d->cls_emb; e.attr_tab = d->attr_tab; e.h = d->h;
+  e.H = d->H; e.n_bins = d->cfg.num_attribute_bins; e.word = d->word; e.cls_emb = d->cls_emb; e.attr_tab = d->attr_tab; e.h = d->h;
+  const int* l0_rows = l0 ? b + 10 * (size_t)M + 13 * n : nullptr;
+  if (K > 0) {
+    const int* nk = l0_rows + M;
+    e.ids = nk; e.cls = nk + K; e.attrs = nk + 2 * (size_t)K; e.M = K;
+    ETD_TRY(launch_dembed(e, st));
+    ETD_TRY(ln_rows16(d, 0, d->h, K, st));
+    const Layer& w0 = d->layers[0]; DMlpArgs fa = {};
+    fa.mode = DMLP_FILL; fa.D0 = d->l0_D0 + (size_t)d->l0_n * 512; fa.X2 = d->X2b; fa.AO = d->Xcat + d->I; fa.ldao = d->I + d->H; fa.hin = d->h; fa.hout = d->h2;
+    fa.Wm = (const d16*)w0.mlp_frag; fa.b_up = w0.up.b; fa.b_cat = w0.cat.b; fa.eps = d->cfg.layer_norm_eps; fa.M = K;
+    ETD_TRY(launch_dmlp_fused(fa, st));
+    const int chunk = (int)std::min<size_t>((size_t)K, (size_t)d->Mcap * (d->I + d->H) / 2 / 1536);
+    for (int k0 = 0; k0 < K; k0 += chunk) {
+      const int kn = std::min(chunk, K - k0);
+      DGemmArgs g = lin_args(w0.qkv, nullptr, d->H, kn); g.Y = reinterpret_cast<float*>(d->Xcat); g.ldy = 1536;
+      ETD_TRY(linear16(w0.qkv, d->X1b + (size_t)k0 * d->H, kn, g, DEPI_BIAS, st));
+      L0QkvArgs qa = {}; qa.tab = d->l0_QKV + (size_t)(d->l0_n + k0) * L0Q_ROW_BYTES; qa.raw = g.Y; qa.n = kn;
+      ETD_TRY(launch_l0_qkv_fill(qa, st));
+    }
+    d->l0_n += K; d->stat_l0_fills += 1; d->stat_l0_keys += K;
+  }
+  l0p.committed = true; d->l0_new.clear();
+  e.ids = sg->ids; e.cls = sg->cls; e.attrs = sg->attrs; e.M = M;
   e.rows = DecRows{sg->row_slot, sg->row_pos, sg->row_active, sg->row_seq};
   ETD_TRY(launch_dembed(e, st));
   PrefillInfo pf{n, sg->seq_row0, sg->seq_len, max_len, aflops};
   const bool can_mfma_attn = (d->bf16w ? d->Qb != nullptr : d->X1f != nullptr);
   LastOnly lo{n, sg->last_idx, DecRows{sg->last_slot, sg->last_pos, sg->last_active}};
-  return forward_rows(d, M, e.rows, can_mfma_attn ? &pf : nullptr, &lo, st, hfinal, last_only);
+  d->l0_rows_dev = l0_rows;
+  const int rc = forward_rows(d, M, e.rows, can_mfma_attn ? &pf : nullptr, &lo, st, hfinal, last_only);
+  d->l0_rows_dev = nullptr;
+  return rc;
 }
 
 int alloc_workspaces(etd_dec* d) {
@@ -613,13 +723,14 @@
   ETD_TRY(P.alloc(&d->samp_dev, (size_t)1, true)); ETD_TRY(P.alloc(&d->rng_key, (size_t)d->S, true));
   ETD_TRY(P.alloc(&d->row_sp, (size_t)2 * d->Mmax, true));
   ETD_TRY(P.alloc(&d->row_slot, (size_t)d->Mmax)); ETD_TRY(P.alloc(&d->row_pos, (size_t)d->Mmax)); ETD_TRY(P.alloc(&d->row_active, (size_t)d->Mmax));
-  ETD_TRY(P.alloc(&d->ids, 10 * M + 13 * (size_t)d->S)); ETD_TRY(P.alloc(&d->slots_dev, (size_t)d->S));
+  const size_t stage_ints = (d->bf16w ? 17 : 10) * M + 13 * (size_t)d->S;
+  ETD_TRY(P.alloc(&d->ids, stage_ints)); ETD_TRY(P.alloc(&d->slots_dev, (size_t)d->S));
   const size_t S = d->S;
   ETD_TRY(P.alloc(&d->cur_tok, S, true)); ETD_TRY(P.alloc(&d->len, S, true)); ETD_TRY(P.alloc(&d->done, S, true));
   ETD_TRY(P.alloc(&d->n_out, S, true)); ETD_TRY(P.alloc(&d->eos, S, true)); ETD_TRY(P.alloc(&d->limit, S, true));
   ETD_TRY(P.alloc(&d->tgt_proj, S * (size_t)d->H, true));
   ETD_TRY(P.alloc(&d->tgt_attrs, 4 * S, true)); ETD_TRY(P.alloc(&d->out_tok, S * d->out_cap, true));
-  d->pin_stage_ints = 10 * M + 13 * S;
+  d->pin_stage_ints = stage_ints;
   if (hipHostMalloc((void**)&d->pin_stage, d->pin_stage_ints * 4, hipHostMallocDefault) != hipSuccess) { d->pin_stage = nullptr; (void)hipGetLastError(); }
   if (hipHostMalloc((void**)&d->pin_rb, (2 * S + S * (size_t)d->out_cap) * 4, hipHostMallocDefault) != hipSuccess) { d->pin_rb = nullptr; (void)hipGetLastError(); }
   if (d->pin_stage && hipEventCreateWithFlags(&d->pin_stage_evt, hipEventDisableTiming) != hipSuccess) { (void)hipHostFree(d->pin_stage); d->pin_stage = nullptr; d->pin_stage_evt = nullptr; }
@@ -856,6 +967,7 @@
   if (d->trace_q) { (void)hipFree(d->trace_q); d->trace_q = nullptr; }
   if (d->trace_dbg) { (void)hipFree(d->trace_dbg); d->trace_dbg = nullptr; }
   if (d->stamp_dev) { (void)hipFree(d->stamp_dev); d->stamp_dev = nullptr; }
+  l0_release(d);
   if (d->logits_dbg) { (void)hipFree(d->logits_dbg); d->logits_dbg = nullptr; }
   if (d->sc_i) { (void)hipFree(d->sc_i); d->sc_i = nullptr; }
   if (d->sc_f) { (void)hipFree(d->sc_f); d->sc_f = nullptr; }
@@ -1090,8 +1202,9 @@
   double w = 0;
   for (const Layer& l : d->layers) w += ((double)l.qkv.N * l.qkv.K + (double)l.dense.N * l.dense.K + (double)l.up.N * l.up.K + (double)l.down.N * l.down.K) * (d->bf16w ? 2.0 : 4.0);
   w += (double)d->V * d->H * (d->bf16w ? 2.0 : 4.0);
-  const double v[8] = {d->stat_steps, d->stat_row_steps, d->stat_kv_bytes, d->stat_attn_launches, (double)n_stamped, (double)sum_ticks * 1e-8 , d->stat_stamp_bytes, w};
-  for (int i = 0; i < n; ++i) out[i] = i < 8 ? v[i] : 0.0;
+  const double v[13] = {d->stat_steps, d->stat_row_steps, d->stat_kv_bytes, d->stat_attn_launches, (double)n_stamped, (double)sum_ticks * 1e-8 , d->stat_stamp_bytes, w,
+                        d->stat_l0_fills, d->stat_l0_passes, d->stat_l0_overflows, d->stat_l0_keys, d->stat_l0_nomem};
+  for (int i = 0; i < n; ++i) out[i] = i < 13 ? v[i] : 0.0;
   return ETD_OK;
 }
 
@@ -1116,6 +1229,7 @@
 extern "C" int etd_decoder_stats_reset(etd_dec* d, void* stream) {
   if (!d) ETD_FAIL(ETD_EINVAL, "decoder_stats_reset: null handle");
   d->stat_steps = d->stat_row_steps = d->stat_kv_bytes = d->stat_attn_launches = d->stat_stamp_bytes = 0;
+  d->stat_l0_fills = d->stat_l0_passes = d->stat_l0_overflows = d->stat_l0_keys = d->stat_l0_nomem = 0;
   if (d->stamp_dev) {
     HIP_TRY(hipStreamSynchronize((hipStream_t)stream));
     HIP_TRY(hipMemset(d->stamp_dev, 0, ETD_STAMP_HDR * 8));
@@ -1131,6 +1245,22 @@
   }
   HIP_TRY(hipStreamSynchronize((hipStream_t)stream));
   d->stamp_armed = on != 0; d->stamp_on = false; d->stamp_skip = on ? skip_steps : 0;
+  return ETD_OK;
+}
+
+extern "C" long long etd_debug_decoder_l0_key_space(const etd_dec_cfg* cfg) { return cfg ? l0_key_space(*cfg) : 0; }
+extern "C" int etd_debug_decoder_l0_key(const etd_dec_cfg* cfg, int id, int cls, const int32_t* attrs4, long long* key) {
+  if (!cfg || !attrs4 || !key || l0_key_space(*cfg) <= 0) ETD_FAIL(ETD_EINVAL, "l0_key: bad arguments");
+  if (id < 0 || id >= cfg->vocab_size || cls < 0 || cls >= cfg->num_classes) ETD_FAIL(ETD_EINVAL, "l0_key: token/class id out of range");
+  for (int a = 0; a < 4; ++a) if (attrs4[a] < 0 || attrs4[a] >= cfg->num_attribute_bins) ETD_FAIL(ETD_EINVAL, "l0_key: attribute bin out of range");
+  *key = l0_key(*cfg, id, cls, attrs4[0], attrs4[1], attrs4[2], attrs4[3]);
+  return ETD_OK;
+}
+extern "C" int etd_debug_decoder_l0_capacity(etd_dec* d, int rows, void* stream) {
+  if (!d || rows < 0) ETD_FAIL(ETD_EINVAL, "l0_capacity: bad arguments");
+  HIP_TRY(hipStreamSynchronize((hipStream_t)stream));
+  l0_release(d);
+  d->l0_cap_req = rows; d->l0_failed = false;
   return ETD_OK;
 }
 
diff --git a/etude_amd/csrc/dec_epilogue.h b/etude_amd/csrc/dec_epilogue.h
--- a/etude_amd/csrc/dec_epilogue.h
+++ b/etude_amd/csrc/dec_epilogue.h
@@ -26,10 +26,7 @@
 #pragma unroll
       for (int i = 0; i < 4; ++i) {
         const int d = i + 4 * h;
-        const float c = cs[d], s = sn[d];
-        const float x1 = v[i], x2 = v[i + 4];
-        v[i] = x1 * c - x2 * s;
-        v[i + 4] = x2 * c + x1 * s;
+        rope_pair(v[i], v[i + 4], cs[d], sn[d]);
       }
     }
     if (a.Qb && part == 0) {
diff --git a/etude_amd/csrc/dec_fused.hip b/etude_amd/csrc/dec_fused.hip
--- a/etude_amd/csrc/dec_fused.hip
+++ b/etude_amd/csrc/dec_fused.hip
@@ -199,7 +199,7 @@
 #else
 #define PMS(i) do { } while (0)
 #endif
-__global__ __launch_bounds__(256) __attribute__((amdgpu_waves_per_eu(1, 1))) void k_dmlp_fused(DMlpArgs a) {
+template <int MODE> __global__ __launch_bounds__(256) __attribute__((amdgpu_waves_per_eu(1, 1))) void k_dmlp_fused(DMlpArgs a) {
   __shared__ __attribute__((aligned(16))) unsigned char smem[2 * PM_SLOT_ELEMS * 2 + 2048 * 4];
   d16* ring = reinterpret_cast<d16*>(smem);
   float* sbu = reinterpret_cast<float*>(smem + 2 * PM_SLOT_ELEMS * 2);
@@ -225,13 +225,13 @@
     __syncthreads();                                     \
   } while (0)
   auto next_of = [&](int k) {
-    return PmNext{a.Wm + (long long)(k + 1) * PM_SLOT_ELEMS + wave * (16 * 512) + lane * 8, ring + ((k + 1) & 1) * PM_SLOT_ELEMS + wave * (16 * 512), k + 1 < DMLP_NCHUNK};
+    return PmNext{a.Wm + (long long)(k + 1) * PM_SLOT_ELEMS + wave * (16 * 512) + lane * 8, ring + ((k + 1) & 1) * PM_SLOT_ELEMS + wave * (16 * 512), k + 1 < (MODE == DMLP_FILL ? 65 : DMLP_NCHUNK)};
   };
 
-  issue(0);
+  issue(MODE == DMLP_L0 ? 65 : 0);
   d16x8 xf[32];
   {
-    const d16* xp = a.X2 + (long long)mc * 512 + 8 * h;
+    const d16* xp = MODE == DMLP_L0 ? a.AO + (long long)mc * a.ldao + 8 * h : a.X2 + (long long)mc * 512 + 8 * h;
 #define PM_X4(S) PM_LOADX(xf[S], xp, S); PM_LOADX(xf[(S) + 1], xp, (S) + 1); PM_LOADX(xf[(S) + 2], xp, (S) + 2); PM_LOADX(xf[(S) + 3], xp, (S) + 3)
     PM_X4(0); PM_X4(4); PM_X4(8); PM_X4(12); PM_X4(16); PM_X4(20); PM_X4(24); PM_X4(28);
 #undef PM_X4
@@ -240,19 +240,34 @@
 #ifdef ETD_PMLP_STAMP
   const unsigned long long ps_tx = __builtin_amdgcn_s_memtime();
 #endif
-  for (int i = tid; i < 2048; i += 256) sbu[i] = a.b_up[i];
+  if constexpr (MODE != DMLP_L0) for (int i = tid; i < 2048; i += 256) sbu[i] = a.b_up[i];
 
   f32x16 acc2[16];
-#pragma unroll
-  for (int t = 0; t < 16; ++t)
-#pragma unroll
-    for (int i = 0; i < 16; ++i) acc2[t][i] = 0.f;
+  if constexpr (MODE == DMLP_L0) {
+    const float* dp = a.D0 + (long long)a.l0_row[mc] * 512 + 16 * h;
+#pragma unroll
+    for (int t = 0; t < 16; ++t)
+#pragma unroll
+      for (int q = 0; q < 4; ++q) {
+        const f32x4 v = *reinterpret_cast<const f32x4*>(dp + 32 * t + 4 * q);
+        acc2[t][4 * q] = v[0]; acc2[t][4 * q + 1] = v[1]; acc2[t][4 * q + 2] = v[2]; acc2[t][4 * q + 3] = v[3];
+      }
+  } else {
+#pragma unroll
+    for (int t = 0; t < 16; ++t)
+#pragma unroll
+      for (int i = 0; i < 16; ++i) acc2[t][i] = 0.f;
+  }
   f32x16 accA, accB;
   d16x8 buf[2][4], hf[2];
   using seq8 = std::make_integer_sequence<int, 8>;
   using seq16 = std::make_integer_sequence<int, 16>;
 #define PM_ZERO(x) _Pragma("unroll") for (int i_ = 0; i_ < 16; ++i_) x[i_] = 0.f
 
+#ifdef ETD_PMLP_STAMP
+  unsigned long long ps_acc[5] = {0, 0, 0, 0, 0}, ps_t = ps_tx, ps_t1 = ps_tx, ps_t2 = ps_tx, ps_t2b = ps_tx;
+#endif
+  if constexpr (MODE != DMLP_L0) {
   {
     PM_TOP(0);
     PM_ZERO(accA);
@@ -261,8 +276,8 @@
     pm_gelu2<0>(accA, sbu, 0, h); pm_gelu2<1>(accA, sbu, 0, h);
   }
 #ifdef ETD_PMLP_STAMP
-  unsigned long long ps_acc[5] = {0, 0, 0, 0, 0}, ps_t = __builtin_amdgcn_s_memtime();
-  const unsigned long long ps_t1 = ps_t;
+  ps_t = __builtin_amdgcn_s_memtime();
+  ps_t1 = ps_t;
 #define PM_TOP_S(k)                                                                         \
   do {                                                                                      \
     if ((k) > 1) PMS(0); else ps_t = __builtin_amdgcn_s_memtime();                          \
@@ -283,10 +298,10 @@
     PM_CHUNK(k, accA, accB, false);
     PM_CHUNK(k + 1, accB, accA, false);
   }
-  PM_CHUNK(63, accA, accB, true);
+  PM_CHUNK(63, accA, accB, MODE == DMLP_FULL);
 #ifdef ETD_PMLP_STAMP
   PMS(0);
-  const unsigned long long ps_t2 = ps_t;
+  ps_t2 = ps_t;
 #endif
   {
     PM_TOP(64);
@@ -297,8 +312,28 @@
     pm_down_only(buf, sa, acc2, hf, next_of(64), seq8{});
   }
 #ifdef ETD_PMLP_STAMP
-  const unsigned long long ps_t2b = __builtin_amdgcn_s_memtime();
-#endif
+  ps_t2b = __builtin_amdgcn_s_memtime();
+#endif
+  }
+  if constexpr (MODE == DMLP_FILL) {
+    asm volatile("s_nop 15\n\ts_nop 15" : "+a"(acc2[0]), "+a"(acc2[1]), "+a"(acc2[2]), "+a"(acc2[3]), "+a"(acc2[4]), "+a"(acc2[5]), "+a"(acc2[6]), "+a"(acc2[7]) : : "memory");
+    asm volatile("" : "+v"(acc2[8]), "+v"(acc2[9]), "+v"(acc2[10]), "+v"(acc2[11]), "+v"(acc2[12]), "+v"(acc2[13]), "+v"(acc2[14]), "+v"(acc2[15]));
+    if (m < a.M) {
+      float* dp = a.D0 + (long long)m * 512 + 16 * h;
+#pragma unroll
+      for (int t = 0; t < 16; ++t)
+#pragma unroll
+        for (int q = 0; q < 4; ++q) {
+          const f32x4 v = {acc2[t][4 * q], acc2[t][4 * q + 1], acc2[t][4 * q + 2], acc2[t][4 * q + 3]};
+          *reinterpret_cast<f32x4*>(dp + 32 * t + 4 * q) = v;
+        }
+    }
+    return;
+  }
+  if constexpr (MODE == DMLP_L0) {
+    asm volatile("s_nop 7\n\ts_nop 7" : "+a"(acc2[0]), "+a"(acc2[1]), "+a"(acc2[2]), "+a"(acc2[3]), "+a"(acc2[4]), "+a"(acc2[5]), "+a"(acc2[6]), "+a"(acc2[7]),
+                 "+v"(acc2[8]), "+v"(acc2[9]), "+v"(acc2[10]), "+v"(acc2[11]), "+v"(acc2[12]), "+v"(acc2[13]), "+v"(acc2[14]), "+v"(acc2[15]) : : "memory");
+  }
   { PM_TOP(65); pm_dense_chunk<0>(buf, ring_lds + (65 & 1) * (PM_SLOT_ELEMS * 2), acc2, xf, next_of(65), seq16{}); }
   { PM_TOP(66); pm_dense_chunk<1>(buf, ring_lds + (66 & 1) * (PM_SLOT_ELEMS * 2), acc2, xf, next_of(66), seq16{}); }
   { PM_TOP(67); pm_dense_chunk<2>(buf, ring_lds + (67 & 1) * (PM_SLOT_ELEMS * 2), acc2, xf, next_of(67), seq16{}); }
@@ -447,10 +482,20 @@
 int launch_dmlp_fused(const DMlpArgs& a, hipStream_t st) {
   if (a.M <= 0 || !a.X2 || !a.AO || a.ldao < 512 || (a.ldao % 8) || !a.hin || !a.hout || a.hin == a.hout || !a.Wm || !a.b_up || !a.b_cat ||
       (((uintptr_t)a.X2 | (uintptr_t)a.AO | (uintptr_t)a.Wm | (uintptr_t)a.hin | (uintptr_t)a.hout | (uintptr_t)a.nx1 | (uintptr_t)a.nx2) & 15) ||
-      (a.nx1 && (!a.nx2 || !a.g1 || !a.b1 || !a.g2 || !a.b2)))
+      (a.nx1 && (!a.nx2 || !a.g1 || !a.b1 || !a.g2 || !a.b2)) || a.mode < DMLP_FULL || a.mode > DMLP_L0 ||
+      (a.mode != DMLP_FULL && (!a.D0 || ((uintptr_t)a.D0 & 15))) || (a.mode == DMLP_L0 && !a.l0_row))
     ETD_FAIL(ETD_EINVAL, "dmlp_fused: bad arguments");
-  ProfScope ps("k_dmlp_fused", st, 2.0 * a.M * 512.0 * (2048.0 * 2 + 512.0), (double)a.M * 512 * (2 + 2 + 4 + 4 + (a.nx1 ? 4 : 0)) + (double)DMLP_STREAM_ELEMS * 2);
-  hipLaunchKernelGGL(k_dmlp_fused, dim3((a.M + 127) / 128), dim3(256), 0, st, a);
+  const dim3 grid((a.M + 127) / 128);
+  if (a.mode == DMLP_FILL) {
+    ProfScope ps("k_dmlp_fused_fill", st, 2.0 * a.M * 512.0 * 2048.0 * 2, (double)a.M * 512 * (2 + 4) + 65.0 * PM_SLOT_ELEMS * 2);
+    hipLaunchKernelGGL(k_dmlp_fused<DMLP_FILL>, grid, dim3(256), 0, st, a);
+  } else if (a.mode == DMLP_L0) {
+    ProfScope ps("k_dmlp_fused_l0", st, 2.0 * a.M * 512.0 * 512.0, (double)a.M * 512 * (4 + 2 + 4 + 4 + (a.nx1 ? 4 : 0)) + (double)a.M * 4 + 8.0 * PM_SLOT_ELEMS * 2);
+    hipLaunchKernelGGL(k_dmlp_fused<DMLP_L0>, grid, dim3(256), 0, st, a);
+  } else {
+    ProfScope ps("k_dmlp_fused", st, 2.0 * a.M * 512.0 * (2048.0 * 2 + 512.0), (double)a.M * 512 * (2 + 2 + 4 + 4 + (a.nx1 ? 4 : 0)) + (double)DMLP_STREAM_ELEMS * 2);
+    hipLaunchKernelGGL(k_dmlp_fused<DMLP_FULL>, grid, dim3(256), 0, st, a);
+  }
   HIP_TRY(hipGetLastError());
   return ETD_OK;
 }
diff --git a/etude_amd/csrc/dec_kernels.h b/etude_amd/csrc/dec_kernels.h
--- a/etude_amd/csrc/dec_kernels.h
+++ b/etude_amd/csrc/dec_kernels.h
@@ -126,6 +126,25 @@
   d16* Kc; d16* Vc; long long slot_stride; int max_ctx, n_heads;
 };
 int launch_pqkv(const PQkvArgs& a, hipStream_t st);
+#ifdef __HIPCC__
+__device__ __forceinline__ void rope_pair(float& x1, float& x2, float c, float s) {
+  const float a = x1 * c - x2 * s, b = x2 * c + x1 * s;
+  x1 = a; x2 = b;
+}
+#endif
+#define L0Q_ROT_FLOATS 256
+#define L0Q_ROW_BYTES (L0Q_ROT_FLOATS * 4 + 1536 * 2)
+struct L0QkvArgs {
+  unsigned char* tab;
+  const float* raw; int n;
+  const int* l0_row; int M;
+  DecRows rows;
+  const float* rope_cos; const float* rope_sin;
+  d16* Qb;
+  d16* Kc; d16* Vc; long long slot_stride; int max_ctx;
+};
+int launch_l0_qkv_fill(const L0QkvArgs& a, hipStream_t st);
+int launch_l0_qkv(const L0QkvArgs& a, hipStream_t st);
 
 int launch_ln_rows(const float* h, int M, int H, const float* g1, const float* b1, const float* g2, const float* b2, float eps,
                    d16* x1, d16* x2, hipStream_t st);
@@ -145,7 +164,9 @@
   const float* g1; const float* b1; const float* g2; const float* b2; float eps;
   d16* nx1; d16* nx2;
   int M;
+  int mode; float* D0; const int* l0_row;
 };
+enum { DMLP_FULL = 0, DMLP_FILL = 1, DMLP_L0 = 2 };
 int launch_dmlp_fused(const DMlpArgs& a, hipStream_t st);
 void pack_dmlp_weights(const uint16_t* Wup_bf16 , const uint16_t* Wcat_bf16 , uint16_t* dst );
 
diff --git a/etude_amd/csrc/dec_prefill.hip b/etude_amd/csrc/dec_prefill.hip
--- a/etude_amd/csrc/dec_prefill.hip
+++ b/etude_amd/csrc/dec_prefill.hip
@@ -263,9 +263,7 @@
       if (part < 2) {
 #pragma unroll
         for (int i = 0; i < 4; ++i) {
-          const float x1 = v[0][i], x2 = v[0][i + 4];
-          v[0][i] = x1 * c4[i] - x2 * s4[i];
-          v[0][i + 4] = x2 * c4[i] + x1 * s4[i];
+          rope_pair(v[0][i], v[0][i + 4], c4[i], s4[i]);
         }
       }
 #pragma unroll
@@ -295,3 +293,73 @@
   HIP_TRY(hipGetLastError());
   return ETD_OK;
 }
+
+__global__ __launch_bounds__(192) void k_l0_qkv_fill(L0QkvArgs a) {
+  const int key = blockIdx.x, c = threadIdx.x, head = c / 24, part = (c - head * 24) >> 3, ch = c & 7;
+  const float* src = a.raw + (long long)key * 1536 + c * 8;
+  const f32x4 lo = *reinterpret_cast<const f32x4*>(src), hi = *reinterpret_cast<const f32x4*>(src + 4);
+  unsigned char* row = a.tab + (long long)key * L0Q_ROW_BYTES;
+  d16* hp = reinterpret_cast<d16*>(row + L0Q_ROT_FLOATS * 4) + c * 8;
+  *reinterpret_cast<d16x4*>(hp) = pack4d(lo[0], lo[1], lo[2], lo[3]);
+  *reinterpret_cast<d16x4*>(hp + 4) = pack4d(hi[0], hi[1], hi[2], hi[3]);
+  if (part < 2 && ch < 2) {
+    float* rp = reinterpret_cast<float*>(row) + (head * 2 + part) * 16 + ch * 8;
+    *reinterpret_cast<f32x4*>(rp) = lo; *reinterpret_cast<f32x4*>(rp + 4) = hi;
+  }
+}
+__global__ __launch_bounds__(256) void k_l0_qkv(L0QkvArgs a) {
+  const int lane = threadIdx.x & 63, m = blockIdx.x * 4 + (threadIdx.x >> 6);
+  if (m >= a.M) return;
+  const unsigned char* row = a.tab + (long long)a.l0_row[m] * L0Q_ROW_BYTES;
+  const float* rot = reinterpret_cast<const float*>(row);
+  const d16* hp = reinterpret_cast<const d16*>(row + L0Q_ROT_FLOATS * 4);
+  const int pos = a.rows.pos[m], slot = a.rows.slot[m];
+  const bool kv_on = a.rows.active[m] && pos < a.max_ctx;
+  const int pt = pos < a.max_ctx ? pos : a.max_ctx - 1;
+  const float* cs = a.rope_cos + (long long)pt * 8; const float* sn = a.rope_sin + (long long)pt * 8;
+#pragma unroll
+  for (int j = 0; j < 3; ++j) {
+    const int c = lane + 64 * j, head = c / 24, part = (c - head * 24) >> 3, ch = c & 7;
+    if (part < 2 && ch == 1) continue;
+    d16* dst;
+    if (part == 0) dst = a.Qb + (long long)m * 512 + head * 64 + ch * 8;
+    else {
+      if (!kv_on) continue;
+      dst = (part == 1 ? a.Kc : a.Vc) + (long long)slot * a.slot_stride + ((long long)head * a.max_ctx + pos) * 64 + ch * 8;
+    }
+    if (part < 2 && ch == 0) {
+      const float* rp = rot + (head * 2 + part) * 16;
+      f32x4 x[4];
+#pragma unroll
+      for (int q = 0; q < 4; ++q) x[q] = *reinterpret_cast<const f32x4*>(rp + 4 * q);
+      float v[16];
+#pragma unroll
+      for (int q = 0; q < 4; ++q)
+#pragma unroll
+        for (int e = 0; e < 4; ++e) v[4 * q + e] = x[q][e];
+#pragma unroll
+      for (int d = 0; d < 8; ++d) rope_pair(v[d], v[d + 8], cs[d], sn[d]);
+#pragma unroll
+      for (int q = 0; q < 4; ++q) *reinterpret_cast<d16x4*>(dst + 4 * q) = pack4d(v[4 * q], v[4 * q + 1], v[4 * q + 2], v[4 * q + 3]);
+    } else {
+      *reinterpret_cast<u32x4*>(dst) = *reinterpret_cast<const u32x4*>(hp + c * 8);
+    }
+  }
+}
+
+int launch_l0_qkv_fill(const L0QkvArgs& a, hipStream_t st) {
+  if (!a.tab || !a.raw || a.n <= 0 || (((uintptr_t)a.tab | (uintptr_t)a.raw) & 15)) ETD_FAIL(ETD_EINVAL, "l0_qkv_fill: bad arguments");
+  ProfScope ps("k_l0_qkv_fill", st, 0, (double)a.n * (1536 * 4 + L0Q_ROW_BYTES));
+  hipLaunchKernelGGL(k_l0_qkv_fill, dim3(a.n), dim3(192), 0, st, a);
+  HIP_TRY(hipGetLastError());
+  return ETD_OK;
+}
+int launch_l0_qkv(const L0QkvArgs& a, hipStream_t st) {
+  if (!a.tab || !a.l0_row || a.M <= 0 || !a.rows.pos || !a.rows.slot || !a.rows.active || !a.rope_cos || !a.rope_sin || !a.Qb || !a.Kc || !a.Vc || (a.slot_stride % 8) ||
+      (((uintptr_t)a.tab | (uintptr_t)a.Qb | (uintptr_t)a.Kc | (uintptr_t)a.Vc) & 15))
+    ETD_FAIL(ETD_EINVAL, "l0_qkv: bad arguments");
+  ProfScope ps("k_l0_qkv", st, 0, (double)a.M * (L0Q_ROW_BYTES - 512 + 3 * 1024 + 16));
+  hipLaunchKernelGGL(k_l0_qkv, dim3((a.M + 3) / 4), dim3(256), 0, st, a);
+  HIP_TRY(hipGetLastError());
+  return ETD_OK;
+}
diff --git a/etude_amd/csrc/ext_kernels.hip b/etude_amd/csrc/ext_kernels.hip
--- a/etude_amd/csrc/ext_kernels.hip
+++ b/etude_amd/csrc/ext_kernels.hip
@@ -293,9 +293,7 @@
               const f32x4 s4 = *reinterpret_cast<const f32x4*>(g.rope_sin + (long long)pos_l * 8 + 4 * h);
 #pragma unroll
               for (int i = 0; i < 4; ++i) {
-                const float x1 = v[0][i], x2 = v[0][i + 4];
-                v[0][i] = x1 * c4[i] - x2 * s4[i];
-                v[0][i + 4] = x2 * c4[i] + x1 * s4[i];
+                rope_pair(v[0][i], v[0][i + 4], c4[i], s4[i]);
               }
             }
 #pragma unroll
diff --git a/include/etude_hip_debug.h b/include/etude_hip_debug.h
--- a/include/etude_hip_debug.h
+++ b/include/etude_hip_debug.h
@@ -49,6 +49,9 @@
   float* next_h; void *next_ln1, *next_ln2; int32_t* next_pos;
 } etd_debug_dec_taps;
 int etd_debug_decoder_stage_taps(etd_dec*, const etd_debug_dec_taps* taps, void* stream);
+int etd_debug_decoder_l0_key(const etd_dec_cfg* cfg, int id, int cls, const int32_t* attrs4, long long* key);
+long long etd_debug_decoder_l0_key_space(const etd_dec_cfg* cfg);
+int etd_debug_decoder_l0_capacity(etd_dec*, int rows, void* stream);
 int etd_debug_decoder_peek_kv_many(etd_dec*, int layer, int n, const int32_t* slots, int n_pos, unsigned short* k_out, unsigned short* v_out, void* stream);
 
 int etd_debug_sample_rows(const float* logits_dev, int M, int V, int ld, float temperature, float top_p, unsigned long long seed,
```

After: 605.3 (median of 6 runs). Within noise of the previous version (+1.3%).
